# PTsolvers/JustRelax.jl

Hardware: AMD Instinct MI355X
Metric: PT-iterations/s (3D Stokes SolVi3D, 512^3 fp64 block per GPU, block-iterations summed over GPUs) (higher is better)
Workload: dtype f64; 1 GPU; SolVi3D 512^3 per GPU (configs[3]): eta inclusion 1e-3, G=1, K=Inf, dt=Inf, free-slip, pure shear; kernel_form=viscous_limit_no_body_forces, halo=none, arrays=library constructor, field_placement=1 (pool-dealt chunks, mapped once), operand_cache=0

## Files before the change

justrelax.jl_amd/csrc/handle.hip:

```cpp
#include "jrx_internal.hpp"
#include "jrx_tuning.h"

char g_jrx_create_err[512] = {0};

jrx_status jrx_ensure_etatau(jrx_handle *h, size_t n)
{
    if (h->etatau_cap >= n) return JRX_OK;
    if (h->etatau) JRX_TRY(jrx_dev_free(h, h->etatau));
    h->etatau = nullptr;
    h->etatau_cap = 0;
    JRX_TRY(jrx_dev_alloc(h, n * sizeof(double), (void **)&h->etatau, 2));
    h->etatau_cap = n;
    return JRX_OK;
}

jrx_status jrx_check_device(jrx_handle *h)
{
    if (!h) return JRX_ERR_ARG;
    int cur = -1;
    JRX_HIP(h, hipGetDevice(&cur));
    if (cur != h->device)
        return jrx_fail(h, JRX_ERR_ARG, "this handle is bound to device %d but the calling thread's current device is %d (hipSetDevice / torch.cuda.set_device "
                                        "first: the library does not change it)", h->device, cur);
    return JRX_OK;
}

extern "C" {

int32_t jrx_version(void) { return JRX_VERSION; }

#ifndef JRX_BUILD_ID
#define JRX_BUILD_ID "unknown"
#endif
static const char g_jrx_build_marker[] = "JRX_BUILD_ID=" JRX_BUILD_ID;
const char *jrx_build_id(void) { return g_jrx_build_marker + 13; }

const char *jrx_last_error(const jrx_handle *h) { return h ? h->err : g_jrx_create_err; }

jrx_status jrx_create(int32_t device, jrx_handle **out)
{
    if (!out) return jrx_fail(nullptr, JRX_ERR_ARG, "jrx_create: out is NULL");
    *out = nullptr;
    int ndev = 0;
    if (hipGetDeviceCount(&ndev) != hipSuccess || ndev <= 0)
        return jrx_fail(nullptr, JRX_ERR_HIP, "jrx_create: no HIP device visible");
    if (device < 0 || device >= ndev) return jrx_fail(nullptr, JRX_ERR_ARG, "jrx_create: device %d out of range [0,%d)", device, ndev);
    jrx_handle *h = new jrx_handle();
    h->device = device;
    int prev_device = -1;
    (void)hipGetDevice(&prev_device);
#define CK(call)                                                                                   \
    do {                                                                                           \
        hipError_t e_ = (call);                                                                    \
        if (e_ != hipSuccess) {                                                                    \
            jrx_status st_ = jrx_fail(nullptr, JRX_ERR_HIP, "jrx_create: %s -> %s", #call, hipGetErrorString(e_)); \
            (void)jrx_destroy(h);                  \
            if (prev_device >= 0) (void)hipSetDevice(prev_device);                                 \
            return st_;                                                                            \
        }                                                                                          \
    } while (0)
    CK(hipSetDevice(device));
    CK(hipStreamCreateWithFlags(&h->stream, hipStreamNonBlocking));
    {
        int lo = 0, hi = 0;
        CK(hipDeviceGetStreamPriorityRange(&lo, &hi));
        CK(hipStreamCreateWithPriority(&h->halo_stream, hipStreamNonBlocking, hi));
    }
    for (int i = 0; i < 3; i++) CK(hipEventCreateWithFlags(&h->ev[i], hipEventDisableTiming));
    for (int i = 3; i < 8; i++) CK(hipEventCreate(&h->ev[i]));
    CK(hipMalloc(&h->d_partials, sizeof(double) * 4 * kMaxRedBlocks));
    CK(hipMalloc(&h->d_sums, sizeof(double) * 16));
    CK(hipMemset(h->d_sums, 0, sizeof(double) * 16));
    CK(hipHostMalloc(&h->h_sums, sizeof(double) * 16, hipHostMallocDefault));
#undef CK
    if (prev_device >= 0 && prev_device != device) (void)hipSetDevice(prev_device);
    *out = h;
    return JRX_OK;
}

jrx_status jrx_destroy(jrx_handle *h)
{
    if (!h) return JRX_OK;
    (void)hipSetDevice(h->device);
    if (h->comm) (void)jrx_comm_destroy(h);
    if (h->stream) (void)hipStreamSynchronize(h->stream);
    if (h->halo_stream) (void)hipStreamSynchronize(h->halo_stream);
    for (int i = 0; i < 8; i++)
        if (h->ev[i]) (void)hipEventDestroy(h->ev[i]);
    if (h->d_partials) (void)hipFree(h->d_partials);
    if (h->d_sums) (void)hipFree(h->d_sums);
    if (h->h_sums) (void)hipHostFree(h->h_sums);
    jrx_pool_destroy(h);
    for (int q = 0; q < 3; q++)
        if (h->tscratch2[q]) (void)hipFree(h->tscratch2[q]);
    for (int q = 0; q < 6; q++)
        if (h->scratch2d[q]) (void)hipFree(h->scratch2d[q]);
    if (h->stream) (void)hipStreamDestroy(h->stream);
    if (h->halo_stream) (void)hipStreamDestroy(h->halo_stream);
    delete h;
    return JRX_OK;
}

namespace {
struct OptRef { const char *key; int kind; void *p; };
int find_opt(jrx_handle *h, const char *key, bool tuning, OptRef *out)
{
    const OptRef pub[] = {
        {"kernel_variant", 1, &h->kernel_variant}, {"fused_overlap", 1, &h->fused_overlap}, {"thermal_fused", 0, &h->thermal_fused},
        {"fused_comm", 0, &h->fused_comm}, {"loop_graphs", 0, &h->loop_graphs}, {"scratch_sets", 0, &h->scratch_sets},
        {"viscous_limit", 0, &h->viscous_limit}, {"field_placement", 1, &h->field_placement}, {"field_chunk_mib", 1, &h->field_chunk_mib}, {"operand_cache", 0, &h->operand_cache}, {"stat_operand_cache_hits", 2, &h->stat_operand_cache_hits}, {"stat_fused3d_general_hif", 2, &h->stat_fused3d_general_hif},
        {"stat_fused3d", 2, &h->stat_fused3d}, {"stat_fused2d", 2, &h->stat_fused2d}, {"stat_fused2d_b", 2, &h->stat_fused2d_b}, {"stat_sweeps3d", 2, &h->stat_sweeps3d}, {"stat_thermal_fused", 2, &h->stat_thermal_fused},
        {"stat_vep3_fused", 2, &h->stat_vep3_fused}, {"stat_graph_replays", 2, &h->stat_graph_replays},
        {"stat_fused3d_visc", 2, &h->stat_fused3d_visc}, {"stat_fused3d_inkernel", 2, &h->stat_fused3d_inkernel}, {"stat_visc_checks", 2, &h->stat_visc_checks}, {"stat_visc_fallbacks", 2, &h->stat_visc_fallbacks}, {"stat_fused3d_nof1", 2, &h->stat_fused3d_nof1}, {"stat_fused3d_nof2", 2, &h->stat_fused3d_nof2},
        {"stat_weno_calls", 2, &h->stat_weno_calls}, {"stat_weno_fused", 2, &h->stat_weno_fused}, {"stat_principal_calls", 2, &h->stat_principal_calls},
    };
    const OptRef tun[] = {
        {"fused_split", 0, &h->fused_split}, {"fused_tile", 1, &h->fused_tile}, {"fused_ylds", 0, &h->fused_ylds}, {"fused_hiface", 0, &h->fused_hiface}, {"visc_fold", 0, &h->visc_fold}, {"zero_forces", 0, &h->zero_forces}, {"scratch_stagger", 1, &h->scratch_stagger}, {"scratch_contiguous", 0, &h->scratch_contiguous}, {"end_flips", 0, &h->end_flips}, {"comm_bcs_lazy", 0, &h->comm_bcs_lazy}, {"fused_first_pct", 1, &h->fused_first_pct},
        {"b_width_x", 1, &h->b_width_opt[0]}, {"b_width_y", 1, &h->b_width_opt[1]}, {"b_width_z", 1, &h->b_width_opt[2]},
        {"halo_self_rccl", 0, &h->halo_self_rccl}, {"thermal_cfg", 1, &h->thermal_cfg}, {"thermal_xg", 1, &h->thermal_xg}, {"thermal_tile", 1, &h->thermal_tile}, {"thermal_nt", 0, &h->thermal_nt},
        {"fused2d", 0, &h->fused2d}, {"vep3_edges", 1, &h->vep3_edges}, {"vep3_cfg", 1, &h->vep3_cfg}, {"vep3_peel", 0, &h->vep3_peel}, {"vep3_peel_fork", 0, &h->vep3_peel_fork}, {"vep3_nt", 0, &h->vep3_nt}, {"vep3_prekz", 1, &h->vep3_prekz},
        {"vep3_hide_comm", 1, &h->vep3_hide_comm}, {"vep3_fork", 0, &h->vep3_fork}, {"vep3_fuse_pc", 0, &h->vep3_fuse_pc}, {"vep3_np_const", 0, &h->vep3_np_const}, {"vep3_prec_tile", 1, &h->vep3_prec_tile}, {"thermal_np_const", 0, &h->thermal_np_const}, {"thermal_fused_ph", 0, &h->thermal_fused_ph}, {"fused2d_batch", 0, &h->fused2d_batch}, {"fused2d_max_nodes", 1, &h->fused2d_max_nodes}, {"vep3_map", 0, &h->vep3_map}, {"vep3_xcd", 0, &h->vep3_xcd}, {"comm_timeout_ms", 1, &h->comm_timeout_ms}, {"vep_store_all", 0, &h->vep_store_all}, {"chain_profile", 0, &h->chain_profile},
        {"general_hif", 1, &h->general_hif}, {"field_shuffle", 0, &h->field_shuffle}, {"field_pool_pct", 1, &h->field_pool_pct}, {"fused_kz", 1, &h->fused_kz}, {"fused_ym", 1, &h->fused_ym}, {"nbr_feeder", 0, &h->nbr_feeder}, {"stat_fused3d_ym", 2, &h->stat_fused3d_ym}, {"scratch_poison", 1, &h->scratch_poison},
        {"weno_fused", 0, &h->weno_fused}, {"weno_rows", 1, &h->weno_rows},
    };
    if (tuning) {
        for (const OptRef &o : tun)
            if (strcmp(o.key, key) == 0) { *out = o; return 1; }
    } else {
        for (const OptRef &o : pub)
            if (strcmp(o.key, key) == 0) { *out = o; return 1; }
    }
    return 0;
}
jrx_status opt_set(jrx_handle *h, const char *key, int64_t value, bool tuning, const char *fn)
{
    if (!h) return JRX_ERR_ARG;
    if (!key) return jrx_fail(h, JRX_ERR_ARG, "%s: key is NULL", fn);
    OptRef o;
    if (!find_opt(h, key, tuning, &o)) {
        if (find_opt(h, key, !tuning, &o))
            return jrx_fail(h, JRX_ERR_ARG, "%s: '%s' is %s", fn, key, tuning ? "an option of the public ABI (jrx_set_option)" : "a tuning switch (jrx_tuning_set, include/jrx_tuning.h)");
        return jrx_fail(h, JRX_ERR_ARG, "%s: unknown key '%s'", fn, key);
    }
    if (o.kind == 2) return jrx_fail(h, JRX_ERR_ARG, "%s: '%s' is a read-only counter", fn, key);
    if (o.kind == 0) *(bool *)o.p = value != 0;
    else *(int *)o.p = (int)value;
    if (strcmp(key, "comm_timeout_ms") == 0) jrx_comm_set_timeout(h, (double)value * 1e-3);
    return JRX_OK;
}
jrx_status opt_get(jrx_handle *h, const char *key, int64_t *value, bool tuning, const char *fn)
{
    if (!h) return JRX_ERR_ARG;
    if (!key || !value) return jrx_fail(h, JRX_ERR_ARG, "%s: null argument", fn);
    OptRef o;
    if (!find_opt(h, key, tuning, &o)) return jrx_fail(h, JRX_ERR_ARG, "%s: unknown key '%s'", fn, key);
    *value = o.kind == 0 ? (int64_t)*(bool *)o.p : (o.kind == 1 ? (int64_t)*(int *)o.p : *(int64_t *)o.p);
    return JRX_OK;
}
}

jrx_status jrx_fields_dirty(jrx_handle *h)
{
    if (!h) return JRX_ERR_ARG;
    h->opv.valid = false;
    return JRX_OK;
}
jrx_status jrx_set_option(jrx_handle *h, const char *key, int64_t value) { return opt_set(h, key, value, false, "jrx_set_option"); }
jrx_status jrx_get_option(jrx_handle *h, const char *key, int64_t *value) { return opt_get(h, key, value, false, "jrx_get_option"); }
jrx_status jrx_tuning_set(jrx_handle *h, const char *key, int64_t value) { return opt_set(h, key, value, true, "jrx_tuning_set"); }
jrx_status jrx_tuning_get(jrx_handle *h, const char *key, int64_t *value) { return opt_get(h, key, value, true, "jrx_tuning_get"); }
jrx_status jrx_tuning_chain_profile(jrx_handle *h, double out_us[8], int64_t *samples)
{
    if (!h) return JRX_ERR_ARG;
    if (!out_us || !samples) return jrx_fail(h, JRX_ERR_ARG, "jrx_tuning_chain_profile: null argument");
    for (int q = 0; q < 8; q++) out_us[q] = h->chain_us[q];
    *samples = h->chain_n;
    return JRX_OK;
}

int64_t jrx_n_global(int64_t n, int32_t dims, int32_t periodic)
{
    if (n == 1) return 1;
    return (int64_t)dims * (n - 2) + (periodic ? 0 : 2);
}

jrx_status jrx_halo_planes(int64_t n, int64_t nA, int64_t *send_left, int64_t *send_right, int64_t *recv_left, int64_t *recv_right)
{
    const int64_t ol = 2 + (nA - n);
    if (ol < 2 || nA < ol) return JRX_ERR_ARG;
    if (send_left) *send_left = ol - 1;
    if (send_right) *send_right = nA - ol;
    if (recv_left) *recv_left = 0;
    if (recv_right) *recv_right = nA - 1;
    return JRX_OK;
}

jrx_status jrx_cart_create(int32_t rank, int32_t nprocs, const int64_t n[3], const int32_t dims_in[3],
                           const int32_t periods[3], jrx_cart *out)
{
    if (!out || !n || nprocs < 1 || rank < 0 || rank >= nprocs) return JRX_ERR_ARG;
    int32_t dims[3] = {1, 1, 1};
    const bool fixed = dims_in && (dims_in[0] || dims_in[1] || dims_in[2]);
    if (fixed) {
        for (int d = 0; d < 3; d++) dims[d] = dims_in[d] ? dims_in[d] : 1;
    } else {
        int idx[3], na = 0;
        for (int d = 0; d < 3; d++)
            if (n[d] > 1) idx[na++] = d;
        if (na > 0) {
            int fac[32], nf = 0, m = nprocs;
            for (int p = 2; m > 1; p++)
                while (m % p == 0) { fac[nf++] = p; m /= p; }
            int v[3] = {1, 1, 1};
            for (int q = nf - 1; q >= 0; q--) {
                int j = 0;
                for (int a = 1; a < na; a++)
                    if (v[a] < v[j]) j = a;
                v[j] *= fac[q];
            }
            for (int a = 0; a < na; a++)
                for (int b = a + 1; b < na; b++)
                    if (v[b] > v[a]) { int t = v[a]; v[a] = v[b]; v[b] = t; }
            for (int a = 0; a < na; a++) dims[idx[a]] = v[a];
        }
    }
    if ((int64_t)dims[0] * dims[1] * dims[2] != nprocs) return JRX_ERR_ARG;
    out->rank = rank; out->nprocs = nprocs;
    int r = rank;
    for (int d = 2; d >= 0; d--) { out->coords[d] = r % dims[d]; r /= dims[d]; }
    for (int d = 0; d < 3; d++) { out->dims[d] = dims[d]; out->periods[d] = periods ? periods[d] : 0; }
    for (int d = 0; d < 3; d++)
        for (int sgn = 0; sgn < 2; sgn++) {
            int c[3] = {out->coords[0], out->coords[1], out->coords[2]};
            c[d] += sgn ? 1 : -1;
            int nb = -1;
            if (c[d] >= 0 && c[d] < dims[d]) nb = (c[0] * dims[1] + c[1]) * dims[2] + c[2];
            else if (out->periods[d]) {
                c[d] = (c[d] + dims[d]) % dims[d];
                nb = (c[0] * dims[1] + c[1]) * dims[2] + c[2];
            }
            out->neighbor[d][sgn] = nb;
        }
    return JRX_OK;
}

}
```

justrelax.jl_amd/csrc/jrx_internal.hpp:

```cpp
#pragma once
#include <hip/hip_runtime.h>
#include <cstdarg>
#include <cstdint>
#include <cstdio>
#include <cstring>
#include <cmath>
#include "jrx.h"

struct jrx_comm_state;
struct jrx_field_pool;

struct jrx_handle {
    int device = 0;
    hipStream_t stream = nullptr;
    hipStream_t halo_stream = nullptr;
    hipEvent_t ev[8] = {};
    double *d_partials = nullptr;
    double *d_sums = nullptr;
    double *h_sums = nullptr;
    double *etatau = nullptr;
    size_t etatau_cap = 0;
    jrx_comm_state *comm = nullptr;
    jrx_field_pool *pool = nullptr;
    int field_placement = 0;
    int field_chunk_mib = 64;
    bool field_shuffle = true;
    int scratch_poison = 0;
    int fused_kz = 0;
    int field_pool_pct = 70;
    double *scratch_base[10] = {};
    bool scratch_contiguous = false;
    int scratch_stagger = 0, scratch_stagger_used = 0;
    double *scratch[10] = {};
    int scratch_dims[3] = {0, 0, 0};
    double *tscratch[4] = {};
    int tscratch_dims[3] = {0, 0, 0};
    double *scratch2d[6] = {};
    int scratch2d_dims[2] = {0, 0};
    double *tscratch2[3] = {};
    int tscratch2_dims[2] = {0, 0};
    bool loop_graphs = true;
    bool thermal_fused = true;
    int fused_overlap = 3;
    int kernel_variant = 0;
    bool fused_split = false;
    int fused_tile = 2;
    bool fused_comm = true;
    bool vep_store_all = false;
    bool viscous_limit = true;
    bool visc_ok = false;
    int fused_first_pct = 15;
    bool comm_bcs_lazy = false;
    bool end_flips = true;
    bool zero_forces = true;
    bool operand_cache = false;
    struct { bool valid = false; const void *ptr[14] = {}; int64_t n[3] = {}; double dt = 0.0; int flags = 0; bool visc_ok = false; int nof = 0; } opv;
    int64_t stat_operand_cache_hits = 0;
    int nof = 0;
    bool visc_fold = true;
    bool fused_hiface = true;
    bool fused_ylds = true;
    int general_hif = 0;
    int64_t stat_fused3d_general_hif = 0;
    bool nbr_feeder = true;
    int fused_ym = 0;
    int64_t stat_fused3d_ym = 0;
    int b_width_opt[3] = {0, 0, 0};
    bool halo_self_rccl = false;
    int thermal_cfg = 0, thermal_xg = 8;
    bool thermal_nt = false;
    int thermal_tile = 0;
    bool fused2d = true;
    bool vep3_peel = true;
    bool vep3_peel_fork = false;
    bool vep3_nt = false;
    int vep3_prekz = 0;
    int vep3_cfg = 0;
    int vep3_edges = 4;
    int vep3_hide_comm = 0;
    bool fused2d_batch = true;
    int fused2d_max_nodes = 1200000;
    bool thermal_fused_ph = true;
    bool thermal_np_const = true;
    int vep3_prec_tile = 2;
    bool vep3_np_const = true;
    bool vep3_fuse_pc = true;
    bool vep3_fork = false;
    bool vep3_map = true, vep3_xcd = true;
    bool scratch_sets = true;
    bool weno_fused = true;
    int weno_rows = 0;
    int64_t stat_weno_calls = 0, stat_weno_fused = 0;
    int64_t stat_principal_calls = 0;
    int64_t stat_fused3d_inkernel = 0;
    int64_t stat_fused3d_visc = 0, stat_visc_checks = 0, stat_visc_fallbacks = 0, stat_fused3d_nof1 = 0, stat_fused3d_nof2 = 0;
    int64_t stat_sweeps3d = 0;
    int64_t stat_fused2d_b = 0;
    int64_t stat_fused3d = 0, stat_fused2d = 0, stat_thermal_fused = 0, stat_vep3_fused = 0, stat_graph_replays = 0;
    bool chain_profile = false;
    double chain_us[8] = {};
    int64_t chain_n = 0;
    int comm_timeout_ms = 120000;
    char err[512] = {0};
};

static constexpr int kMaxRedBlocks = 2048;

extern char g_jrx_create_err[512];

static inline jrx_status jrx_fail(jrx_handle *h, jrx_status st, const char *fmt, ...)
{
    char *dst = h ? h->err : g_jrx_create_err;
    va_list ap;
    va_start(ap, fmt);
    vsnprintf(dst, 512, fmt, ap);
    va_end(ap);
    return st;
}

#define JRX_HIP(h, call)                                                                         \
    do {                                                                                         \
        hipError_t e_ = (call);                                                                  \
        if (e_ != hipSuccess)                                                                    \
            return jrx_fail((h), JRX_ERR_HIP, "%s:%d: %s -> %s", __FILE__, __LINE__, #call,      \
                            hipGetErrorString(e_));                                              \
    } while (0)

#define JRX_TRY(call)                          \
    do {                                       \
        jrx_status s_ = (call);                \
        if (s_ != JRX_OK) return s_;           \
    } while (0)

#define JRX_LAUNCH_CHECK(h) JRX_HIP(h, hipGetLastError())

struct GraphExecs {
    hipGraphExec_t g[2] = {nullptr, nullptr};
    GraphExecs() = default;
    GraphExecs(const GraphExecs &) = delete;
    GraphExecs &operator=(const GraphExecs &) = delete;
    ~GraphExecs() { reset(); }
    void reset() { for (auto &x : g) if (x) { (void)hipGraphExecDestroy(x); x = nullptr; } }
    hipGraphExec_t &operator[](int i) { return g[i]; }
};

template <class F>
static inline jrx_status jrx_capture_graph(hipStream_t s, hipGraphExec_t *out, F &&body)
{
    *out = nullptr;
    if (hipStreamBeginCapture(s, hipStreamCaptureModeThreadLocal) != hipSuccess) { (void)hipGetLastError(); return JRX_OK; }
    const jrx_status st = body();
    hipGraph_t g = nullptr;
    const hipError_t e = hipStreamEndCapture(s, &g);
    if (st == JRX_OK && e == hipSuccess && g && hipGraphInstantiate(out, g, nullptr, nullptr, 0) != hipSuccess) *out = nullptr;
    if (g) (void)hipGraphDestroy(g);
    (void)hipGetLastError();
    return st;
}
static constexpr double kGraphCells3D = 48.0 * 48.0 * 48.0;

jrx_status jrx_check_device(jrx_handle *h);

jrx_status jrx_dev_alloc(jrx_handle *h, size_t bytes, void **out, int tag = 4);
jrx_status jrx_dev_free(jrx_handle *h, void *p);
void jrx_pool_destroy(jrx_handle *h);

jrx_status jrx_ensure_etatau(jrx_handle *h, size_t n);

__device__ __forceinline__ double wave_sum(double v)
{
#pragma unroll
    for (int off = 32; off > 0; off >>= 1) v += __shfl_down(v, off, 64);
    return v;
}

typedef long long i64;

__device__ __forceinline__ i64 clampll(i64 v, i64 lo, i64 hi) { return v < lo ? lo : (v > hi ? hi : v); }
__device__ __forceinline__ int clampi(int v, int lo, int hi) { return v < lo ? lo : (v > hi ? hi : v); }

__device__ __forceinline__ double dev_dtau_r(double theta_dtau, double eta, double _Gdt)
{
    return 1.0 / (theta_dtau + fma(eta, _Gdt, 1.0));
}
__device__ __forceinline__ double dev_stress_inc(double t, double to, double eta, double e, double _Gdt, double dtr)
{
    return dtr * fma(2.0 * eta, e, fma(-(t - to) * eta, _Gdt, -t));
}

jrx_status jrx_halo_exchange(jrx_handle *h, hipStream_t s, int narrays, double *const *arrays,
                             const int64_t (*ext)[3], const int64_t n[3]);
bool jrx_comm_active(const jrx_handle *h);
jrx_status jrx_allreduce_sum_host(jrx_handle *h, double *vals, int count);
jrx_status jrx_allreduce_host(jrx_handle *h, double *vals, int count, int op);
int jrx_comm_rank(const jrx_handle *h);
void jrx_comm_set_timeout(jrx_handle *h, double seconds);
bool jrx_comm_has_neighbor(const jrx_handle *h, int d, int side);

jrx_status jrx3d_velocity_sweep(jrx_handle *h, hipStream_t s, const jrx_stokes3d_fields *f, const double *etatau, const jrx_stokes3d_params *p, bool diag, int nof = 0);
jrx_status jrx3d_forces_zero(jrx_handle *h, hipStream_t s, const double *fx, const double *fy, const double *fz, int64_t nc, int *nof);
jrx_status jrx3d_velocity_hidden(jrx_handle *h, const jrx_stokes3d_fields *f, const double *etatau, const jrx_stokes3d_params *p, bool diag, int bc_kind);
jrx_status jrx3d_scaleU(jrx_handle *h, hipStream_t s, const jrx_stokes3d_fields *f, const jrx_stokes3d_params *p);
jrx_status jrx3d_bcs(jrx_handle *h, hipStream_t s, double *Vx, double *Vy, double *Vz, int nx, int ny, int nz, uint32_t fs, uint32_t ns, uint32_t pe);
jrx_status jrx3d_bcs_faces(jrx_handle *h, hipStream_t s, double *Vx, double *Vy, double *Vz, int nx, int ny, int nz, uint32_t fs, uint32_t ns);
jrx_status jrx3d_sumsq(jrx_handle *h, hipStream_t s, const jrx_stokes3d_fields *f, const jrx_stokes3d_params *p);

jrx_status jrx2d_bcs(jrx_handle *h, hipStream_t s, double *Vx, double *Vy, int nx, int ny, uint32_t fs, uint32_t ns, uint32_t pe);
jrx_status jrx2d_sumsq(jrx_handle *h, hipStream_t s, const jrx_stokes2d_fields *f, const jrx_stokes2d_params *p);
bool jrx2d_spacing_ok(const double *const sp[6]);
```

justrelax.jl_amd/csrc/stokes3d.hip:

```cpp
#include <vector>
#include <cstdlib>
#include "jrx_internal.hpp"
#include "jrx_kernels.hpp"
#include "stokes3d_kernels.hpp"
#include "jrx_tuning.h"

namespace {

SweepArgs make_args(const jrx_stokes3d_fields *f, const double *etatau, const jrx_stokes3d_params *p)
{
    SweepArgs a;
    a.f = *f;
    a.o = Out10{f->P, f->txx, f->tyy, f->tzz, f->tyz, f->txz, f->txy, f->Vx, f->Vy, f->Vz};
    a.etatau = etatau;
    a._dx = p->_dx; a._dy = p->_dy; a._dz = p->_dz;
    a.dt = p->dt; a.r = p->r; a.theta_dtau = p->theta_dtau; a.eta_dtau = p->eta_dtau;
    a.L = make_lay((int)p->nx, (int)p->ny, (int)p->nz);
    a.i0 = a.j0 = a.k0 = 0;
    a.i1 = a.j1 = a.k1 = 0;
    return a;
}

jrx_status check_params(jrx_handle *h, const jrx_stokes3d_fields *f, const jrx_stokes3d_params *p)
{
    if (!h) return JRX_ERR_ARG;
    if (!f || !p) return jrx_fail(h, JRX_ERR_ARG, "null fields/params");
    JRX_TRY(jrx_check_device(h));
    if (p->nx < 3 || p->ny < 3 || p->nz < 3) return jrx_fail(h, JRX_ERR_ARG, "3D Stokes needs at least 3 cells per dimension");
    const double cells = (double)(p->nx + 2) * (double)(p->ny + 2) * (double)(p->nz + 2);
    if (cells >= 2147483647.0) return jrx_fail(h, JRX_ERR_UNSUPPORTED, "local block too large for 32-bit plane indices");
    const void *req[] = {f->P, f->P0, f->Q, f->Vx, f->Vy, f->Vz, f->txx, f->tyy, f->tzz, f->tyz, f->txz, f->txy,
                         f->toxx, f->toyy, f->tozz, f->toyz, f->toxz, f->toxy, f->eta, f->K, f->G, f->fx, f->fy, f->fz};
    for (const void *q : req)
        if (!q) return jrx_fail(h, JRX_ERR_ARG, "a required field pointer is NULL");
    return JRX_OK;
}

jrx_status check_diag(jrx_handle *h, const jrx_stokes3d_fields *f)
{
    const void *req[] = {f->divV, f->exx, f->eyy, f->ezz, f->eyz, f->exz, f->exy, f->RP, f->Rx, f->Ry, f->Rz, f->Ux, f->Uy, f->Uz};
    for (const void *q : req)
        if (!q) return jrx_fail(h, JRX_ERR_ARG, "a diagnostic field pointer (∇V, ε, R, U) is NULL");
    return JRX_OK;
}

jrx_status launch_stress_v1(jrx_handle *h, hipStream_t s, SweepArgs a, bool diag, int i0, int i1, int j0, int j1, int k0, int k1)
{
    if (i1 <= i0 || j1 <= j0 || k1 <= k0) return JRX_OK;
    a.i0 = i0; a.i1 = i1; a.j0 = j0; a.j1 = j1; a.k0 = k0; a.k1 = k1;
    const i64 plane = (i64)(i1 - i0) * (j1 - j0);
    dim3 grid((unsigned)((plane + 255) / 256), (unsigned)(k1 - k0));
    if (diag) hipLaunchKernelGGL(k_stress3d<true>, grid, dim3(256), 0, s, a);
    else hipLaunchKernelGGL(k_stress3d<false>, grid, dim3(256), 0, s, a);
    JRX_LAUNCH_CHECK(h);
    return JRX_OK;
}

jrx_status launch_velocity_v1(jrx_handle *h, hipStream_t s, SweepArgs a, bool diag, int i0, int i1, int j0, int j1, int k0, int k1)
{
    if (i1 <= i0 || j1 <= j0 || k1 <= k0) return JRX_OK;
    a.i0 = i0; a.i1 = i1; a.j0 = j0; a.j1 = j1; a.k0 = k0; a.k1 = k1;
    const i64 plane = (i64)(i1 - i0) * (j1 - j0);
    dim3 grid((unsigned)((plane + 255) / 256), (unsigned)(k1 - k0));
    if (diag) hipLaunchKernelGGL(k_velocity3d<true>, grid, dim3(256), 0, s, a);
    else hipLaunchKernelGGL(k_velocity3d<false>, grid, dim3(256), 0, s, a);
    JRX_LAUNCH_CHECK(h);
    return JRX_OK;
}

bool fits_u32(const Lay3 &L)
{
    const double m = (double)(L.nx + 2) * (double)(L.ny + 2) * (double)(L.nz + 2) * 8.0;
    return m < 4294967296.0;
}

template <class F>
__device__ __forceinline__ void scan_pairs(const double *__restrict__ p, i64 n, F f)
{
    if (n <= 0) return;
    const i64 stride = (i64)gridDim.x * blockDim.x, t0 = (i64)blockIdx.x * blockDim.x + threadIdx.x;
    const i64 head = (reinterpret_cast<uintptr_t>(p) & 15) ? 1 : 0;
    const double2 *__restrict__ q = reinterpret_cast<const double2 *>(p + head);
    const i64 m = n - head;
    for (i64 t = t0; t < (m >> 1); t += stride) { const double2 v = q[t]; f(v.x); f(v.y); }
    if (t0 == 0) { if (head) f(p[0]); if (m & 1) f(p[n - 1]); }
}
__global__ __launch_bounds__(256) void k_visc_operands_ok(const double *__restrict__ c0, const double *__restrict__ c1, const double *__restrict__ c2, const double *__restrict__ c3,
                                                          const double *__restrict__ c4, const double *__restrict__ eta, i64 nc, const double *__restrict__ K, const double *__restrict__ G,
                                                          const double *__restrict__ yz, i64 nyz, const double *__restrict__ xz, i64 nxz, const double *__restrict__ xy, i64 nxy, int *bad,
                                                          const unsigned long long *__restrict__ fx, const unsigned long long *__restrict__ fy, const unsigned long long *__restrict__ fz)
{
    bool b = false;
    unsigned long long bxy = 0, bz = 0;
    auto fin = [&](double v) { b |= !isfinite(v); };
    auto mod = [&](double v) { b |= (v != v) || v == 0.0; };
    scan_pairs(c0, nc, fin); scan_pairs(c1, nc, fin); scan_pairs(c2, nc, fin); scan_pairs(c3, nc, fin); scan_pairs(c4, nc, fin); scan_pairs(eta, nc, fin);
    scan_pairs(K, nc, mod); scan_pairs(G, nc, mod);
    scan_pairs(yz, nyz, fin); scan_pairs(xz, nxz, fin); scan_pairs(xy, nxy, fin);
    if (fx) {
        scan_pairs(reinterpret_cast<const double *>(fx), nc, [&](double v) { bxy |= (unsigned long long)__double_as_longlong(v); });
        scan_pairs(reinterpret_cast<const double *>(fy), nc, [&](double v) { bxy |= (unsigned long long)__double_as_longlong(v); });
        scan_pairs(reinterpret_cast<const double *>(fz), nc, [&](double v) { bz |= (unsigned long long)__double_as_longlong(v); });
    }
    if (__any(b) && (threadIdx.x & 63) == 0) atomicOr(bad, 1);
    if (fx) {
        const int m = (__any(bxy != 0) ? 2 : 0) | (__any(bz != 0) ? 4 : 0);
        if (m && (threadIdx.x & 63) == 0) atomicOr(bad, m);
    }
}

__global__ __launch_bounds__(256) void k_forces_zero(const unsigned long long *__restrict__ fx, const unsigned long long *__restrict__ fy, const unsigned long long *__restrict__ fz, i64 nc, int *bad)
{
    const i64 stride = (i64)gridDim.x * blockDim.x;
    unsigned long long bxy = 0, bz = 0;
    for (i64 t = (i64)blockIdx.x * blockDim.x + threadIdx.x; t < nc; t += stride) { bxy |= fx[t] | fy[t]; bz |= fz[t]; }
    const int m = (__any(bxy != 0) ? 2 : 0) | (__any(bz != 0) ? 4 : 0);
    if (m && (threadIdx.x & 63) == 0) atomicOr(bad, m);
}

static jrx_status visc_operands_local(jrx_handle *h, const jrx_stokes3d_fields *f, const jrx_stokes3d_params *p, bool forces);
jrx_status visc_operands_check(jrx_handle *h, const jrx_stokes3d_fields *f, const jrx_stokes3d_params *p, bool forces = true)
{
    JRX_TRY(visc_operands_local(h, f, p, forces));
    if (jrx_comm_active(h)) {
        double v[2] = {h->visc_ok ? 0.0 : 1.0, (double)(2 - h->nof)};
        JRX_TRY(jrx_allreduce_host(h, v, 2, 1));
        h->visc_ok = v[0] == 0.0;
        h->nof = 2 - (int)v[1];
    }
    return JRX_OK;
}
static jrx_status visc_operands_local(jrx_handle *h, const jrx_stokes3d_fields *f, const jrx_stokes3d_params *p, bool forces)
{
    h->visc_ok = false;
    h->nof = 0;
    forces = forces && h->zero_forces && f->fx && f->fy && f->fz;
    const void *key[14] = {f->P0, f->Q, f->toxx, f->toyy, f->tozz, f->toyz, f->toxz, f->toxy, f->eta, f->K, f->G, f->fx, f->fy, f->fz};
    const int kflags = (forces ? 1 : 0) | (h->viscous_limit ? 2 : 0) | (p->displacement_bcs ? 4 : 0) | (h->kernel_variant << 3);
    if (h->operand_cache && h->opv.valid && h->opv.dt == p->dt && h->opv.flags == kflags && h->opv.n[0] == p->nx && h->opv.n[1] == p->ny && h->opv.n[2] == p->nz &&
        memcmp(h->opv.ptr, key, sizeof(key)) == 0) {
        h->visc_ok = h->opv.visc_ok;
        h->nof = h->opv.nof;
        h->stat_operand_cache_hits++;
        return JRX_OK;
    }
    struct Remember {
        jrx_handle *h; const void *const *key; const jrx_stokes3d_params *p; int kflags; bool ok = false;
        ~Remember() {
            h->opv.valid = ok;
            if (!ok) return;
            memcpy(h->opv.ptr, key, sizeof(h->opv.ptr));
            h->opv.n[0] = p->nx; h->opv.n[1] = p->ny; h->opv.n[2] = p->nz; h->opv.dt = p->dt; h->opv.flags = kflags; h->opv.visc_ok = h->visc_ok; h->opv.nof = h->nof;
        }
    } remember{h, key, p, kflags};
    if ((!h->viscous_limit || p->dt != INFINITY) && forces && !p->displacement_bcs && (h->kernel_variant == 0 || h->kernel_variant == 3) && p->nx >= 48) {
        const i64 nc = (i64)p->nx * p->ny * p->nz;
        int *d_bad = reinterpret_cast<int *>(h->d_sums + 6), *h_bad = reinterpret_cast<int *>(h->h_sums + 6);
        hipStream_t s = h->stream;
        JRX_HIP(h, hipMemsetAsync(d_bad, 0, sizeof(double), s));
        hipLaunchKernelGGL(k_forces_zero, dim3(2048), dim3(256), 0, s, reinterpret_cast<const unsigned long long *>(f->fx), reinterpret_cast<const unsigned long long *>(f->fy),
                           reinterpret_cast<const unsigned long long *>(f->fz), nc, d_bad);
        JRX_LAUNCH_CHECK(h);
        JRX_HIP(h, hipMemcpyAsync(h_bad, d_bad, sizeof(double), hipMemcpyDeviceToHost, s));
        JRX_HIP(h, hipStreamSynchronize(s));
        if (!(*h_bad & 2)) h->nof = (*h_bad & 4) ? 1 : 2;
        remember.ok = true;
        return JRX_OK;
    }
    if (!h->viscous_limit || p->dt != INFINITY) { remember.ok = true; return JRX_OK; }
    const i64 nx = p->nx, ny = p->ny, nz = p->nz;
    int *d_bad = reinterpret_cast<int *>(h->d_sums + 6), *h_bad = reinterpret_cast<int *>(h->h_sums + 6);
    hipStream_t s = h->stream;
    JRX_HIP(h, hipMemsetAsync(d_bad, 0, sizeof(double), s));
    hipLaunchKernelGGL(k_visc_operands_ok, dim3(4096), dim3(256), 0, s, f->P0, f->Q, f->toxx, f->toyy, f->tozz, f->eta, nx * ny * nz, f->K, f->G, f->toyz, nx * (ny + 1) * (nz + 1),
                       f->toxz, (nx + 1) * ny * (nz + 1), f->toxy, (nx + 1) * (ny + 1) * nz, d_bad,
                       forces ? reinterpret_cast<const unsigned long long *>(f->fx) : nullptr, reinterpret_cast<const unsigned long long *>(f->fy), reinterpret_cast<const unsigned long long *>(f->fz));
    JRX_LAUNCH_CHECK(h);
    JRX_HIP(h, hipMemcpyAsync(h_bad, d_bad, sizeof(double), hipMemcpyDeviceToHost, s));
    JRX_HIP(h, hipStreamSynchronize(s));
    h->visc_ok = ((*h_bad & 1) == 0);
    if (h->visc_ok && forces && !(*h_bad & 2)) h->nof = (*h_bad & 4) ? 1 : 2;
    h->stat_visc_checks++;
    if (!h->visc_ok) h->stat_visc_fallbacks++;
    remember.ok = true;
    return JRX_OK;
}

template <int TX, int TY, int KZ>
jrx_status launch_stress_zb(jrx_handle *h, hipStream_t s, const SweepArgs &a, bool diag)
{
    const TileMap tm = make_tilemap(a.L.nx, a.L.ny, a.L.nz, TX, TY, KZ);
    if (diag) hipLaunchKernelGGL((k_stress3d_zb<true, TX, TY, KZ, 4, false, 8, true>), dim3(tm.ntiles), dim3(TX * TY), 0, s, a, tm);
    else if (h->viscous_limit && h->visc_ok && a.dt == INFINITY)
        hipLaunchKernelGGL((k_stress3d_zb<false, TX, TY, KZ, 4, false, 8, true, true>), dim3(tm.ntiles), dim3(TX * TY), 0, s, a, tm);
    else hipLaunchKernelGGL((k_stress3d_zb<false, TX, TY, KZ, 4, false, 8, true>), dim3(tm.ntiles), dim3(TX * TY), 0, s, a, tm);
    JRX_LAUNCH_CHECK(h);
    h->stat_sweeps3d++;
    return JRX_OK;
}

template <int TX, int TY, int KZ>
jrx_status launch_velocity_zb(jrx_handle *h, hipStream_t s, const SweepArgs &a, bool diag, int nof = 0)
{
    const TileMap tm = make_tilemap(a.i1 - a.i0, a.j1 - a.j0, a.k1 - a.k0, TX, TY, KZ);
    if (!diag && nof == 2) hipLaunchKernelGGL((k_velocity3d_zb<false, TX, TY, KZ, 4, 8, true, 2>), dim3(tm.ntiles), dim3(TX * TY), 0, s, a, tm);
    else if (!diag && nof == 1) hipLaunchKernelGGL((k_velocity3d_zb<false, TX, TY, KZ, 4, 8, true, 1>), dim3(tm.ntiles), dim3(TX * TY), 0, s, a, tm);
    else if (diag) hipLaunchKernelGGL((k_velocity3d_zb<true, TX, TY, KZ, 4, 8, true>), dim3(tm.ntiles), dim3(TX * TY), 0, s, a, tm);
    else hipLaunchKernelGGL((k_velocity3d_zb<false, TX, TY, KZ, 4, 8, true>), dim3(tm.ntiles), dim3(TX * TY), 0, s, a, tm);
    JRX_LAUNCH_CHECK(h);
    h->stat_sweeps3d++;
    return JRX_OK;
}

static jrx_status launch_stress_boxes(jrx_handle *h, hipStream_t s, const SweepArgs &a, const int (*box)[6], int nbox, bool diag,
                                      const GhostRule *rule = nullptr);

jrx_status launch_stress(jrx_handle *h, hipStream_t s, SweepArgs a, bool diag, int i0, int i1, int j0, int j1, int k0, int k1)
{
    const int nx = a.L.nx, ny = a.L.ny, nz = a.L.nz;
    const bool full = i0 == 0 && j0 == 0 && k0 == 0 && i1 == nx + 1 && j1 == ny + 1 && k1 == nz + 1;
    const bool small = (double)nx * ny * nz <= 681472.0;
    if (h->kernel_variant == 1 || !full || !fits_u32(a.L) || nx < 48 || small) return launch_stress_v1(h, s, a, diag, i0, i1, j0, j1, k0, k1);
    a.i0 = a.j0 = a.k0 = 0; a.i1 = nx; a.j1 = ny; a.k1 = nz;
    if (nx > 384) JRX_TRY((launch_stress_zb<512, 1, 4>(h, s, a, diag)));
    else if (nx > 192) JRX_TRY((launch_stress_zb<256, 1, 8>(h, s, a, diag)));
    else if (nx > 96) JRX_TRY((launch_stress_zb<128, 2, 8>(h, s, a, diag)));
    else JRX_TRY((launch_stress_zb<64, 4, 8>(h, s, a, diag)));
    const int planes[3][6] = {{nx, nx + 1, 0, ny + 1, 0, nz + 1}, {0, nx, ny, ny + 1, 0, nz + 1}, {0, nx, 0, ny, nz, nz + 1}};
    return launch_stress_boxes(h, s, a, planes, 3, diag);
}

jrx_status launch_velocity(jrx_handle *h, hipStream_t s, SweepArgs a, bool diag, int i0, int i1, int j0, int j1, int k0, int k1, int nof = 0)
{
    if (i1 <= i0 || j1 <= j0 || k1 <= k0) return JRX_OK;
    const int w = i1 - i0;
    const bool small = (double)w * (j1 - j0) * (k1 - k0) <= 681472.0;
    if (h->kernel_variant == 1 || !fits_u32(a.L) || w < 48 || (k1 - k0) < 4 || small) return launch_velocity_v1(h, s, a, diag, i0, i1, j0, j1, k0, k1);
    a.i0 = i0; a.i1 = i1; a.j0 = j0; a.j1 = j1; a.k0 = k0; a.k1 = k1;
    if (w > 384) return launch_velocity_zb<512, 1, 4>(h, s, a, diag, nof);
    if (w > 192) return launch_velocity_zb<256, 1, 8>(h, s, a, diag, nof);
    if (w > 96) return launch_velocity_zb<128, 2, 8>(h, s, a, diag, nof);
    return launch_velocity_zb<64, 4, 8>(h, s, a, diag, nof);
}

jrx_status launch_scaleU(jrx_handle *h, hipStream_t s, const jrx_stokes3d_fields *f, const jrx_stokes3d_params *p)
{
    const i64 n0 = (i64)(p->nx + 1) * (p->ny + 2) * (p->nz + 2), n1 = (i64)(p->nx + 2) * (p->ny + 1) * (p->nz + 2),
              n2 = (i64)(p->nx + 2) * (p->ny + 2) * (p->nz + 1);
    hipLaunchKernelGGL(k_scale3, dim3(2048), dim3(256), 0, s, f->Ux, f->Vx, n0, f->Uy, f->Vy, n1, f->Uz, f->Vz, n2, p->dt);
    JRX_LAUNCH_CHECK(h);
    return JRX_OK;
}

jrx_status launch_bcs(jrx_handle *h, hipStream_t s, double *Vx, double *Vy, double *Vz, int nx, int ny, int nz,
                      uint32_t fs, uint32_t ns, uint32_t pe)
{
    BcArr A[3] = {{Vx, {nx + 1, ny + 2, nz + 2}}, {Vy, {nx + 2, ny + 1, nz + 2}}, {Vz, {nx + 2, ny + 2, nz + 1}}};
    auto run = [&](int type, int dim, bool lo, bool hi) -> jrx_status {
        if (!lo && !hi) return JRX_OK;
        const int d1 = dim == 0 ? 1 : 0, d2 = dim == 2 ? 1 : 2;
        int na = 0, nb = 0;
        for (int c = 0; c < 3; c++) { na = A[c].n[d1] > na ? A[c].n[d1] : na; nb = A[c].n[d2] > nb ? A[c].n[d2] : nb; }
        hipLaunchKernelGGL(k_bc3d, dim3((na + 255) / 256, nb), dim3(256), 0, s, A[0], A[1], A[2], type, dim, (int)lo, (int)hi);
        JRX_LAUNCH_CHECK(h);
        return JRX_OK;
    };
    if (ns) {
        JRX_TRY(run(1, 0, ns & JRX_FACE_LEFT, ns & JRX_FACE_RIGHT));
        JRX_TRY(run(1, 1, ns & JRX_FACE_FRONT, ns & JRX_FACE_BACK));
        JRX_TRY(run(1, 2, ns & JRX_FACE_BOT, ns & JRX_FACE_TOP));
    }
    if (fs) {
        JRX_TRY(run(0, 1, fs & JRX_FACE_FRONT, fs & JRX_FACE_BACK));
        JRX_TRY(run(0, 2, fs & JRX_FACE_TOP, fs & JRX_FACE_BOT));
        JRX_TRY(run(0, 0, fs & JRX_FACE_LEFT, fs & JRX_FACE_RIGHT));
    }
    if (pe) {
        JRX_TRY(run(2, 0, pe & JRX_FACE_LEFT, pe & JRX_FACE_RIGHT));
        JRX_TRY(run(2, 1, pe & JRX_FACE_FRONT, pe & JRX_FACE_BACK));
        JRX_TRY(run(2, 2, pe & JRX_FACE_BOT, pe & JRX_FACE_TOP));
    }
    return JRX_OK;
}

static jrx_status launch_bcs_faces(jrx_handle *h, hipStream_t s, double *Vx, double *Vy, double *Vz, int nx, int ny, int nz, uint32_t fs, uint32_t ns)
{
    BcArr A[3] = {{Vx, {nx + 1, ny + 2, nz + 2}}, {Vy, {nx + 2, ny + 1, nz + 2}}, {Vz, {nx + 2, ny + 2, nz + 1}}};
    auto ty = [&](uint32_t fsbit, uint32_t nsbit) { return (ns & nsbit) ? 2 : ((fs & fsbit) ? 1 : 0); };
    const int t[6] = {ty(JRX_FACE_LEFT, JRX_FACE_LEFT), ty(JRX_FACE_RIGHT, JRX_FACE_RIGHT), ty(JRX_FACE_FRONT, JRX_FACE_FRONT),
                      ty(JRX_FACE_BACK, JRX_FACE_BACK), ty(JRX_FACE_TOP, JRX_FACE_BOT), ty(JRX_FACE_BOT, JRX_FACE_TOP)};
    if (!(t[0] | t[1] | t[2] | t[3] | t[4] | t[5])) return JRX_OK;
    const int na = (nx > ny ? nx : ny) + 2, nb = (ny > nz ? ny : nz) + 2;
    hipLaunchKernelGGL(k_bc3d_faces, dim3((na + 255) / 256, nb, 3), dim3(256), 0, s, A[0], A[1], A[2], t[0], t[1], t[2], t[3], t[4], t[5]);
    JRX_LAUNCH_CHECK(h);
    return JRX_OK;
}

static jrx_status launch_stress_boxes(jrx_handle *h, hipStream_t s, const SweepArgs &a, const int (*box)[6], int nbox, bool diag, const GhostRule *rule)
{
    StressBoxes B = {};
    int tot = 0;
    for (int q = 0; q < nbox; q++) {
        const int *b = box[q];
        if (b[1] <= b[0] || b[3] <= b[2] || b[5] <= b[4]) continue;
        const i64 plane = (i64)(b[1] - b[0]) * (b[3] - b[2]);
        for (int c = 0; c < 6; c++) B.box[B.n][c] = b[c];
        B.per_plane[B.n] = (int)((plane + 255) / 256);
        B.start[B.n] = tot;
        tot += B.per_plane[B.n] * (b[5] - b[4]);
        B.n++;
    }
    if (!B.n) return JRX_OK;
    B.start[B.n] = tot;
    const GhostRule none = {{0, 0, 0, 0, 0, 0}};
    const bool visc = !diag && h->viscous_limit && h->visc_ok && a.dt == INFINITY;
    if (rule && visc) hipLaunchKernelGGL((k_stress3d_boxes<false, true, true>), dim3((unsigned)tot), dim3(256), 0, s, a, B, *rule);
    else if (rule) hipLaunchKernelGGL((k_stress3d_boxes<false, true>), dim3((unsigned)tot), dim3(256), 0, s, a, B, *rule);
    else if (visc) hipLaunchKernelGGL((k_stress3d_boxes<false, false, true>), dim3((unsigned)tot), dim3(256), 0, s, a, B, none);
    else if (diag) hipLaunchKernelGGL(k_stress3d_boxes<true>, dim3((unsigned)tot), dim3(256), 0, s, a, B, none);
    else hipLaunchKernelGGL(k_stress3d_boxes<false>, dim3((unsigned)tot), dim3(256), 0, s, a, B, none);
    JRX_LAUNCH_CHECK(h);
    return JRX_OK;
}

jrx_status launch_sumsq(jrx_handle *h, hipStream_t s, const jrx_stokes3d_fields *f, const jrx_stokes3d_params *p)
{
    const int nx = (int)p->nx, ny = (int)p->ny, nz = (int)p->nz;
    RedArr A0 = {f->Rx, {nx - 1, ny, nz}, 1}, A1 = {f->Ry, {nx, ny - 1, nz}, 1}, A2 = {f->Rz, {nx, ny, nz - 1}, 1},
           A3 = {f->RP, {nx, ny, nz}, 0};
    const i64 n = (i64)nx * ny * nz;
    int nb = (int)((n + 256 * 8 - 1) / (256 * 8));
    nb = nb < 1 ? 1 : (nb > kMaxRedBlocks ? kMaxRedBlocks : nb);
    hipLaunchKernelGGL(k_sumsq_partial, dim3(nb), dim3(256), 0, s, A0, A1, A2, A3, h->d_partials);
    JRX_LAUNCH_CHECK(h);
    hipLaunchKernelGGL(k_sumsq_final, dim3(1), dim3(256), 0, s, h->d_partials, nb, h->d_sums);
    JRX_LAUNCH_CHECK(h);
    return JRX_OK;
}

}

jrx_status jrx3d_velocity_sweep(jrx_handle *h, hipStream_t s, const jrx_stokes3d_fields *f, const double *etatau, const jrx_stokes3d_params *p, bool diag, int nof)
{
    if (diag && (!f->Rx || !f->Ry || !f->Rz)) return jrx_fail(h, JRX_ERR_ARG, "residual arrays are NULL");
    return launch_velocity(h, s, make_args(f, etatau, p), diag, 0, (int)p->nx, 0, (int)p->ny, 0, (int)p->nz, nof);
}
jrx_status jrx3d_forces_zero(jrx_handle *h, hipStream_t s, const double *fx, const double *fy, const double *fz, int64_t nc, int *nof)
{
    *nof = 0;
    if (!h->zero_forces || !fx || !fy || !fz) return JRX_OK;
    int *d_bad = reinterpret_cast<int *>(h->d_sums + 6), *h_bad = reinterpret_cast<int *>(h->h_sums + 6);
    JRX_HIP(h, hipMemsetAsync(d_bad, 0, sizeof(double), s));
    hipLaunchKernelGGL(k_forces_zero, dim3(2048), dim3(256), 0, s, reinterpret_cast<const unsigned long long *>(fx), reinterpret_cast<const unsigned long long *>(fy),
                       reinterpret_cast<const unsigned long long *>(fz), (i64)nc, d_bad);
    JRX_LAUNCH_CHECK(h);
    JRX_HIP(h, hipMemcpyAsync(h_bad, d_bad, sizeof(double), hipMemcpyDeviceToHost, s));
    JRX_HIP(h, hipStreamSynchronize(s));
    if (!(*h_bad & 2)) *nof = (*h_bad & 4) ? 1 : 2;
    return JRX_OK;
}
jrx_status jrx3d_scaleU(jrx_handle *h, hipStream_t s, const jrx_stokes3d_fields *f, const jrx_stokes3d_params *p) { return launch_scaleU(h, s, f, p); }
jrx_status jrx3d_bcs(jrx_handle *h, hipStream_t s, double *Vx, double *Vy, double *Vz, int nx, int ny, int nz, uint32_t fs, uint32_t ns, uint32_t pe)
{
    return launch_bcs(h, s, Vx, Vy, Vz, nx, ny, nz, fs, ns, pe);
}
jrx_status jrx3d_sumsq(jrx_handle *h, hipStream_t s, const jrx_stokes3d_fields *f, const jrx_stokes3d_params *p) { return launch_sumsq(h, s, f, p); }
jrx_status jrx3d_bcs_faces(jrx_handle *h, hipStream_t s, double *Vx, double *Vy, double *Vz, int nx, int ny, int nz, uint32_t fs, uint32_t ns)
{
    return launch_bcs_faces(h, s, Vx, Vy, Vz, nx, ny, nz, fs, ns);
}

jrx_status jrx3d_velocity_hidden(jrx_handle *h, const jrx_stokes3d_fields *f, const double *etatau, const jrx_stokes3d_params *p, bool diag, int bc_kind)
{
    if (diag && (!f->Rx || !f->Ry || !f->Rz)) return jrx_fail(h, JRX_ERR_ARG, "residual arrays are NULL");
    const int nx = (int)p->nx, ny = (int)p->ny, nz = (int)p->nz;
    hipStream_t s = h->stream;
    const SweepArgs a = make_args(f, etatau, p);
    int bx = p->b_width[0] > 0 ? p->b_width[0] : 4, by = p->b_width[1] > 0 ? p->b_width[1] : 4,
        bz = p->b_width[2] > 0 ? p->b_width[2] : 4;
    if (h->b_width_opt[0] > 0) bx = h->b_width_opt[0];
    if (h->b_width_opt[1] > 0) by = h->b_width_opt[1];
    if (h->b_width_opt[2] > 0) bz = h->b_width_opt[2];
    const int xa = bx < nx / 2 ? bx : nx / 2, ya = by < ny / 2 ? by : ny / 2, za = bz < nz / 2 ? bz : nz / 2;
    hipStream_t hs = h->halo_stream;
    JRX_HIP(h, hipEventRecord(h->ev[0], s));
    JRX_HIP(h, hipStreamWaitEvent(hs, h->ev[0], 0));
    JRX_TRY(launch_velocity(h, hs, a, diag, 0, nx, 0, ny, 0, za));
    JRX_TRY(launch_velocity(h, hs, a, diag, 0, nx, 0, ny, nz - za, nz));
    JRX_TRY(launch_velocity(h, hs, a, diag, 0, nx, 0, ya, za, nz - za));
    JRX_TRY(launch_velocity(h, hs, a, diag, 0, nx, ny - ya, ny, za, nz - za));
    JRX_TRY(launch_velocity(h, hs, a, diag, 0, xa, ya, ny - ya, za, nz - za));
    JRX_TRY(launch_velocity(h, hs, a, diag, nx - xa, nx, ya, ny - ya, za, nz - za));
    JRX_TRY(launch_velocity(h, s, a, diag, xa, nx - xa, ya, ny - ya, za, nz - za));
    if (diag) {
        JRX_HIP(h, hipEventRecord(h->ev[1], s));
        JRX_HIP(h, hipStreamWaitEvent(hs, h->ev[1], 0));
        JRX_TRY(launch_scaleU(h, hs, f, p));
    }
    if (bc_kind == 0) JRX_TRY(launch_bcs(h, hs, f->Vx, f->Vy, f->Vz, nx, ny, nz, p->free_slip, p->no_slip, p->periodic));
    else if (bc_kind == 1) JRX_TRY(launch_bcs_faces(h, hs, f->Vx, f->Vy, f->Vz, nx, ny, nz, p->free_slip, p->no_slip));
    else if (bc_kind == 2) JRX_TRY(launch_bcs(h, hs, f->Ux, f->Uy, f->Uz, nx, ny, nz, p->free_slip, p->no_slip, p->periodic));
    double *arrs[3] = {f->Vx, f->Vy, f->Vz};
    const int64_t ext[3][3] = {{nx + 1, ny + 2, nz + 2}, {nx + 2, ny + 1, nz + 2}, {nx + 2, ny + 2, nz + 1}};
    const int64_t n[3] = {nx, ny, nz};
    JRX_TRY(jrx_halo_exchange(h, hs, 3, arrs, ext, n));
    JRX_HIP(h, hipEventRecord(h->ev[2], hs));
    JRX_HIP(h, hipStreamWaitEvent(s, h->ev[2], 0));
    return JRX_OK;
}

extern "C" {

jrx_status jrx_stokes3d_sweep_stress(jrx_handle *h, const jrx_stokes3d_fields *f, const jrx_stokes3d_params *p, int32_t flags)
{
    JRX_TRY(check_params(h, f, p));
    const bool diag = flags & JRX_OUT_DIAG;
    if (diag) JRX_TRY(check_diag(h, f));
    SweepArgs a = make_args(f, nullptr, p);
    if (h->operand_cache) JRX_TRY(visc_operands_check(h, f, p, false));
    else { h->visc_ok = false; h->nof = 0; }
    JRX_TRY(launch_stress(h, h->stream, a, diag, 0, (int)p->nx + 1, 0, (int)p->ny + 1, 0, (int)p->nz + 1));
    JRX_HIP(h, hipStreamSynchronize(h->stream));
    return JRX_OK;
}

jrx_status jrx_stokes3d_sweep_velocity(jrx_handle *h, const jrx_stokes3d_fields *f, const double *etatau,
                                       const jrx_stokes3d_params *p, int32_t flags)
{
    JRX_TRY(check_params(h, f, p));
    if (!etatau) return jrx_fail(h, JRX_ERR_ARG, "etatau is NULL");
    const bool diag = flags & JRX_OUT_DIAG;
    if (diag) JRX_TRY(check_diag(h, f));
    SweepArgs a = make_args(f, etatau, p);
    JRX_TRY(launch_velocity(h, h->stream, a, diag, 0, (int)p->nx, 0, (int)p->ny, 0, (int)p->nz));
    if (diag) JRX_TRY(launch_scaleU(h, h->stream, f, p));
    JRX_HIP(h, hipStreamSynchronize(h->stream));
    return JRX_OK;
}

jrx_status jrx_flow_bcs3d(jrx_handle *h, double *Vx, double *Vy, double *Vz, int64_t nx, int64_t ny, int64_t nz,
                          uint32_t free_slip, uint32_t no_slip, uint32_t periodic)
{
    if (!h) return JRX_ERR_ARG;
    if (!Vx || !Vy || !Vz) return jrx_fail(h, JRX_ERR_ARG, "null velocity pointer");
    JRX_TRY(launch_bcs(h, h->stream, Vx, Vy, Vz, (int)nx, (int)ny, (int)nz, free_slip, no_slip, periodic));
    JRX_HIP(h, hipStreamSynchronize(h->stream));
    return JRX_OK;
}

jrx_status jrx_stokes3d_residual_sumsq(jrx_handle *h, const jrx_stokes3d_fields *f, const jrx_stokes3d_params *p, double out[4])
{
    JRX_TRY(check_params(h, f, p));
    JRX_TRY(check_diag(h, f));
    JRX_TRY(launch_sumsq(h, h->stream, f, p));
    JRX_HIP(h, hipMemcpyAsync(h->h_sums, h->d_sums, 4 * sizeof(double), hipMemcpyDeviceToHost, h->stream));
    JRX_HIP(h, hipStreamSynchronize(h->stream));
    for (int c = 0; c < 4; c++) out[c] = h->h_sums[c];
    return JRX_OK;
}

jrx_status jrx_velocity2displacement(jrx_handle *h, double *const U[3], const double *const V[3], const int64_t n[3], double dt)
{
    if (!h) return JRX_ERR_ARG;
    if (!U || !V || !n || !U[0] || !U[1] || !V[0] || !V[1]) return jrx_fail(h, JRX_ERR_ARG, "velocity2displacement!: null argument");
    hipLaunchKernelGGL(k_scale3, dim3(2048), dim3(256), 0, h->stream, U[0], V[0], (i64)n[0], U[1], V[1], (i64)n[1], U[2], V[2], (i64)(U[2] ? n[2] : 0), dt);
    JRX_LAUNCH_CHECK(h);
    JRX_HIP(h, hipStreamSynchronize(h->stream));
    return JRX_OK;
}
jrx_status jrx_displacement2velocity(jrx_handle *h, double *const V[3], const double *const U[3], const int64_t n[3], double dt)
{
    return jrx_velocity2displacement(h, V, U, n, 1.0 / dt);
}

jrx_status jrx_compute_dt(jrx_handle *h, const double *const V[3], const int64_t n[3], const double di[3], int32_t ndim, double dt_diff, double *dt_out)
{
    if (!h) return JRX_ERR_ARG;
    if (!V || !n || !di || !dt_out || ndim < 2 || ndim > 3 || !V[0] || !V[1] || (ndim == 3 && !V[2])) return jrx_fail(h, JRX_ERR_ARG, "compute_dt: bad argument");
    i64 nmax = 0;
    for (int d = 0; d < ndim; d++) nmax = n[d] > nmax ? (i64)n[d] : nmax;
    int nb = (int)((nmax + 2047) / 2048);
    nb = nb < 1 ? 1 : (nb > kMaxRedBlocks ? kMaxRedBlocks : nb);
    hipStream_t s = h->stream;
    hipLaunchKernelGGL(k_maxabs_partial, dim3(nb), dim3(256), 0, s, V[0], (i64)n[0], V[1], (i64)n[1], ndim == 3 ? V[2] : (const double *)nullptr,
                       (i64)(ndim == 3 ? n[2] : 0), h->d_partials);
    hipLaunchKernelGGL(k_maxabs_final, dim3(1), dim3(256), 0, s, h->d_partials, nb, h->d_sums);
    JRX_LAUNCH_CHECK(h);
    JRX_HIP(h, hipMemcpyAsync(h->h_sums, h->d_sums, 4 * sizeof(double), hipMemcpyDeviceToHost, s));
    JRX_HIP(h, hipStreamSynchronize(s));
    double m[3] = {h->h_sums[0], h->h_sums[1], h->h_sums[2]};
    JRX_TRY(jrx_allreduce_host(h, m, ndim, 1));
    double dt_adv = INFINITY;
    for (int d = 0; d < ndim; d++) dt_adv = fmin(dt_adv, di[d] * (1.0 / m[d]));
    *dt_out = fmin(dt_diff, dt_adv * 0.9);
    return JRX_OK;
}

jrx_status jrx_compute_maxloc(jrx_handle *h, double *B, const double *A, int64_t nx, int64_t ny, int64_t nz)
{
    if (!h) return JRX_ERR_ARG;
    if (!A || !B || nx < 1 || ny < 1 || nz < 1) return jrx_fail(h, JRX_ERR_ARG, "bad compute_maxloc arguments");
    if (A == B) return jrx_fail(h, JRX_ERR_ARG, "compute_maxloc!: B must not alias A");
    const i64 plane = (i64)nx * ny;
    hipLaunchKernelGGL(k_maxloc, dim3((unsigned)((plane + 255) / 256), (unsigned)nz), dim3(256), 0, h->stream, B, A, (int)nx, (int)ny, (int)nz);
    JRX_LAUNCH_CHECK(h);
    JRX_HIP(h, hipStreamSynchronize(h->stream));
    return JRX_OK;
}

}

struct FusedShape { int tx, ty, kz; };
static void fused_tiles(const Lay3 &L, const FusedShape S, int nt[3])
{
    nt[0] = (L.nx + S.tx - 3) / (S.tx - 2); nt[1] = (L.ny + S.ty - 2) / (S.ty - 1); nt[2] = (L.nz + S.kz - 1) / S.kz;
}
static FusedShape fused_shape(const jrx_handle *h, const Lay3 &L, double dt)
{
    const bool narrow = h->fused_tile == 1 || (h->fused_tile == 2 && L.nx > 62 && L.nx <= 90);
    FusedShape S = narrow ? FusedShape{32, 8, 8} : FusedShape{64, 4, 8};
    int nt[3];
    {
        const int tkz = h->fused_kz == 8 || h->fused_kz == 12 ? h->fused_kz : (L.nz >= 384 ? 12 : 8);
        const FusedShape T{64, 8, tkz};
        fused_tiles(L, T, nt);
        const bool visc = h->viscous_limit && h->visc_ok && dt == INFINITY;
        if (h->fused_ylds && h->fused_tile == 4) return FusedShape{64, 16, 12};
        if (h->fused_ylds && (h->fused_tile == 3 || ((visc || L.nz >= 384) && h->fused_tile == 2 && !narrow && (long long)nt[0] * nt[1] * nt[2] >= 4096))) return T;
    }
    for (int kz = 8; kz >= 2; kz /= 2) {
        S.kz = kz;
        fused_tiles(L, S, nt);
        if ((long long)nt[0] * nt[1] * nt[2] >= 512) break;
    }
    return S;
}

struct Iter3D {
    jrx_handle *h;
    const jrx_stokes3d_params *p;
    const double *etatau;
    jrx_stokes3d_fields cur;
    Out10 setU, setS;
    bool pt_user = true, v_user = true;
    bool flip_A = false, flip_B = false;
    bool all_user() const { return pt_user && v_user; }
    bool stress_done = false;
    bool fusable = false;
    bool bcs_ordered[2] = {false, false};
    bool ghosts_stale = false;
};

static Out10 out_of(const jrx_stokes3d_fields &f) { return Out10{f.P, f.txx, f.tyy, f.tzz, f.tyz, f.txz, f.txy, f.Vx, f.Vy, f.Vz}; }
static void set_state(jrx_stokes3d_fields &f, const Out10 &o)
{
    f.P = o.P; f.txx = o.txx; f.tyy = o.tyy; f.tzz = o.tzz; f.tyz = o.tyz; f.txz = o.txz; f.txy = o.txy; f.Vx = o.Vx; f.Vy = o.Vy; f.Vz = o.Vz;
}
static Out10 mix_sets(const Out10 &pt, const Out10 &v) { return Out10{pt.P, pt.txx, pt.tyy, pt.tzz, pt.tyz, pt.txz, pt.txy, v.Vx, v.Vy, v.Vz}; }

static jrx_status ensure_scratch(jrx_handle *h, int nx, int ny, int nz)
{
    const size_t n[10] = {(size_t)nx * ny * nz, (size_t)nx * ny * nz, (size_t)nx * ny * nz, (size_t)nx * ny * nz,
                          (size_t)nx * (ny + 1) * (nz + 1), (size_t)(nx + 1) * ny * (nz + 1), (size_t)(nx + 1) * (ny + 1) * nz,
                          (size_t)(nx + 1) * (ny + 2) * (nz + 2), (size_t)(nx + 2) * (ny + 1) * (nz + 2), (size_t)(nx + 2) * (ny + 2) * (nz + 1)};
    if (h->scratch_dims[0] == nx && h->scratch_dims[1] == ny && h->scratch_dims[2] == nz && h->scratch[0] && h->scratch_stagger_used == h->scratch_stagger + 1000003 * (int)h->scratch_contiguous) return JRX_OK;
    for (int q = 0; q < 10; q++) {
        if (h->scratch_base[q]) JRX_TRY(jrx_dev_free(h, h->scratch_base[q]));
        h->scratch[q] = h->scratch_base[q] = nullptr;
    }
    h->scratch_dims[0] = h->scratch_dims[1] = h->scratch_dims[2] = 0;
    const size_t stg = (size_t)(h->scratch_stagger > 0 ? h->scratch_stagger : 0) & ~(size_t)255;
    for (int q = 0; q < 10; q++) {
        void *b = nullptr;
        const int keep = h->field_placement;
        if (h->scratch_contiguous) h->field_placement = 2;
        const jrx_status st = jrx_dev_alloc(h, n[q] * sizeof(double) + (size_t)q * stg, &b, 1);
        h->field_placement = keep;
        JRX_TRY(st);
        h->scratch_base[q] = (double *)b;
        h->scratch[q] = (double *)((char *)b + (size_t)q * stg);
    }
    h->scratch_stagger_used = h->scratch_stagger + 1000003 * (int)h->scratch_contiguous;
    h->scratch_dims[0] = nx; h->scratch_dims[1] = ny; h->scratch_dims[2] = nz;
    return JRX_OK;
}

static jrx_status iter_begin(Iter3D &I, jrx_handle *h, const jrx_stokes3d_fields *f, const double *etatau, const jrx_stokes3d_params *p)
{
    I.h = h; I.p = p; I.etatau = etatau;
    JRX_TRY(visc_operands_check(h, f, p));
    I.cur = *f;
    I.setU = out_of(*f);
    I.pt_user = I.v_user = true; I.flip_A = I.flip_B = false; I.stress_done = false;
    const Lay3 L = make_lay((int)p->nx, (int)p->ny, (int)p->nz);
    I.fusable = !p->displacement_bcs && (h->kernel_variant == 0 || h->kernel_variant == 3) && h->scratch_sets && (h->fused_comm || !jrx_comm_active(h)) && fits_u32(L) && p->nx >= 48 && p->ny >= 8 && p->nz >= 8;
    if (I.fusable && h->kernel_variant == 0) {
        const FusedShape S = fused_shape(h, L, p->dt);
        int nt[3];
        fused_tiles(L, S, nt);
        const int W = p->nx > 384 ? 512 : (p->nx > 192 ? 256 : (p->nx > 96 ? 128 : 64));
        const double lanes_f = (double)nt[0] * S.tx * S.ty / (S.ty - 1), lanes_s = (double)((p->nx + W - 1) / W) * W;
        if ((double)p->nx * (double)p->ny * (double)p->nz >= 1e6 && 0.62 * lanes_f > 1.15 * lanes_s) I.fusable = false;
    }
    if (I.fusable) {
        JRX_TRY(ensure_scratch(h, (int)p->nx, (int)p->ny, (int)p->nz));
        double **S = h->scratch;
        I.setS = Out10{S[0], S[1], S[2], S[3], S[4], S[5], S[6], S[7], S[8], S[9]};
        const int nx = (int)p->nx, ny = (int)p->ny, nz = (int)p->nz;
        const BcArr D[3] = {{I.setS.Vx, {nx + 1, ny + 2, nz + 2}}, {I.setS.Vy, {nx + 2, ny + 1, nz + 2}}, {I.setS.Vz, {nx + 2, ny + 2, nz + 1}}};
        const CBcArr S3[3] = {{f->Vx, {nx + 1, ny + 2, nz + 2}}, {f->Vy, {nx + 2, ny + 1, nz + 2}}, {f->Vz, {nx + 2, ny + 2, nz + 1}}};
        const int m1 = (nx > ny ? nx : ny) + 2, m2 = (ny > nz ? ny : nz) + 2;
        hipLaunchKernelGGL(k_copy_shell3, dim3((unsigned)(((i64)m1 * m2 + 255) / 256), 6, 3), dim3(256), 0, h->stream, D[0], D[1], D[2], S3[0], S3[1], S3[2]);
        JRX_LAUNCH_CHECK(h);
    }
    return JRX_OK;
}

static int general_hif_eff(const jrx_handle *h);
template <int TX, int TY, int KZ, int MW = 4, int XGV = 1, bool GH = false>
static jrx_status launch_fused_t(jrx_handle *h, hipStream_t s, const SweepArgs &a, const FusedBC &bc, const int b[6], bool hiface, bool fold, const FusedShell *shell = nullptr)
{
    const int ntx = b[1] - b[0], nty = b[3] - b[2], ntz = b[5] - b[4];
    if (ntx <= 0 || nty <= 0 || ntz <= 0) return JRX_OK;
    const bool visc = h->viscous_limit && h->visc_ok && a.dt == INFINITY && h->fused_ylds;
    const bool vf = h->visc_fold;
    const bool gfold = GH && fold && !visc && h->fused_ylds && general_hif_eff(h) != 0;
    const int nof = ((visc && fold && vf) || (!visc && h->fused_ylds && (!shell || gfold))) ? h->nof : 0;
    if constexpr (GH) {
        if (gfold) {
            const int nblk = shell ? (shell->cls == 0 ? shell->start[1] : shell->start[shell->nbox] - shell->start[1]) : ntx * nty * ntz;
            const FusedShell none = FusedShell{};
            const FusedShell &sh = shell ? *shell : none;
            if (nblk > 0) {
#define GHL(MW_, NBR_, NOF_) hipLaunchKernelGGL((k_fused3d<TX, TY, KZ, MW_, 1, false, XGV, false, true, 3, 1, 0, false, true, false, NBR_, NOF_>), dim3((unsigned)nblk), dim3(TX * TY), 0, s, a, bc, ntx, nty, b[0], b[2], b[4], sh)
                const int key = (general_hif_eff(h) == 3 ? 100 : 0) + (shell ? 10 : 0) + nof;
                switch (key) {
                case 0: GHL(4, false, 0); break; case 1: GHL(4, false, 1); break; case 2: GHL(4, false, 2); break;
                case 10: GHL(4, true, 0); break; case 11: GHL(4, true, 1); break; case 12: GHL(4, true, 2); break;
                case 100: GHL(3, false, 0); break; case 101: GHL(3, false, 1); break; case 102: GHL(3, false, 2); break;
                case 110: GHL(3, true, 0); break; case 111: GHL(3, true, 1); break; default: GHL(3, true, 2); break;
                }
#undef GHL
            }
            JRX_LAUNCH_CHECK(h);
            if (shell && shell->cls == 0) return JRX_OK;
            if (shell) h->stat_fused3d_inkernel++;
            if (nof == 1) h->stat_fused3d_nof1++; else if (nof == 2) h->stat_fused3d_nof2++;
            h->stat_fused3d++;
            h->stat_fused3d_general_hif++;
            return JRX_OK;
        }
    }
    if (shell) {
        if (!(visc && fold)) return jrx_fail(h, JRX_ERR_ARG, "internal: the in-kernel neighbour faces need a one-launch form of the kernel");
        const int nblk = shell->cls == 0 ? shell->start[1] : shell->start[shell->nbox] - shell->start[1];
        if (nblk > 0) {
            if (nof == 2)
                hipLaunchKernelGGL((k_fused3d<TX, TY, KZ, MW, 1, false, XGV, false, true, 3, 1, 0, true, true, true, true, 2>), dim3((unsigned)nblk), dim3(TX * TY), 0, s, a, bc, ntx, nty, b[0], b[2], b[4], *shell);
            else if (nof == 1)
                hipLaunchKernelGGL((k_fused3d<TX, TY, KZ, MW, 1, false, XGV, false, true, 3, 1, 0, true, true, true, true, 1>), dim3((unsigned)nblk), dim3(TX * TY), 0, s, a, bc, ntx, nty, b[0], b[2], b[4], *shell);
            else
                hipLaunchKernelGGL((k_fused3d<TX, TY, KZ, MW, 1, false, XGV, false, true, 3, 1, 0, true, true, true, true>), dim3((unsigned)nblk), dim3(TX * TY), 0, s, a, bc, ntx, nty, b[0], b[2], b[4], *shell);
        }
        if (shell->cls != 0) { h->stat_fused3d_inkernel++; if (nof == 1) h->stat_fused3d_nof1++; else if (nof == 2) h->stat_fused3d_nof2++; }
        else { JRX_LAUNCH_CHECK(h); return JRX_OK; }
    } else if (visc && fold && vf && TX == 64 && TY == 8 && h->fused_ym > 1) {
        const int ym = h->fused_ym >= 3 ? 4 : 2;
        const unsigned nblk = (unsigned)(ntx * ((nty + ym - 1) / ym) * ntz);
#define YML(NOF_, YM_) hipLaunchKernelGGL((k_fused3d<TX, TY, KZ, MW, 1, false, XGV, false, true, 3, 1, 0, true, true, true, false, NOF_, YM_>), dim3(nblk), dim3(TX * TY), 0, s, a, bc, ntx, nty, b[0], b[2], b[4])
        if constexpr (TX == 64 && TY == 8) {
            switch (nof * 10 + (ym >= 3 ? 4 : 2)) {
            case 2: YML(0, 2); break; case 4: YML(0, 4); break;
            case 12: YML(1, 2); break; case 14: YML(1, 4); break;
            case 22: YML(2, 2); break; default: YML(2, 4); break;
            }
        }
#undef YML
        if (nof == 1) h->stat_fused3d_nof1++; else if (nof == 2) h->stat_fused3d_nof2++;
        h->stat_fused3d_ym++;
    } else if (visc && fold && vf) {
        if (nof == 2) {
            hipLaunchKernelGGL((k_fused3d<TX, TY, KZ, MW, 1, false, XGV, false, true, 3, 1, 0, true, true, true, false, 2>), dim3((unsigned)(ntx * nty * ntz)), dim3(TX * TY), 0, s, a, bc, ntx, nty, b[0], b[2], b[4]);
            h->stat_fused3d_nof2++;
        } else if (nof == 1) {
            hipLaunchKernelGGL((k_fused3d<TX, TY, KZ, MW, 1, false, XGV, false, true, 3, 1, 0, true, true, true, false, 1>), dim3((unsigned)(ntx * nty * ntz)), dim3(TX * TY), 0, s, a, bc, ntx, nty, b[0], b[2], b[4]);
            h->stat_fused3d_nof1++;
        } else
            hipLaunchKernelGGL((k_fused3d<TX, TY, KZ, MW, 1, false, XGV, false, true, 3, 1, 0, true, true, true>), dim3((unsigned)(ntx * nty * ntz)), dim3(TX * TY), 0, s, a, bc, ntx, nty, b[0], b[2], b[4]);
    }
    else if (visc && fold)
        hipLaunchKernelGGL((k_fused3d<TX, TY, KZ, MW, 1, false, XGV, false, true, 3, 1, 0, true, true>), dim3((unsigned)(ntx * nty * ntz)), dim3(TX * TY), 0, s, a, bc, ntx, nty, b[0], b[2], b[4]);
    else if (visc && !hiface && vf)
        hipLaunchKernelGGL((k_fused3d<TX, TY, KZ, MW, 1, false, XGV, false, true, 3, 1, 0, true, false, true>), dim3((unsigned)(ntx * nty * ntz)), dim3(TX * TY), 0, s, a, bc, ntx, nty, b[0], b[2], b[4]);
    else if (visc && hiface)
        hipLaunchKernelGGL((k_fused3d<TX, TY, KZ, MW, 1, false, XGV, false, true, 3, 1, 1, true>), dim3((unsigned)(ntx * nty * ntz)), dim3(TX * TY), 0, s, a, bc, ntx, nty, b[0], b[2], b[4]);
    else if (visc)
        hipLaunchKernelGGL((k_fused3d<TX, TY, KZ, MW, 1, false, XGV, false, true, 3, 1, 0, true>), dim3((unsigned)(ntx * nty * ntz)), dim3(TX * TY), 0, s, a, bc, ntx, nty, b[0], b[2], b[4]);
    else if (h->fused_ylds && hiface) {
        if (nof == 2)
            hipLaunchKernelGGL((k_fused3d<TX, TY, KZ, MW, 1, true, XGV, false, true, 3, 1, 1, false, false, false, false, 2>), dim3((unsigned)(ntx * nty * ntz)), dim3(TX * TY), 0, s, a, bc, ntx, nty, b[0], b[2], b[4]);
        else if (nof == 1)
            hipLaunchKernelGGL((k_fused3d<TX, TY, KZ, MW, 1, true, XGV, false, true, 3, 1, 1, false, false, false, false, 1>), dim3((unsigned)(ntx * nty * ntz)), dim3(TX * TY), 0, s, a, bc, ntx, nty, b[0], b[2], b[4]);
        else
            hipLaunchKernelGGL((k_fused3d<TX, TY, KZ, MW, 1, true, XGV, false, true, 3, 1, 1>), dim3((unsigned)(ntx * nty * ntz)), dim3(TX * TY), 0, s, a, bc, ntx, nty, b[0], b[2], b[4]);
        if (nof == 1) h->stat_fused3d_nof1++; else if (nof == 2) h->stat_fused3d_nof2++;
    } else if (h->fused_ylds && nof == 2) {
        hipLaunchKernelGGL((k_fused3d<TX, TY, KZ, MW, 1, true, XGV, false, true, 3, 1, 0, false, false, false, false, 2>), dim3((unsigned)(ntx * nty * ntz)), dim3(TX * TY), 0, s, a, bc, ntx, nty, b[0], b[2], b[4]);
        h->stat_fused3d_nof2++;
    } else if (h->fused_ylds && nof == 1) {
        hipLaunchKernelGGL((k_fused3d<TX, TY, KZ, MW, 1, true, XGV, false, true, 3, 1, 0, false, false, false, false, 1>), dim3((unsigned)(ntx * nty * ntz)), dim3(TX * TY), 0, s, a, bc, ntx, nty, b[0], b[2], b[4]);
        h->stat_fused3d_nof1++;
    } else if (h->fused_ylds)
        hipLaunchKernelGGL((k_fused3d<TX, TY, KZ, MW, 1, true, XGV, false, true, 3, 1>), dim3((unsigned)(ntx * nty * ntz)), dim3(TX * TY), 0, s, a, bc, ntx, nty, b[0], b[2], b[4]);
    else
        hipLaunchKernelGGL((k_fused3d<TX, TY, KZ, 2, 1, false, 8, false, true>), dim3((unsigned)(ntx * nty * ntz)), dim3(TX * TY), 0, s, a, bc, ntx, nty, b[0], b[2], b[4]);
    JRX_LAUNCH_CHECK(h);
    h->stat_fused3d++;
    if (visc) h->stat_fused3d_visc++;
    return JRX_OK;
}
static FusedShape fused_shape(const jrx_handle *h, const Lay3 &L, double dt);
static int general_hif_eff(const jrx_handle *h) { return h->general_hif > 0 ? h->general_hif : 0; }
static bool fused_folds_hiface(const jrx_handle *h, const SweepArgs &a)
{
    if (!h->fused_hiface || !h->fused_ylds) return false;
    if (h->viscous_limit && h->visc_ok && a.dt == INFINITY) return true;
    const FusedShape S = fused_shape(h, a.L, a.dt);
    return general_hif_eff(h) != 0 && S.tx == 64 && S.ty == 4;
}
static jrx_status launch_fused(jrx_handle *h, hipStream_t s, const SweepArgs &a, const FusedBC &bc, const int b[6], bool hiface = false, bool fold = false, const FusedShell *shell = nullptr)
{
    const FusedShape S = fused_shape(h, a.L, a.dt);
    const int kz = S.kz;
    if (S.tx == 64 && S.ty == 16) return launch_fused_t<64, 16, 12, 4, 2>(h, s, a, bc, b, hiface, fold, shell);
    if (S.tx == 64 && S.ty == 8) return kz == 12 ? launch_fused_t<64, 8, 12, 4, 4>(h, s, a, bc, b, hiface, fold, shell) : launch_fused_t<64, 8, 8, 4, 4>(h, s, a, bc, b, hiface, fold, shell);
    if (S.tx == 64) {
        if (kz == 8) return launch_fused_t<64, 4, 8, 4, 1, true>(h, s, a, bc, b, hiface, fold, shell);
        if (kz == 4) return launch_fused_t<64, 4, 4, 4, 1, true>(h, s, a, bc, b, hiface, fold, shell);
        return launch_fused_t<64, 4, 2, 4, 1, true>(h, s, a, bc, b, hiface, fold, shell);
    }
    if (kz == 8) return launch_fused_t<32, 8, 8>(h, s, a, bc, b, hiface, fold, shell);
    if (kz == 4) return launch_fused_t<32, 8, 4>(h, s, a, bc, b, hiface, fold, shell);
    return launch_fused_t<32, 8, 2>(h, s, a, bc, b, hiface, fold, shell);
}

static void physical_faces(const jrx_handle *h, uint32_t *fs_keep, uint32_t *ns_keep)
{
    const uint32_t fs_lo[3] = {JRX_FACE_LEFT, JRX_FACE_FRONT, JRX_FACE_TOP}, fs_hi[3] = {JRX_FACE_RIGHT, JRX_FACE_BACK, JRX_FACE_BOT};
    const uint32_t ns_lo[3] = {JRX_FACE_LEFT, JRX_FACE_FRONT, JRX_FACE_BOT}, ns_hi[3] = {JRX_FACE_RIGHT, JRX_FACE_BACK, JRX_FACE_TOP};
    *fs_keep = *ns_keep = 0;
    for (int d = 0; d < 3; d++) {
        if (!jrx_comm_has_neighbor(h, d, 0)) { *fs_keep |= fs_lo[d]; *ns_keep |= ns_lo[d]; }
        if (!jrx_comm_has_neighbor(h, d, 1)) { *fs_keep |= fs_hi[d]; *ns_keep |= ns_hi[d]; }
    }
}

static inline int imin(int a, int b) { return a < b ? a : b; }
static jrx_status iter_step(Iter3D &I, bool diag, bool fuse_next, hipEvent_t *tev, int *was_fused, double *ncells_timed = nullptr, hipEvent_t *cev = nullptr, int *chain_mode = nullptr)
{
    jrx_handle *h = I.h;
    const jrx_stokes3d_params *p = I.p;
    const int nx = (int)p->nx, ny = (int)p->ny, nz = (int)p->nz;
    hipStream_t s = h->stream;
    SweepArgs a = make_args(&I.cur, I.etatau, p);
    if (was_fused) *was_fused = 0;
    if (chain_mode) *chain_mode = 0;
    if (ncells_timed) *ncells_timed = (double)nx * ny * nz;
    if (tev) JRX_HIP(h, hipEventRecord(tev[0], s));
    if (!I.stress_done) {
        if (I.flip_A) {
            const Out10 other = mix_sets(I.pt_user ? I.setS : I.setU, I.v_user ? I.setU : I.setS);
            a.o = other;
            JRX_TRY(launch_stress(h, s, a, diag, 0, nx + 1, 0, ny + 1, 0, nz + 1));
            set_state(I.cur, other);
            I.pt_user = !I.pt_user;
            I.flip_A = false;
            a = make_args(&I.cur, I.etatau, p);
        } else
            JRX_TRY(launch_stress(h, s, a, diag, 0, nx + 1, 0, ny + 1, 0, nz + 1));
    }
    I.stress_done = false;
    if (tev) JRX_HIP(h, hipEventRecord(tev[1], s));

    if (I.fusable && fuse_next && !diag) {
        const Out10 dst = mix_sets(I.pt_user ? I.setS : I.setU, I.v_user ? I.setS : I.setU);
        a.o = dst;
        FusedBC bc;
        const uint32_t fs = p->free_slip, ns = p->no_slip;
        bc.fsL = !!(fs & JRX_FACE_LEFT); bc.nsL = !!(ns & JRX_FACE_LEFT); bc.fsF = !!(fs & JRX_FACE_FRONT); bc.nsF = !!(ns & JRX_FACE_FRONT);
        bc.fsK0 = !!(fs & JRX_FACE_TOP);  bc.nsK0 = !!(ns & JRX_FACE_BOT);
        bc.nsR = !!(ns & JRX_FACE_RIGHT); bc.nsBk = !!(ns & JRX_FACE_BACK); bc.nsK1 = !!(ns & JRX_FACE_TOP);
        bc.fsR = !!(fs & JRX_FACE_RIGHT); bc.fsBk = !!(fs & JRX_FACE_BACK); bc.fsK1 = !!(fs & JRX_FACE_BOT);
        bc.nbL = bc.nbR = bc.nbF = bc.nbBk = bc.nbK0 = bc.nbK1 = 0;
        bc.feed = h->nbr_feeder ? 1 : 0;
        int nt[3];
        const FusedShape S = fused_shape(h, a.L, a.dt);
        fused_tiles(a.L, S, nt);
        const bool comm = jrx_comm_active(h);
        const bool per = p->periodic != 0;
        hipStream_t bs = s;
        bool &ordered = I.bcs_ordered[I.v_user ? 1 : 0];
        auto fused_bcs = [&](hipStream_t st) -> jrx_status {
            if (ordered && !per) return launch_bcs_faces(h, st, dst.Vx, dst.Vy, dst.Vz, nx, ny, nz, p->free_slip, p->no_slip);
            ordered = true;
            return launch_bcs(h, st, dst.Vx, dst.Vy, dst.Vz, nx, ny, nz, p->free_slip, p->no_slip, p->periodic);
        };
        bool nb[3][2] = {};
        bool folded = false;
        bool rules_with_comm = false;
        const bool overlap = h->fused_overlap == 1;
        const bool visc_form = h->viscous_limit && h->visc_ok && a.dt == INFINITY;
        const bool inkernel = (h->fused_overlap == 3 || h->fused_overlap == 4) && comm && !per && fused_folds_hiface(h, a) && (h->visc_fold || !visc_form);
        const bool early = (h->fused_overlap == 2 || (h->fused_overlap >= 3 && !inkernel)) && comm && !per;
        const bool split = !comm && !per && h->fused_split && nt[0] > 1 && nt[1] > 1 && nt[2] > 1;
        if (split) {
            bs = h->halo_stream;
            JRX_HIP(h, hipEventRecord(h->ev[0], s));
            JRX_HIP(h, hipStreamWaitEvent(bs, h->ev[0], 0));
            const int inner[6] = {0, nt[0] - 1, 0, nt[1] - 1, 0, nt[2] - 1};
            JRX_TRY(launch_fused(h, s, a, bc, inner));
            if (tev) JRX_HIP(h, hipEventRecord(tev[3], s));
            const int hx[6] = {nt[0] - 1, nt[0], 0, nt[1], 0, nt[2]}, hy[6] = {0, nt[0] - 1, nt[1] - 1, nt[1], 0, nt[2]},
                      hz[6] = {0, nt[0] - 1, 0, nt[1] - 1, nt[2] - 1, nt[2]};
            JRX_TRY(launch_fused(h, bs, a, bc, hx, true));
            JRX_TRY(launch_fused(h, bs, a, bc, hy, true));
            JRX_TRY(launch_fused(h, bs, a, bc, hz, true));
            I.ghosts_stale = true;
            if (ncells_timed) *ncells_timed = (double)imin(nx, (nt[0] - 1) * (S.tx - 2)) * (double)imin(ny, (nt[1] - 1) * (S.ty - 1)) * (double)imin(nz, (nt[2] - 1) * S.kz);
        } else if (inkernel) {
            bs = h->halo_stream;
            JRX_HIP(h, hipEventRecord(h->ev[0], s));
            JRX_HIP(h, hipStreamWaitEvent(bs, h->ev[0], 0));
            bool nbf[3][2];
            for (int d = 0; d < 3; d++) { nbf[d][0] = jrx_comm_has_neighbor(h, d, 0); nbf[d][1] = jrx_comm_has_neighbor(h, d, 1); }
            {
                const int w = 4;
                const int xa = imin(w, nx / 2), ya = imin(w, ny / 2), za = imin(w, nz / 2);
                const bool L0 = nbf[0][0], H0 = nbf[0][1], L1 = nbf[1][0], H1 = nbf[1][1], L2 = nbf[2][0], H2 = nbf[2][1];
                const int z0 = L2 ? za : 0, z1 = H2 ? nz - za : nz, y0 = L1 ? ya : 0, y1 = H1 ? ny - ya : ny;
                if (L2) JRX_TRY(launch_velocity(h, bs, a, false, 0, nx, 0, ny, 0, za));
                if (H2) JRX_TRY(launch_velocity(h, bs, a, false, 0, nx, 0, ny, nz - za, nz));
                if (L1) JRX_TRY(launch_velocity(h, bs, a, false, 0, nx, 0, ya, z0, z1));
                if (H1) JRX_TRY(launch_velocity(h, bs, a, false, 0, nx, ny - ya, ny, z0, z1));
                if (L0) JRX_TRY(launch_velocity(h, bs, a, false, 0, xa, y0, y1, z0, z1));
                if (H0) JRX_TRY(launch_velocity(h, bs, a, false, nx - xa, nx, y0, y1, z0, z1));
            }
            if (cev) { JRX_HIP(h, hipEventRecord(cev[0], bs)); JRX_HIP(h, hipEventRecord(cev[1], bs)); }
            {
                double *arrs[3] = {dst.Vx, dst.Vy, dst.Vz};
                const int64_t ext[3][3] = {{nx + 1, ny + 2, nz + 2}, {nx + 2, ny + 1, nz + 2}, {nx + 2, ny + 2, nz + 1}};
                const int64_t n[3] = {nx, ny, nz};
                JRX_TRY(jrx_halo_exchange(h, bs, 3, arrs, ext, n));
            }
            JRX_HIP(h, hipEventRecord(h->ev[2], bs));
            if (cev) JRX_HIP(h, hipEventRecord(cev[2], bs));
            FusedShell sh;
            memset(&sh, 0, sizeof(sh));
            int lo[3], hi[3];
            for (int d = 0; d < 3; d++) { lo[d] = (nbf[d][0] && nt[d] > 1) ? 1 : 0; hi[d] = (nbf[d][1] && nt[d] > 1) ? nt[d] - 1 : nt[d]; if (hi[d] < lo[d]) hi[d] = lo[d]; }
            for (int d = 0; d < 3; d++) if ((nbf[d][0] || nbf[d][1]) && nt[d] == 1) { lo[d] = 0; hi[d] = 0; }
            int zs = lo[2] + ((hi[2] - lo[2]) * h->fused_first_pct + 99) / 100;
            if (zs > hi[2]) zs = hi[2];
            if (hi[0] <= lo[0] || hi[1] <= lo[1]) zs = lo[2];
            {
                const int boxes[7][6] = {{lo[0], hi[0], lo[1], hi[1], lo[2], zs},
                                         {0, nt[0], 0, nt[1], zs, nt[2]},
                                         {0, nt[0], 0, nt[1], 0, lo[2]},
                                         {0, nt[0], 0, lo[1], lo[2], zs}, {0, nt[0], hi[1], nt[1], lo[2], zs},
                                         {0, lo[0], lo[1], hi[1], lo[2], zs}, {hi[0], nt[0], lo[1], hi[1], lo[2], zs}};
                const int band[7] = {1, 1, 1, 0, 0, 0, 0};
                int tot = 0;
                for (int q = 0; q < 7; q++) {
                    const int *b = boxes[q];
                    const bool empty = b[1] <= b[0] || b[3] <= b[2] || b[5] <= b[4];
                    if (empty && q > 0) continue;
                    for (int c = 0; c < 6; c++) sh.box[sh.nbox][c] = empty ? 0 : b[c];
                    if (empty) { sh.box[sh.nbox][1] = sh.box[sh.nbox][3] = sh.box[sh.nbox][5] = 1; }
                    sh.banded[sh.nbox] = band[q];
                    sh.start[sh.nbox] = tot;
                    tot += empty ? 0 : (b[1] - b[0]) * (b[3] - b[2]) * (b[5] - b[4]);
                    sh.nbox++;
                }
                sh.start[sh.nbox] = tot;
                if (tot != nt[0] * nt[1] * nt[2]) return jrx_fail(h, JRX_ERR_ARG, "internal: the tile classes of the fused kernel do not cover the block (%d of %d)", tot, nt[0] * nt[1] * nt[2]);
            }
            FusedBC bn = bc;
            bn.nbL = nbf[0][0]; bn.nbR = nbf[0][1]; bn.nbF = nbf[1][0]; bn.nbBk = nbf[1][1]; bn.nbK0 = nbf[2][0]; bn.nbK1 = nbf[2][1];
            if (bn.nbL) bn.fsL = bn.nsL = 0;
            if (bn.nbR) bn.fsR = bn.nsR = 0;
            if (bn.nbF) bn.fsF = bn.nsF = 0;
            if (bn.nbBk) bn.fsBk = bn.nsBk = 0;
            if (bn.nbK0) bn.fsK0 = bn.nsK0 = 0;
            if (bn.nbK1) bn.fsK1 = bn.nsK1 = 0;
            const int all[6] = {0, nt[0], 0, nt[1], 0, nt[2]};
            sh.blk0 = 0; sh.cls = 0;
            JRX_TRY(launch_fused(h, s, a, bn, all, false, true, &sh));
            JRX_HIP(h, hipStreamWaitEvent(s, h->ev[2], 0));
            sh.blk0 = sh.start[1]; sh.cls = 1;
            JRX_TRY(launch_fused(h, s, a, bn, all, false, true, &sh));
            if (tev) JRX_HIP(h, hipEventRecord(tev[3], s));
            bs = s;
            if (cev) { JRX_HIP(h, hipEventRecord(cev[3], s)); if (chain_mode) *chain_mode = 2; }
            I.ghosts_stale = true;
            folded = true;
        } else if (early) {
            bs = h->halo_stream;
            JRX_HIP(h, hipEventRecord(h->ev[0], s));
            JRX_HIP(h, hipStreamWaitEvent(bs, h->ev[0], 0));
            {
                const int w = 4;
                const int xa = imin(w, nx / 2), ya = imin(w, ny / 2), za = imin(w, nz / 2);
                const bool L0 = jrx_comm_has_neighbor(h, 0, 0), H0 = jrx_comm_has_neighbor(h, 0, 1), L1 = jrx_comm_has_neighbor(h, 1, 0), H1 = jrx_comm_has_neighbor(h, 1, 1),
                           L2 = jrx_comm_has_neighbor(h, 2, 0), H2 = jrx_comm_has_neighbor(h, 2, 1);
                const int z0 = L2 ? za : 0, z1 = H2 ? nz - za : nz, y0 = L1 ? ya : 0, y1 = H1 ? ny - ya : ny;
                if (L2) JRX_TRY(launch_velocity(h, bs, a, false, 0, nx, 0, ny, 0, za));
                if (H2) JRX_TRY(launch_velocity(h, bs, a, false, 0, nx, 0, ny, nz - za, nz));
                if (L1) JRX_TRY(launch_velocity(h, bs, a, false, 0, nx, 0, ya, z0, z1));
                if (H1) JRX_TRY(launch_velocity(h, bs, a, false, 0, nx, ny - ya, ny, z0, z1));
                if (L0) JRX_TRY(launch_velocity(h, bs, a, false, 0, xa, y0, y1, z0, z1));
                if (H0) JRX_TRY(launch_velocity(h, bs, a, false, nx - xa, nx, y0, y1, z0, z1));
            }
            if (cev) JRX_HIP(h, hipEventRecord(cev[0], bs));
            const bool lazy = h->comm_bcs_lazy;
            if (!lazy) JRX_TRY(fused_bcs(bs));
            if (cev) JRX_HIP(h, hipEventRecord(cev[1], bs));
            {
                double *arrs[3] = {dst.Vx, dst.Vy, dst.Vz};
                const int64_t ext[3][3] = {{nx + 1, ny + 2, nz + 2}, {nx + 2, ny + 1, nz + 2}, {nx + 2, ny + 2, nz + 1}};
                const int64_t n[3] = {nx, ny, nz};
                JRX_TRY(jrx_halo_exchange(h, bs, 3, arrs, ext, n));
            }
            if (cev) JRX_HIP(h, hipEventRecord(cev[2], bs));
            const int all[6] = {0, nt[0], 0, nt[1], 0, nt[2]};
            JRX_TRY(launch_fused(h, s, a, bc, all));
            if (tev) JRX_HIP(h, hipEventRecord(tev[3], s));
            JRX_HIP(h, hipEventRecord(h->ev[2], bs));
            JRX_HIP(h, hipStreamWaitEvent(s, h->ev[2], 0));
            bs = s;
            if (lazy) { I.ghosts_stale = true; rules_with_comm = true; }
            else {
                uint32_t fs_keep, ns_keep;
                physical_faces(h, &fs_keep, &ns_keep);
                JRX_TRY(launch_bcs_faces(h, s, dst.Vx, dst.Vy, dst.Vz, nx, ny, nz, p->free_slip & fs_keep, p->no_slip & ns_keep));
            }
            if (cev) { JRX_HIP(h, hipEventRecord(cev[3], s)); if (chain_mode) *chain_mode = 2; }
            for (int d = 0; d < 3; d++) { nb[d][0] = jrx_comm_has_neighbor(h, d, 0); nb[d][1] = jrx_comm_has_neighbor(h, d, 1); }
        } else if (!comm || !overlap) {
            const int all[6] = {0, nt[0], 0, nt[1], 0, nt[2]};
            folded = !comm && !per && fused_folds_hiface(h, a);
            JRX_TRY(launch_fused(h, s, a, bc, all, false, folded));
            if (tev) JRX_HIP(h, hipEventRecord(tev[3], s));
            if (per || (comm && !h->comm_bcs_lazy)) JRX_TRY(fused_bcs(s));
            else { I.ghosts_stale = true; rules_with_comm = comm; }
            if (cev && comm) JRX_HIP(h, hipEventRecord(cev[1], s));
            if (per) {
                const uint32_t lo[3] = {JRX_FACE_LEFT, JRX_FACE_FRONT, JRX_FACE_BOT}, hi[3] = {JRX_FACE_RIGHT, JRX_FACE_BACK, JRX_FACE_TOP};
                for (int d = 0; d < 3; d++) { nb[d][0] = (p->periodic & lo[d]) != 0; nb[d][1] = (p->periodic & hi[d]) != 0; }
            }
            if (comm) {
                double *arrs[3] = {dst.Vx, dst.Vy, dst.Vz};
                const int64_t ext[3][3] = {{nx + 1, ny + 2, nz + 2}, {nx + 2, ny + 1, nz + 2}, {nx + 2, ny + 2, nz + 1}};
                const int64_t n[3] = {nx, ny, nz};
                JRX_TRY(jrx_halo_exchange(h, s, 3, arrs, ext, n));
                for (int d = 0; d < 3; d++) { nb[d][0] |= jrx_comm_has_neighbor(h, d, 0); nb[d][1] |= jrx_comm_has_neighbor(h, d, 1); }
                if (cev) { JRX_HIP(h, hipEventRecord(cev[2], s)); if (chain_mode) *chain_mode = 1; }
            }
        } else {
            bs = h->halo_stream;
            JRX_HIP(h, hipEventRecord(h->ev[0], s));
            JRX_HIP(h, hipStreamWaitEvent(bs, h->ev[0], 0));
            int lo[3][2], mid[3][2], hi[3][2];
            for (int d = 0; d < 3; d++) {
                lo[d][0] = 0; lo[d][1] = 1;
                hi[d][0] = nt[d] > 1 ? nt[d] - 1 : 1; hi[d][1] = nt[d];
                mid[d][0] = 1; mid[d][1] = hi[d][0];
            }
            const int boxes[6][6] = {{0, nt[0], 0, nt[1], lo[2][0], lo[2][1]},  {0, nt[0], 0, nt[1], hi[2][0], hi[2][1]},
                                     {0, nt[0], lo[1][0], lo[1][1], mid[2][0], mid[2][1]}, {0, nt[0], hi[1][0], hi[1][1], mid[2][0], mid[2][1]},
                                     {lo[0][0], lo[0][1], mid[1][0], mid[1][1], mid[2][0], mid[2][1]}, {hi[0][0], hi[0][1], mid[1][0], mid[1][1], mid[2][0], mid[2][1]}};
            for (int q = 0; q < 6; q++) JRX_TRY(launch_fused(h, bs, a, bc, boxes[q]));
            const int inner[6] = {mid[0][0], mid[0][1], mid[1][0], mid[1][1], mid[2][0], mid[2][1]};
            JRX_TRY(launch_fused(h, s, a, bc, inner));
            JRX_TRY(fused_bcs(bs));
            double *arrs[3] = {dst.Vx, dst.Vy, dst.Vz};
            const int64_t ext[3][3] = {{nx + 1, ny + 2, nz + 2}, {nx + 2, ny + 1, nz + 2}, {nx + 2, ny + 2, nz + 1}};
            const int64_t n[3] = {nx, ny, nz};
            JRX_TRY(jrx_halo_exchange(h, bs, 3, arrs, ext, n));
            for (int d = 0; d < 3; d++) { nb[d][0] = jrx_comm_has_neighbor(h, d, 0); nb[d][1] = jrx_comm_has_neighbor(h, d, 1); }
            if (per) {
                const uint32_t lo[3] = {JRX_FACE_LEFT, JRX_FACE_FRONT, JRX_FACE_BOT}, hi[3] = {JRX_FACE_RIGHT, JRX_FACE_BACK, JRX_FACE_TOP};
                for (int d = 0; d < 3; d++) { nb[d][0] |= (p->periodic & lo[d]) != 0; nb[d][1] |= (p->periodic & hi[d]) != 0; }
            }
        }
        SweepArgs e = a;
        e.f.Vx = dst.Vx; e.f.Vy = dst.Vy; e.f.Vz = dst.Vz;
        const int ilo = nb[0][0] ? 1 : 0, ihi = nb[0][1] ? nx - 1 : nx, jlo = nb[1][0] ? 1 : 0, jhi = nb[1][1] ? ny - 1 : ny,
                  klo = nb[2][0] ? 1 : 0, khi = nb[2][1] ? nz - 1 : nz;
        const int fix[6][6] = {{0, ilo, 0, ny + 1, 0, nz + 1}, {ihi, nx + 1, 0, ny + 1, 0, nz + 1}, {ilo, ihi, 0, jlo, 0, nz + 1},
                               {ilo, ihi, jhi, ny + 1, 0, nz + 1}, {ilo, ihi, jlo, jhi, 0, klo}, {ilo, ihi, jlo, jhi, khi, nz + 1}};
        GhostRule gr;
        {
            auto ty = [&](uint32_t fsbit, uint32_t nsbit) { return (p->no_slip & nsbit) ? 2 : ((p->free_slip & fsbit) ? 1 : 0); };
            const int t6[6] = {ty(JRX_FACE_LEFT, JRX_FACE_LEFT), ty(JRX_FACE_RIGHT, JRX_FACE_RIGHT), ty(JRX_FACE_FRONT, JRX_FACE_FRONT),
                               ty(JRX_FACE_BACK, JRX_FACE_BACK), ty(JRX_FACE_TOP, JRX_FACE_BOT), ty(JRX_FACE_BOT, JRX_FACE_TOP)};
            for (int q = 0; q < 6; q++) gr.t[q] = t6[q];
            if (rules_with_comm)
                for (int d = 0; d < 3; d++) { if (nb[d][0]) gr.t[2 * d] = 0; if (nb[d][1]) gr.t[2 * d + 1] = 0; }
        }
        if (!folded) JRX_TRY(launch_stress_boxes(h, bs, e, fix, 6, false, ((comm || per) && !rules_with_comm) ? nullptr : &gr));
        if (bs != s) {
            JRX_HIP(h, hipEventRecord(h->ev[2], bs));
            JRX_HIP(h, hipStreamWaitEvent(s, h->ev[2], 0));
            if (tev && !split) JRX_HIP(h, hipEventRecord(tev[3], s));
        }
        set_state(I.cur, dst);
        I.pt_user = !I.pt_user; I.v_user = !I.v_user;
        I.stress_done = true;
        if (was_fused) *was_fused = 1;
        if (tev) JRX_HIP(h, hipEventRecord(tev[2], s));
        return JRX_OK;
    }

    const jrx_stokes3d_fields *f = &I.cur;
    if (!jrx_comm_active(h)) {
        if (I.ghosts_stale && diag) {
            JRX_TRY(launch_bcs(h, s, f->Vx, f->Vy, f->Vz, nx, ny, nz, p->free_slip, p->no_slip, p->periodic));
            I.bcs_ordered[I.v_user ? 0 : 1] = true;
        }
        I.ghosts_stale = false;
        if (I.flip_B && !p->displacement_bcs) {
            const Out10 other = mix_sets(I.pt_user ? I.setU : I.setS, I.v_user ? I.setS : I.setU);
            a.o = other;
            JRX_TRY(launch_velocity(h, s, a, diag, 0, nx, 0, ny, 0, nz, h->nof));
            set_state(I.cur, other);
            I.v_user = !I.v_user;
        } else
            JRX_TRY(launch_velocity(h, s, a, diag, 0, nx, 0, ny, 0, nz, h->nof));
        I.flip_B = false;
        if (tev) JRX_HIP(h, hipEventRecord(tev[2], s));
        if (diag) JRX_TRY(launch_scaleU(h, s, f, p));
        if (p->displacement_bcs) {
            if (diag) JRX_TRY(launch_bcs(h, s, f->Ux, f->Uy, f->Uz, nx, ny, nz, p->free_slip, p->no_slip, p->periodic));
            return JRX_OK;
        }
        bool &ordered = I.bcs_ordered[I.v_user ? 0 : 1];
        if (!diag && ordered && p->periodic == 0) JRX_TRY(launch_bcs_faces(h, s, f->Vx, f->Vy, f->Vz, nx, ny, nz, p->free_slip, p->no_slip));
        else {
            JRX_TRY(launch_bcs(h, s, f->Vx, f->Vy, f->Vz, nx, ny, nz, p->free_slip, p->no_slip, p->periodic));
            ordered = true;
        }
        return JRX_OK;
    }
    if (I.ghosts_stale) {
        uint32_t fs_keep, ns_keep;
        physical_faces(h, &fs_keep, &ns_keep);
        JRX_TRY(launch_bcs(h, s, f->Vx, f->Vy, f->Vz, nx, ny, nz, p->free_slip & fs_keep, p->no_slip & ns_keep, 0));
        I.ghosts_stale = false;
    }
    return jrx3d_velocity_hidden(h, f, I.etatau, p, diag, p->displacement_bcs ? (diag ? 2 : 3) : 0);
}

static jrx_status iter_end(Iter3D &I)
{
    jrx_handle *h = I.h;
    if (I.stress_done) return jrx_fail(h, JRX_ERR_ARG, "internal: iteration pipeline ended with a pending fused stress sweep");
    if (I.all_user()) return JRX_OK;
    const jrx_stokes3d_params *p = I.p;
    const i64 nc = (i64)p->nx * p->ny * p->nz, nyz = (i64)p->nx * (p->ny + 1) * (p->nz + 1), nxz = (i64)(p->nx + 1) * p->ny * (p->nz + 1),
              nxy = (i64)(p->nx + 1) * (p->ny + 1) * p->nz, n0 = (i64)(p->nx + 1) * (p->ny + 2) * (p->nz + 2),
              n1 = (i64)(p->nx + 2) * (p->ny + 1) * (p->nz + 2), n2 = (i64)(p->nx + 2) * (p->ny + 2) * (p->nz + 1);
    const Out10 &S = I.setS, &U = I.setU;
    const i64 zp = I.pt_user ? 0 : 1, zv = I.v_user ? 0 : 1;
    if (zp) {
        hipLaunchKernelGGL(k_copy6, dim3(2048), dim3(256), 0, h->stream, U.P, (const double *)S.P, nc, U.txx, (const double *)S.txx, nc, U.tyy,
                           (const double *)S.tyy, nc, U.tzz, (const double *)S.tzz, nc, U.tyz, (const double *)S.tyz, nyz, U.txz, (const double *)S.txz, nxz);
        JRX_LAUNCH_CHECK(h);
    }
    hipLaunchKernelGGL(k_copy6, dim3(2048), dim3(256), 0, h->stream, U.txy, (const double *)S.txy, nxy * zp, U.Vx, (const double *)S.Vx, n0 * zv, U.Vy,
                       (const double *)S.Vy, n1 * zv, U.Vz, (const double *)S.Vz, n2 * zv, (double *)nullptr, (const double *)nullptr, (i64)0, (double *)nullptr,
                       (const double *)nullptr, (i64)0);
    JRX_LAUNCH_CHECK(h);
    set_state(I.cur, U);
    I.pt_user = I.v_user = true;
    return JRX_OK;
}

extern "C" {

jrx_status jrx_stokes3d_solve(jrx_handle *h, const jrx_stokes3d_fields *f, const jrx_stokes3d_params *p, jrx_solve_result *res)
{
    JRX_TRY(check_params(h, f, p));
    JRX_TRY(check_diag(h, f));
    if (!res) return jrx_fail(h, JRX_ERR_ARG, "null result");
    if (p->nout < 1) return jrx_fail(h, JRX_ERR_ARG, "nout must be >= 1");
    const int nx = (int)p->nx, ny = (int)p->ny, nz = (int)p->nz;
    const size_t n = (size_t)nx * ny * nz;
    hipStream_t s = h->stream;

    JRX_TRY(jrx_ensure_etatau(h, n));
    hipLaunchKernelGGL(k_maxloc, dim3((unsigned)(((i64)nx * ny + 255) / 256), (unsigned)nz), dim3(256), 0, s, h->etatau, f->eta, nx, ny, nz);
    JRX_LAUNCH_CHECK(h);
    if (jrx_comm_active(h)) {
        double *arrs[1] = {h->etatau};
        const int64_t ext[1][3] = {{nx, ny, nz}};
        const int64_t nn[3] = {nx, ny, nz};
        JRX_TRY(jrx_halo_exchange(h, s, 1, arrs, ext, nn));
    }

    if (p->displacement_bcs) {
        hipLaunchKernelGGL(k_scale3, dim3(2048), dim3(256), 0, s, f->Vx, (const double *)f->Ux, (i64)(nx + 1) * (ny + 2) * (nz + 2), f->Vy,
                           (const double *)f->Uy, (i64)(nx + 2) * (ny + 1) * (nz + 2), f->Vz, (const double *)f->Uz, (i64)(nx + 2) * (ny + 2) * (nz + 1),
                           1.0 / p->dt);
        JRX_LAUNCH_CHECK(h);
    }
    double err_it1 = 1.0, err = 1.0;
    int64_t iter = 0, cont = 0;
    res->iter = 0; res->nchecks = 0;
    const int rank = jrx_comm_rank(h);
    hipEvent_t t0 = h->ev[6], t1 = h->ev[7];
    Iter3D I;
    JRX_TRY(iter_begin(I, h, f, h->etatau, p));
    JRX_HIP(h, hipEventRecord(t0, s));
    auto keep_going = [&](int64_t it) { return it < 2 || (((err / err_it1) > p->eps_rel && err > p->eps_abs) && it <= p->iterMax); };
    auto is_check = [&](int64_t it1) { return (it1 % p->nout == 0) && it1 > 1; };
    constexpr int GIT = 16;
    GraphExecs gexec;
    bool graphs = h->loop_graphs && !I.fusable && !jrx_comm_active(h) && !p->displacement_bcs && p->periodic == 0 && (double)n <= kGraphCells3D;
    while (keep_going(iter)) {
        if (graphs && iter >= 2 && I.bcs_ordered[0] && I.all_user() && !I.stress_done) {
            int64_t nxt = ((iter / p->nout) + 1) * p->nout;
            if (nxt > p->iterMax + 1) nxt = p->iterMax + 1;
            int64_t run = nxt - 1 - iter;
            if (run >= GIT) {
                if (!gexec[0]) {
                    JRX_TRY(jrx_capture_graph(s, &gexec[0], [&]() -> jrx_status {
                        for (int q = 0; q < GIT; q++) JRX_TRY(iter_step(I, false, false, nullptr, nullptr));
                        return JRX_OK;
                    }));
                    if (!gexec[0]) graphs = false;
                }
                if (gexec[0]) {
                    while (run >= GIT) {
                        JRX_HIP(h, hipGraphLaunch(gexec[0], s));
                        iter += GIT; run -= GIT;
                        h->stat_graph_replays++;
                    }
                    continue;
                }
            }
        }
        const int64_t it1 = iter + 1;
        const bool check = is_check(it1);
        const bool diag = check || !keep_going(it1);
        const bool fuse_next = !diag && keep_going(it1) && !(is_check(it1 + 1) || !keep_going(it1 + 1));
        JRX_TRY(iter_step(I, diag, fuse_next, nullptr, nullptr));
        iter = it1;
        if (check) {
            JRX_TRY(launch_sumsq(h, s, &I.cur, p));
            JRX_HIP(h, hipMemcpyAsync(h->h_sums, h->d_sums, 4 * sizeof(double), hipMemcpyDeviceToHost, s));
            JRX_HIP(h, hipStreamSynchronize(s));
            double ss[4] = {h->h_sums[0], h->h_sums[1], h->h_sums[2], h->h_sums[3]};
            JRX_TRY(jrx_allreduce_sum_host(h, ss, 4));
            const double nRx = sqrt(ss[0]) / (double)((p->nxg - 2) * (p->nyg - 1) * (p->nzg - 1));
            const double nRy = sqrt(ss[1]) / (double)((p->nxg - 1) * (p->nyg - 2) * (p->nzg - 1));
            const double nRz = sqrt(ss[2]) / (double)((p->nxg - 1) * (p->nyg - 1) * (p->nzg - 2));
            const double nDV = sqrt(ss[3]) / (double)(p->nxg * p->nyg * p->nzg);
            err = fmax(fmax(nRx, nRy), fmax(nRz, nDV));
            if (std::isnan(nRx) || std::isnan(nRy) || std::isnan(nRz) || std::isnan(nDV)) err = NAN;
            if (cont < res->cap) {
                if (res->norm_Rx) res->norm_Rx[cont] = nRx;
                if (res->norm_Ry) res->norm_Ry[cont] = nRy;
                if (res->norm_Rz) res->norm_Rz[cont] = nRz;
                if (res->norm_divV) res->norm_divV[cont] = nDV;
                if (res->err_evo1) res->err_evo1[cont] = err;
                if (res->err_evo2) res->err_evo2[cont] = iter;
            }
            if (cont == 0) err_it1 = err;
            cont++;
            if (rank == 0 && ((p->verbose && (err / err_it1) > p->eps_rel && err > p->eps_abs) || iter == p->iterMax))
                printf("iter = %lld, abs_err = %1.3e, rel_err = %1.3e [norm_Rx=%1.3e, norm_Ry=%1.3e, norm_Rz=%1.3e, norm_∇V=%1.3e] \n",
                       (long long)iter, err, err / err_it1, nRx, nRy, nRz, nDV);
            if (std::isnan(err)) {
                res->iter = iter; res->nchecks = cont < res->cap ? cont : res->cap;
                (void)iter_end(I);
                (void)hipStreamSynchronize(s);
                return jrx_fail(h, JRX_ERR_NAN, "NaN(s)");
            }
        }
    }
    JRX_HIP(h, hipEventRecord(t1, s));
    JRX_TRY(iter_end(I));
    h->opv.valid = false;
    const i64 nc = (i64)n, nyz = (i64)nx * (ny + 1) * (nz + 1), nxz = (i64)(nx + 1) * ny * (nz + 1), nxy = (i64)(nx + 1) * (ny + 1) * nz;
    hipLaunchKernelGGL(k_copy6, dim3(2048), dim3(256), 0, s, f->toxx, (const double *)f->txx, nc, f->toyy, (const double *)f->tyy, nc, f->tozz,
                       (const double *)f->tzz, nc, f->toyz, (const double *)f->tyz, nyz, f->toxz, (const double *)f->txz, nxz, f->toxy,
                       (const double *)f->txy, nxy);
    JRX_LAUNCH_CHECK(h);
    if (f->tyz_c && f->toyz_c && f->txz_c && f->toxz_c && f->txy_c && f->toxy_c) {
        hipLaunchKernelGGL(k_copy6, dim3(2048), dim3(256), 0, s, f->toyz_c, (const double *)f->tyz_c, nc, f->toxz_c, (const double *)f->txz_c, nc,
                           f->toxy_c, (const double *)f->txy_c, nc, (double *)nullptr, (const double *)nullptr, (i64)0, (double *)nullptr,
                           (const double *)nullptr, (i64)0, (double *)nullptr, (const double *)nullptr, (i64)0);
        JRX_LAUNCH_CHECK(h);
    }
    JRX_HIP(h, hipStreamSynchronize(s));
    float ms = 0.f;
    JRX_HIP(h, hipEventElapsedTime(&ms, t0, t1));
    res->iter = iter;
    res->nchecks = cont < res->cap ? cont : res->cap;
    res->time_s = ms * 1e-3;
    res->av_time_s = iter > 1 ? res->time_s / (double)(iter - 1) : res->time_s;
    return JRX_OK;
}

jrx_status jrx_stokes3d_iterate_timed(jrx_handle *h, const jrx_stokes3d_fields *f, const double *etatau,
                                      const jrx_stokes3d_params *p, int64_t iters, double times_ms[6])
{
    JRX_TRY(check_params(h, f, p));
    if (!etatau) return jrx_fail(h, JRX_ERR_ARG, "etatau is NULL");
    if (iters < 1) return jrx_fail(h, JRX_ERR_ARG, "iters must be >= 1");
    if (!times_ms) return jrx_fail(h, JRX_ERR_ARG, "times_ms is NULL");
    hipStream_t s = h->stream;
    const int64_t stride = iters > 64 ? (((iters + 63) / 64) | 1) : 1;
    const int nsamp = (int)((iters + stride - 1) / stride);
    const bool chain = h->chain_profile && jrx_comm_active(h);
    std::vector<hipEvent_t> evs((size_t)nsamp * (chain ? 8 : 4));
    std::vector<int> fused((size_t)nsamp, 0), cmode((size_t)nsamp, 0);
    std::vector<double> ncell((size_t)nsamp, 0.0);
    struct EvGuard { std::vector<hipEvent_t> &v; ~EvGuard() { for (auto &e : v) if (e) (void)hipEventDestroy(e); } } guard{evs};
    for (auto &e : evs) e = nullptr;
    for (auto &e : evs) JRX_HIP(h, hipEventCreate(&e));
    Iter3D I;
    JRX_TRY(iter_begin(I, h, f, etatau, p));
    JRX_HIP(h, hipStreamSynchronize(s));
    JRX_HIP(h, hipEventRecord(h->ev[6], s));
    const bool odd = I.fusable && iters >= 2 && ((iters - 1) % 2 == 1);
    const bool flips = odd && h->end_flips && !jrx_comm_active(h) && p->periodic == 0 && !p->displacement_bcs;
    const bool first_unfused = odd && !flips;
    for (int64_t it = 0; it < iters; it++) {
        const bool samp = it % stride == 0;
        const bool fuse_next = it + 1 < iters && !(first_unfused && it == 0);
        if (flips && it == 0) I.flip_A = true;
        if (flips && it == iters - 1) I.flip_B = true;
        const size_t q = (size_t)(it / stride);
        JRX_TRY(iter_step(I, false, fuse_next, samp ? &evs[q * 4] : nullptr, samp ? &fused[q] : nullptr, samp ? &ncell[q] : nullptr,
                          samp && chain ? &evs[(size_t)nsamp * 4 + q * 4] : nullptr, samp && chain ? &cmode[q] : nullptr));
    }
    JRX_HIP(h, hipEventRecord(h->ev[7], s));
    JRX_TRY(iter_end(I));
    JRX_HIP(h, hipStreamSynchronize(s));
    float ms = 0.f;
    JRX_HIP(h, hipEventElapsedTime(&ms, h->ev[6], h->ev[7]));
    times_ms[0] = ms; times_ms[1] = times_ms[2] = times_ms[3] = times_ms[4] = times_ms[5] = 0.0;
    double sa = 0.0, sb = 0.0, sf = 0.0, sk = 0.0, sc = 0.0;
    int na = 0, nb = 0, nf = 0;
    const bool comm = jrx_comm_active(h);
    for (int q = 0; q < nsamp; q++) {
        if (comm && !fused[q]) continue;
        float m1 = 0.f, m2 = 0.f;
        JRX_HIP(h, hipEventElapsedTime(&m1, evs[(size_t)q * 4], evs[(size_t)q * 4 + 1]));
        JRX_HIP(h, hipEventElapsedTime(&m2, evs[(size_t)q * 4 + 1], evs[(size_t)q * 4 + 2]));
        if (fused[q]) {
            float m3 = 0.f;
            JRX_HIP(h, hipEventElapsedTime(&m3, evs[(size_t)q * 4 + 1], evs[(size_t)q * 4 + 3]));
            sf += m2; sk += m3; sc += ncell[q]; nf++;
        }
        else { sb += m2; nb++; }
        if (m1 > 1e-3f) { sa += m1; na++; }
    }
    if (chain) {
        double acc[8] = {0, 0, 0, 0, 0, 0, 0, 0};
        int nc = 0;
        auto el = [&](hipEvent_t a, hipEvent_t b) { float m = 0.f; (void)hipEventElapsedTime(&m, a, b); return (double)m * 1e3; };
        for (int q = 0; q < nsamp; q++) {
            if (!fused[q] || !cmode[q]) continue;
            hipEvent_t *t = &evs[(size_t)q * 4], *c = &evs[(size_t)nsamp * 4 + (size_t)q * 4];
            const double step = el(t[1], t[2]), kern = el(t[1], t[3]);
            if (cmode[q] == 2) {
                const double post = fmin(el(t[3], c[3]), el(c[2], c[3]));
                acc[0] += kern; acc[1] += el(t[1], c[0]); acc[2] += el(c[0], c[1]); acc[3] += el(c[1], c[2]); acc[4] += post; acc[5] += el(c[3], t[2]);
            } else {
                acc[0] += kern; acc[2] += el(t[3], c[1]); acc[3] += el(c[1], c[2]); acc[5] += el(c[2], t[2]);
            }
            acc[6] += step; acc[7] += step - kern;
            nc++;
        }
        for (int q = 0; q < 8; q++) h->chain_us[q] = nc ? acc[q] / nc : 0.0;
        h->chain_n = nc;
        (void)hipGetLastError();
    }
    if (na) times_ms[1] = sa / na;
    if (nb) times_ms[2] = sb / nb;
    if (nf) { times_ms[3] = sf / nf; times_ms[4] = sk / nf; times_ms[5] = sc / nf; }
    return JRX_OK;
}

}
```

justrelax.jl_amd/csrc/stokes3d_kernels.hpp:

```cpp
#pragma once
#include "jrx_internal.hpp"

namespace {

struct Dims3 {
    int nx, ny, nz;
};

struct Lay3 {
    int nx, ny, nz;
    int vx1, vy1, vz1;
    i64 vxp, vyp, vzp;
    i64 cp;
    int xy1; i64 xyp;
    int xz1; i64 xzp;
    int yz1; i64 yzp;
};

__host__ __device__ inline Lay3 make_lay(int nx, int ny, int nz)
{
    Lay3 L;
    L.nx = nx; L.ny = ny; L.nz = nz;
    L.vx1 = nx + 1; L.vxp = (i64)(nx + 1) * (ny + 2);
    L.vy1 = nx + 2; L.vyp = (i64)(nx + 2) * (ny + 1);
// ... 28 lines not shown
{
    if ((i == 0 && g.t[0] == 2) || (i == L.nx && g.t[1] == 2)) return 0.0;
    double sgn = 1.0;
    ghost_tan(j, sgn, L.ny, g.t[2], g.t[3]); ghost_tan(k, sgn, L.nz, g.t[4], g.t[5]);
    return sgn * Vx[i + (i64)L.vx1 * j + L.vxp * k];
}
__device__ __forceinline__ double vy_rule(const double *__restrict__ Vy, const Lay3 &L, const GhostRule &g, int i, int j, int k)
{
    if ((j == 0 && g.t[2] == 2) || (j == L.ny && g.t[3] == 2)) return 0.0;
    double sgn = 1.0;
    ghost_tan(i, sgn, L.nx, g.t[0], g.t[1]); ghost_tan(k, sgn, L.nz, g.t[4], g.t[5]);
    return sgn * Vy[i + (i64)L.vy1 * j + L.vyp * k];
}
__device__ __forceinline__ double vz_rule(const double *__restrict__ Vz, const Lay3 &L, const GhostRule &g, int i, int j, int k)
{
    if ((k == 0 && g.t[4] == 2) || (k == L.nz && g.t[5] == 2)) return 0.0;
    double sgn = 1.0;
    ghost_tan(i, sgn, L.nx, g.t[0], g.t[1]); ghost_tan(j, sgn, L.ny, g.t[2], g.t[3]);
    return sgn * Vz[i + (i64)L.vz1 * j + L.vzp * k];
}

template <bool DIAG, bool GH = false, bool VISC = false>
__device__ __forceinline__ void stress3d_node(const SweepArgs &a, const int i, const int j, const int k, const GhostRule *gr = nullptr)
{
    const Lay3 &L = a.L;
    const int nx = L.nx, ny = L.ny, nz = L.nz;

    const double *__restrict__ Vx = a.f.Vx, *__restrict__ Vy = a.f.Vy, *__restrict__ Vz = a.f.Vz;
    const double *__restrict__ eta = a.f.eta, *__restrict__ G = a.f.G;
    const double _dx = a._dx, _dy = a._dy, _dz = a._dz, dt = a.dt, th = a.theta_dtau;

#define VX(i_, j_, k_) (GH ? vx_rule(Vx, L, *gr, (i_), (j_), (k_)) : Vx[(i_) + (i64)L.vx1 * (j_) + L.vxp * (k_)])
#define VY(i_, j_, k_) (GH ? vy_rule(Vy, L, *gr, (i_), (j_), (k_)) : Vy[(i_) + (i64)L.vy1 * (j_) + L.vyp * (k_)])
#define VZ(i_, j_, k_) (GH ? vz_rule(Vz, L, *gr, (i_), (j_), (k_)) : Vz[(i_) + (i64)L.vz1 * (j_) + L.vzp * (k_)])
#define CC(i_, j_, k_) ((i_) + (i64)nx * (j_) + L.cp * (k_))

    const bool ci = i < nx, cj = j < ny, ck = k < nz;

    if (ci && cj && ck) {
        const i64 c = CC(i, j, k);
        const double dxi = (-VX(i, j + 1, k + 1) + VX(i + 1, j + 1, k + 1)) * _dx;
        const double dyi = (-VY(i + 1, j, k + 1) + VY(i + 1, j + 1, k + 1)) * _dy;
        const double dzi = (-VZ(i + 1, j + 1, k) + VZ(i + 1, j + 1, k + 1)) * _dz;
        const double divV = dxi + dyi + dzi;
        const double e = eta[c];
        const double _Gdt = VISC ? 0.0 : 1.0 / (G[c] * dt);
        {
            const double _Kdt = VISC ? 0.0 : 1.0 / (a.f.K[c] * dt);
            const double _dt = 1.0 / dt;
            const double P = a.f.P[c], P0 = VISC ? 0.0 : a.f.P0[c];
            const double rhs = -divV + ((VISC ? 0.0 : a.f.Q[c]) * _dt);
            const double psi = 1.0 / (1.0 / e + _Gdt) * a.r / th;
            a.o.P[c] = (fma(P0, _Kdt, rhs) * psi + P) / (1.0 + _Kdt * psi);
            if (DIAG) {
                a.f.RP[c] = fma(-(P - P0), _Kdt, rhs);
                a.f.divV[c] = divV;
            }
        }
        const double d3 = divV * (1.0 / 3.0);
        const double exx = dxi - d3, eyy = dyi - d3, ezz = dzi - d3;
        if (DIAG) { a.f.exx[c] = exx; a.f.eyy[c] = eyy; a.f.ezz[c] = ezz; }
        const double dtr = dev_dtau_r(th, e, _Gdt);
        double tv;
        tv = a.f.txx[c]; a.o.txx[c] = tv + dev_stress_inc(tv, (VISC ? 0.0 : a.f.toxx[c]), e, exx, _Gdt, dtr);
        tv = a.f.tyy[c]; a.o.tyy[c] = tv + dev_stress_inc(tv, (VISC ? 0.0 : a.f.toyy[c]), e, eyy, _Gdt, dtr);
        tv = a.f.tzz[c]; a.o.tzz[c] = tv + dev_stress_inc(tv, (VISC ? 0.0 : a.f.tozz[c]), e, ezz, _Gdt, dtr);
    }

    const int im = max(i - 1, 0), ip = min(i, nx - 1);
    const int jm = max(j - 1, 0), jp = min(j, ny - 1);
    const int km = max(k - 1, 0), kp = min(k, nz - 1);

    if (ck) {
        const double exy = 0.5 * (_dy * (VX(i, j + 1, k + 1) - VX(i, j, k + 1)) + _dx * (VY(i + 1, j, k + 1) - VY(i, j, k + 1)));
        const double e = 0.25 * (eta[CC(im, jm, k)] + eta[CC(ip, jm, k)] + eta[CC(im, jp, k)] + eta[CC(ip, jp, k)]);
        const double _Gdt = VISC ? 0.0 : 1.0 / (0.25 * (G[CC(im, jm, k)] + G[CC(ip, jm, k)] + G[CC(im, jp, k)] + G[CC(ip, jp, k)]) * dt);
        const double dtr = dev_dtau_r(th, e, _Gdt);
        const i64 c = i + (i64)L.xy1 * j + L.xyp * k;
        const double tv = a.f.txy[c];
        a.o.txy[c] = tv + dev_stress_inc(tv, (VISC ? 0.0 : a.f.toxy[c]), e, exy, _Gdt, dtr);
        if (DIAG) a.f.exy[c] = exy;
    }
    if (cj) {
        const double exz = 0.5 * (_dz * (VX(i, j + 1, k + 1) - VX(i, j + 1, k)) + _dx * (VZ(i + 1, j + 1, k) - VZ(i, j + 1, k)));
        const double e = 0.25 * (eta[CC(im, j, km)] + eta[CC(ip, j, km)] + eta[CC(im, j, kp)] + eta[CC(ip, j, kp)]);
        const double _Gdt = VISC ? 0.0 : 1.0 / (0.25 * (G[CC(im, j, km)] + G[CC(ip, j, km)] + G[CC(im, j, kp)] + G[CC(ip, j, kp)]) * dt);
        const double dtr = dev_dtau_r(th, e, _Gdt);
        const i64 c = i + (i64)L.xz1 * j + L.xzp * k;
        const double tv = a.f.txz[c];
        a.o.txz[c] = tv + dev_stress_inc(tv, (VISC ? 0.0 : a.f.toxz[c]), e, exz, _Gdt, dtr);
        if (DIAG) a.f.exz[c] = exz;
    }
    if (ci) {
        const double eyz = 0.5 * (_dz * (VY(i + 1, j, k + 1) - VY(i + 1, j, k)) + _dy * (VZ(i + 1, j + 1, k) - VZ(i + 1, j, k)));
        const double e = 0.25 * (eta[CC(i, jm, km)] + eta[CC(i, jp, km)] + eta[CC(i, jm, kp)] + eta[CC(i, jp, kp)]);
        const double _Gdt = VISC ? 0.0 : 1.0 / (0.25 * (G[CC(i, jm, km)] + G[CC(i, jp, km)] + G[CC(i, jm, kp)] + G[CC(i, jp, kp)]) * dt);
        const double dtr = dev_dtau_r(th, e, _Gdt);
        const i64 c = i + (i64)L.yz1 * j + L.yzp * k;
        const double tv = a.f.tyz[c];
        a.o.tyz[c] = tv + dev_stress_inc(tv, (VISC ? 0.0 : a.f.toyz[c]), e, eyz, _Gdt, dtr);
        if (DIAG) a.f.eyz[c] = eyz;
    }
#undef VX
#undef VY
#undef VZ
}

template <bool DIAG>
__global__ __launch_bounds__(256) void k_stress3d(const SweepArgs a)
{
    const int wi = a.i1 - a.i0;
    const int t = blockIdx.x * blockDim.x + threadIdx.x;
    const int jj = t / wi;
    const int j = a.j0 + jj;
    if (j >= a.j1) return;
    stress3d_node<DIAG>(a, a.i0 + (t - jj * wi), j, a.k0 + (int)blockIdx.y);
}

struct StressBoxes {
    int n;
    int box[6][6];
    int start[7];
    int per_plane[6];
};
template <bool DIAG, bool GH = false, bool VISC = false>
__global__ __launch_bounds__(256) void k_stress3d_boxes(const SweepArgs a, const StressBoxes B, const GhostRule gr)
{
    int b = 0;
    while (b + 1 < B.n && (int)blockIdx.x >= B.start[b + 1]) b++;
    const int lb = (int)blockIdx.x - B.start[b];
    const int kz = lb / B.per_plane[b], bx = lb - kz * B.per_plane[b];
    const int wi = B.box[b][1] - B.box[b][0];
    const int t = bx * 256 + (int)threadIdx.x;
    const int jj = t / wi;
    const int j = B.box[b][2] + jj;
    if (j >= B.box[b][3]) return;
    stress3d_node<DIAG, GH, VISC>(a, B.box[b][0] + (t - jj * wi), j, B.box[b][4] + kz, &gr);
}

template <bool DIAG>
__global__ __launch_bounds__(256) void k_velocity3d(const SweepArgs a)
{
    const Lay3 &L = a.L;
    const int nx = L.nx, ny = L.ny, nz = L.nz;
    const int wi = a.i1 - a.i0;
    const int t = blockIdx.x * blockDim.x + threadIdx.x;
    const int jj = t / wi;
    const int i = a.i0 + (t - jj * wi);
    const int j = a.j0 + jj;
    const int k = a.k0 + blockIdx.y;
    if (j >= a.j1) return;

    const double _dx = a._dx, _dy = a._dy, _dz = a._dz, edt = a.eta_dtau;
    const double *__restrict__ P = a.f.P, *__restrict__ et = a.etatau;
    const double *__restrict__ txy = a.f.txy, *__restrict__ txz = a.f.txz, *__restrict__ tyz = a.f.tyz;
#define TXY(i_, j_, k_) txy[(i_) + (i64)L.xy1 * (j_) + L.xyp * (k_)]
#define TXZ(i_, j_, k_) txz[(i_) + (i64)L.xz1 * (j_) + L.xzp * (k_)]
#define TYZ(i_, j_, k_) tyz[(i_) + (i64)L.yz1 * (j_) + L.yzp * (k_)]
    const i64 c = CC(i, j, k);
    const double Pc = P[c], ec = et[c];

    if (i < nx - 1) {
        const i64 cx = c + 1;
        const double R = (-a.f.txx[c] + a.f.txx[cx]) * _dx + _dy * (TXY(i + 1, j + 1, k) - TXY(i + 1, j, k)) +
                         _dz * (TXZ(i + 1, j, k + 1) - TXZ(i + 1, j, k)) - (-Pc + P[cx]) * _dx -
                         0.5 * (a.f.fx[c] + a.f.fx[cx]);
        const i64 v = (i + 1) + (i64)L.vx1 * (j + 1) + L.vxp * (k + 1);
        a.o.Vx[v] = a.f.Vx[v] + R * edt / (0.5 * (ec + et[cx]));
        if (DIAG) a.f.Rx[i + (i64)(nx - 1) * j + (i64)(nx - 1) * ny * k] = R;
    }
    if (j < ny - 1) {
        const i64 cy = c + nx;
        const double R = _dx * (TXY(i + 1, j + 1, k) - TXY(i, j + 1, k)) + _dy * (a.f.tyy[cy] - a.f.tyy[c]) +
                         _dz * (TYZ(i, j + 1, k + 1) - TYZ(i, j + 1, k)) - (-Pc + P[cy]) * _dy -
                         0.5 * (a.f.fy[c] + a.f.fy[cy]);
        const i64 v = (i + 1) + (i64)L.vy1 * (j + 1) + L.vyp * (k + 1);
        a.o.Vy[v] = a.f.Vy[v] + R * edt / (0.5 * (ec + et[cy]));
        if (DIAG) a.f.Ry[i + (i64)nx * j + (i64)nx * (ny - 1) * k] = R;
    }
    if (k < nz - 1) {
        const i64 cz = c + L.cp;
        const double R = _dx * (TXZ(i + 1, j, k + 1) - TXZ(i, j, k + 1)) + _dy * (TYZ(i, j + 1, k + 1) - TYZ(i, j, k + 1)) +
                         (-a.f.tzz[c] + a.f.tzz[cz]) * _dz - (-Pc + P[cz]) * _dz - 0.5 * (a.f.fz[c] + a.f.fz[cz]);
        const i64 v = (i + 1) + (i64)L.vz1 * (j + 1) + L.vzp * (k + 1);
        a.o.Vz[v] = a.f.Vz[v] + R * edt / (0.5 * (ec + et[cz]));
        if (DIAG) a.f.Rz[c] = R;
    }
#undef TXY
#undef TXZ
#undef TYZ
#undef CC
}


#define CC3(i_, j_, k_) ((i_) + (i64)nx * (j_) + L.cp * (k_))

template <bool DIAG>
__device__ __forceinline__ void node_xy(const SweepArgs &a, int I, int J, int k)
{
    const Lay3 &L = a.L;
    const int nx = L.nx, ny = L.ny;
    const double *Vx = a.f.Vx, *Vy = a.f.Vy, *eta = a.f.eta, *G = a.f.G;
    const int im = max(I - 1, 0), ip = min(I, nx - 1), jm = max(J - 1, 0), jp = min(J, ny - 1);
    const double exy = 0.5 * (a._dy * (Vx[I + (i64)L.vx1 * (J + 1) + L.vxp * (k + 1)] - Vx[I + (i64)L.vx1 * J + L.vxp * (k + 1)]) +
                              a._dx * (Vy[(I + 1) + (i64)L.vy1 * J + L.vyp * (k + 1)] - Vy[I + (i64)L.vy1 * J + L.vyp * (k + 1)]));
    const double e = 0.25 * (eta[CC3(im, jm, k)] + eta[CC3(ip, jm, k)] + eta[CC3(im, jp, k)] + eta[CC3(ip, jp, k)]);
    const double g = 0.25 * (G[CC3(im, jm, k)] + G[CC3(ip, jm, k)] + G[CC3(im, jp, k)] + G[CC3(ip, jp, k)]);
    const double _Gdt = 1.0 / (g * a.dt);
    const double dtr = dev_dtau_r(a.theta_dtau, e, _Gdt);
    const i64 c = I + (i64)L.xy1 * J + L.xyp * k;
    const double tv = a.f.txy[c];
    a.o.txy[c] = tv + dev_stress_inc(tv, a.f.toxy[c], e, exy, _Gdt, dtr);
    if (DIAG) a.f.exy[c] = exy;
}
template <bool DIAG>
__device__ __forceinline__ void node_xz(const SweepArgs &a, int I, int j, int Kk)
{
    const Lay3 &L = a.L;
    const int nx = L.nx, nz = L.nz;
    const double *Vx = a.f.Vx, *Vz = a.f.Vz, *eta = a.f.eta, *G = a.f.G;
    const int im = max(I - 1, 0), ip = min(I, nx - 1), km = max(Kk - 1, 0), kp = min(Kk, nz - 1);
    const double exz = 0.5 * (a._dz * (Vx[I + (i64)L.vx1 * (j + 1) + L.vxp * (Kk + 1)] - Vx[I + (i64)L.vx1 * (j + 1) + L.vxp * Kk]) +
                              a._dx * (Vz[(I + 1) + (i64)L.vz1 * (j + 1) + L.vzp * Kk] - Vz[I + (i64)L.vz1 * (j + 1) + L.vzp * Kk]));
    const double e = 0.25 * (eta[CC3(im, j, km)] + eta[CC3(ip, j, km)] + eta[CC3(im, j, kp)] + eta[CC3(ip, j, kp)]);
    const double g = 0.25 * (G[CC3(im, j, km)] + G[CC3(ip, j, km)] + G[CC3(im, j, kp)] + G[CC3(ip, j, kp)]);
    const double _Gdt = 1.0 / (g * a.dt);
    const double dtr = dev_dtau_r(a.theta_dtau, e, _Gdt);
    const i64 c = I + (i64)L.xz1 * j + L.xzp * Kk;
    const double tv = a.f.txz[c];
    a.o.txz[c] = tv + dev_stress_inc(tv, a.f.toxz[c], e, exz, _Gdt, dtr);
    if (DIAG) a.f.exz[c] = exz;
}
template <bool DIAG>
__device__ __forceinline__ void node_yz(const SweepArgs &a, int i, int J, int Kk)
{
    const Lay3 &L = a.L;
    const int nx = L.nx, ny = L.ny, nz = L.nz;
    const double *Vy = a.f.Vy, *Vz = a.f.Vz, *eta = a.f.eta, *G = a.f.G;
    const int jm = max(J - 1, 0), jp = min(J, ny - 1), km = max(Kk - 1, 0), kp = min(Kk, nz - 1);
    const double eyz = 0.5 * (a._dz * (Vy[(i + 1) + (i64)L.vy1 * J + L.vyp * (Kk + 1)] - Vy[(i + 1) + (i64)L.vy1 * J + L.vyp * Kk]) +
                              a._dy * (Vz[(i + 1) + (i64)L.vz1 * (J + 1) + L.vzp * Kk] - Vz[(i + 1) + (i64)L.vz1 * J + L.vzp * Kk]));
    const double e = 0.25 * (eta[CC3(i, jm, km)] + eta[CC3(i, jp, km)] + eta[CC3(i, jm, kp)] + eta[CC3(i, jp, kp)]);
    const double g = 0.25 * (G[CC3(i, jm, km)] + G[CC3(i, jp, km)] + G[CC3(i, jm, kp)] + G[CC3(i, jp, kp)]);
    const double _Gdt = 1.0 / (g * a.dt);
    const double dtr = dev_dtau_r(a.theta_dtau, e, _Gdt);
    const i64 c = i + (i64)L.yz1 * J + L.yzp * Kk;
    const double tv = a.f.tyz[c];
    a.o.tyz[c] = tv + dev_stress_inc(tv, a.f.toyz[c], e, eyz, _Gdt, dtr);
    if (DIAG) a.f.eyz[c] = eyz;
}


typedef unsigned int u32;
#define LDB(p, off) (*(const double *)((const char *)(p) + (off)))
#define STB(p, off, v) (*(double *)((char *)(p) + (off)) = (v))
template <bool NT> __device__ __forceinline__ double LDN(const double *p, u32 off)
{
    const double *q = (const double *)((const char *)p + off);
    return NT ? __builtin_nontemporal_load(q) : *q;
}
template <bool NT> __device__ __forceinline__ void STN(double *p, u32 off, double v)
{
    double *q = (double *)((char *)p + off);
    if (NT) __builtin_nontemporal_store(v, q);
    else *q = v;
}

struct TileMap {
    int ntx, nty, ntz, ntiles, per;
};
__host__ __device__ inline TileMap make_tilemap(int ex, int ey, int ez, int TX, int TY, int KZ)
{
    TileMap m;
    m.ntx = (ex + TX - 1) / TX; m.nty = (ey + TY - 1) / TY; m.ntz = (ez + KZ - 1) / KZ;
    m.ntiles = m.ntx * m.nty * m.ntz;
    m.per = (m.ntiles + 7) / 8;
    return m;
}
template <int XM>
__device__ __forceinline__ bool tile_of_block(const TileMap &m, int &tx, int &ty, int &tz)
{
    const int b = blockIdx.x;
    if (XM >= 2) {
        const int per_z = m.ntx * m.nty;
        if (m.nty % (8 * XM) == 0) {
            tz = b / per_z;
            const int bz = b - tz * per_z;
            const int q = bz & 7, r = bz >> 3;
            tx = r % m.ntx;
            const int r2 = r / m.ntx;
            ty = (r2 / XM) * (8 * XM) + q * XM + (r2 % XM);
            return b < m.ntiles;
        }
    }
    const int lb = XM == 1 ? (b & 7) * m.per + (b >> 3) : b;
    if (lb >= m.ntiles) return false;
    tx = lb % m.ntx;
    const int r = lb / m.ntx;
    ty = r % m.nty;
    tz = r / m.nty;
    return true;
}

template <bool DIAG, int TX, int TY, int KZ, int MINW, bool EDGES, int XCD = 0, bool SHF = false, bool VISC = false>
__global__ __launch_bounds__(TX *TY, MINW) void k_stress3d_zb(const SweepArgs a, const TileMap tm)
{
    static_assert(!SHF || (TX % 64 == 0 && !EDGES), "SHF needs whole waves per row");
    static_assert(!VISC || (!DIAG && !EDGES), "the viscous-limit form is the state-only sweep over the interior tiles");
    const Lay3 &L = a.L;
    const int nx = L.nx, ny = L.ny, nz = L.nz;
    int tx, ty, tz;
    if (!tile_of_block<XCD>(tm, tx, ty, tz)) return;
    const int i = tx * TX + (int)(threadIdx.x % TX);
    const int j = ty * TY + (int)(threadIdx.x / TX);
    const int kb = tz * KZ;
    if (i >= nx || j >= ny) return;
    const int kend = min(kb + KZ, nz);
    const int im = max(i - 1, 0), jm = max(j - 1, 0);
    const bool xhi = (i == nx - 1), yhi = (j == ny - 1);
    const double _dx = a._dx, _dy = a._dy, _dz = a._dz, dt = a.dt, th = a.theta_dtau, _dt = 1.0 / dt, rr = a.r;
    const jrx_stokes3d_fields &f = a.f;

    const u32 sc = (u32)L.cp * 8u, svx = (u32)L.vxp * 8u, svy = (u32)L.vyp * 8u, svz = (u32)L.vzp * 8u;
    const u32 sxy = (u32)L.xyp * 8u, sxz = (u32)L.xzp * 8u, syz = (u32)L.yzp * 8u;
    const u32 rvx = (u32)L.vx1 * 8u, rvy = (u32)L.vy1 * 8u, rvz = (u32)L.vz1 * 8u;
    u32 oc = 8u * (u32)(i + nx * j) + sc * (u32)kb;
    const u32 dcx = 8u * (u32)(i - im), dcy = 8u * (u32)(nx * (j - jm));
    u32 ovx = 8u * (u32)(i + L.vx1 * (j + 1)) + svx * (u32)(kb + 1);
    u32 ovy = 8u * (u32)((i + 1) + L.vy1 * j) + svy * (u32)(kb + 1);
    u32 ovz = 8u * (u32)((i + 1) + L.vz1 * (j + 1)) + svz * (u32)(kb + 1);
    u32 oxy = 8u * (u32)(i + L.xy1 * j) + sxy * (u32)kb;
    u32 oxz = 8u * (u32)(i + L.xz1 * j) + sxz * (u32)kb;
    u32 oyz = 8u * (u32)(i + L.yz1 * j) + syz * (u32)kb;

    double a_p = LDB(f.Vx, ovx - svx), b_p = LDB(f.Vy, ovy - svy);
    double c_p = LDB(f.Vz, ovz - svz), cx_p = LDB(f.Vz, ovz - svz - 8u), cy_p = LDB(f.Vz, ovz - svz - rvz);
    const u32 back = kb > 0 ? sc : 0u;
    double e_p = LDB(f.eta, oc - back), ex_p = LDB(f.eta, oc - back - dcx), ey_p = LDB(f.eta, oc - back - dcy);
    double g_p = 1.0, gx_p = 1.0, gy_p = 1.0;
    if (!VISC) { g_p = LDB(f.G, oc - back); gx_p = LDB(f.G, oc - back - dcx); gy_p = LDB(f.G, oc - back - dcy); }

    for (int k = kb; k < kend; ++k) {
        const double va = LDB(f.Vx, ovx), vay = LDB(f.Vx, ovx - rvx);
        const double vb = LDB(f.Vy, ovy), vby = LDB(f.Vy, ovy + rvy);
        const double vc = LDB(f.Vz, ovz), vcy = LDB(f.Vz, ovz - rvz);
        const double e = LDB(f.eta, oc), ey = LDB(f.eta, oc - dcy);
        const double g = VISC ? 1.0 : LDB(f.G, oc), gy = VISC ? 1.0 : LDB(f.G, oc - dcy);
        double vax, vbx, vcx, ex, exy_, gx = 1.0, gxy = 1.0;
        if (SHF) {
            const int lane = (int)(threadIdx.x & 63);
            vax = __shfl_down(va, 1, 64);
            vbx = __shfl_up(vb, 1, 64); vcx = __shfl_up(vc, 1, 64);
            ex = __shfl_up(e, 1, 64); exy_ = __shfl_up(ey, 1, 64);
            if (!VISC) { gx = __shfl_up(g, 1, 64); gxy = __shfl_up(gy, 1, 64); }
            if (lane == 63 || xhi) vax = LDB(f.Vx, ovx + 8u);
            if (lane == 0) {
                vbx = LDB(f.Vy, ovy - 8u); vcx = LDB(f.Vz, ovz - 8u);
                ex = LDB(f.eta, oc - dcx); exy_ = LDB(f.eta, oc - dcx - dcy);
                if (!VISC) { gx = LDB(f.G, oc - dcx); gxy = LDB(f.G, oc - dcx - dcy); }
            }
        } else {
            vax = LDB(f.Vx, ovx + 8u); vbx = LDB(f.Vy, ovy - 8u); vcx = LDB(f.Vz, ovz - 8u);
            ex = LDB(f.eta, oc - dcx); exy_ = LDB(f.eta, oc - dcx - dcy);
            if (!VISC) { gx = LDB(f.G, oc - dcx); gxy = LDB(f.G, oc - dcx - dcy); }
        }
        const double P = LDB(f.P, oc), P0 = VISC ? 0.0 : LDB(f.P0, oc), Kc = VISC ? 1.0 : LDB(f.K, oc), Qc = VISC ? 0.0 : LDB(f.Q, oc);
        const double txx = LDB(f.txx, oc), tyy = LDB(f.tyy, oc), tzz = LDB(f.tzz, oc);
        const double toxx = VISC ? 0.0 : LDB(f.toxx, oc), toyy = VISC ? 0.0 : LDB(f.toyy, oc), tozz = VISC ? 0.0 : LDB(f.tozz, oc);
        const double txy = LDB(f.txy, oxy), toxy = VISC ? 0.0 : LDB(f.toxy, oxy);
        const double txz = LDB(f.txz, oxz), toxz = VISC ? 0.0 : LDB(f.toxz, oxz);
        const double tyz = LDB(f.tyz, oyz), toyz = VISC ? 0.0 : LDB(f.toyz, oyz);

        {
            const double dxi = (-va + vax) * _dx;
            const double dyi = (-vb + vby) * _dy;
            const double dzi = (-c_p + vc) * _dz;
            const double divV = dxi + dyi + dzi;
            const double _Gdt = VISC ? 0.0 : 1.0 / (g * dt);
            const double _Kdt = VISC ? 0.0 : 1.0 / (Kc * dt);
            const double rhs = -divV + (Qc * _dt);
            const double psi = 1.0 / (1.0 / e + _Gdt) * rr / th;
            STB(a.o.P, oc, (fma(P0, _Kdt, rhs) * psi + P) / (1.0 + _Kdt * psi));
            const double d3 = divV * (1.0 / 3.0);
            const double exx = dxi - d3, eyy = dyi - d3, ezz = dzi - d3;
            if (DIAG) {
                STB(f.RP, oc, fma(-(P - P0), _Kdt, rhs));
                STB(f.divV, oc, divV);
                STB(f.exx, oc, exx); STB(f.eyy, oc, eyy); STB(f.ezz, oc, ezz);
            }
            const double dtr = dev_dtau_r(th, e, _Gdt);
            STB(a.o.txx, oc, txx + dev_stress_inc(txx, toxx, e, exx, _Gdt, dtr));
            STB(a.o.tyy, oc, tyy + dev_stress_inc(tyy, toyy, e, eyy, _Gdt, dtr));
            STB(a.o.tzz, oc, tzz + dev_stress_inc(tzz, tozz, e, ezz, _Gdt, dtr));
        }
        {
            const double s_ = 0.5 * (_dy * (va - vay) + _dx * (vb - vbx));
            const double ee = 0.25 * (exy_ + ey + ex + e);
            const double gg = 0.25 * (gxy + gy + gx + g);
            const double _Gdt = VISC ? 0.0 : 1.0 / (gg * dt);
            const double dtr = dev_dtau_r(th, ee, _Gdt);
            STB(a.o.txy, oxy, txy + dev_stress_inc(txy, toxy, ee, s_, _Gdt, dtr));
            if (DIAG) STB(f.exy, oxy, s_);
        }
        {
            const double s_ = 0.5 * (_dz * (va - a_p) + _dx * (c_p - cx_p));
            const double ee = 0.25 * (ex_p + e_p + ex + e);
            const double gg = 0.25 * (gx_p + g_p + gx + g);
            const double _Gdt = VISC ? 0.0 : 1.0 / (gg * dt);
            const double dtr = dev_dtau_r(th, ee, _Gdt);
            STB(a.o.txz, oxz, txz + dev_stress_inc(txz, toxz, ee, s_, _Gdt, dtr));
            if (DIAG) STB(f.exz, oxz, s_);
        }
        {
            const double s_ = 0.5 * (_dz * (vb - b_p) + _dy * (c_p - cy_p));
            const double ee = 0.25 * (ey_p + e_p + ey + e);
            const double gg = 0.25 * (gy_p + g_p + gy + g);
            const double _Gdt = VISC ? 0.0 : 1.0 / (gg * dt);
            const double dtr = dev_dtau_r(th, ee, _Gdt);
            STB(a.o.tyz, oyz, tyz + dev_stress_inc(tyz, toyz, ee, s_, _Gdt, dtr));
            if (DIAG) STB(f.eyz, oyz, s_);
        }
        if (EDGES) {
            if (xhi) { node_xy<DIAG>(a, nx, j, k); node_xz<DIAG>(a, nx, j, k); }
            if (yhi) { node_xy<DIAG>(a, i, ny, k); node_yz<DIAG>(a, i, ny, k); }
            if (xhi && yhi) node_xy<DIAG>(a, nx, ny, k);
        }

        a_p = va; b_p = vb; c_p = vc; cx_p = vcx; cy_p = vcy;
        e_p = e; ex_p = ex; ey_p = ey; g_p = g; gx_p = gx; gy_p = gy;
        oc += sc; ovx += svx; ovy += svy; ovz += svz; oxy += sxy; oxz += sxz; oyz += syz;
    }
    if (EDGES && kend == nz) {
        node_xz<DIAG>(a, i, j, nz);
        node_yz<DIAG>(a, i, j, nz);
        if (xhi) node_xz<DIAG>(a, nx, j, nz);
        if (yhi) node_yz<DIAG>(a, i, ny, nz);
    }
}

template <bool DIAG, int TX, int TY, int KZ, int MINW, int XCD = 0, bool SHF = false, int NOF = 0>
__global__ __launch_bounds__(TX *TY, MINW) void k_velocity3d_zb(const SweepArgs a, const TileMap tm)
{
    static_assert(!SHF || TX % 64 == 0, "SHF needs whole waves per row");
    const Lay3 &L = a.L;
    const int nx = L.nx, ny = L.ny, nz = L.nz;
    int tx, ty, tz;
    if (!tile_of_block<XCD>(tm, tx, ty, tz)) return;
    const int i = a.i0 + tx * TX + (int)(threadIdx.x % TX);
    const int j = a.j0 + ty * TY + (int)(threadIdx.x / TX);
    const int kb = a.k0 + tz * KZ;
    if (i >= a.i1 || j >= a.j1) return;
    const int kend = min(kb + KZ, a.k1);
    const double _dx = a._dx, _dy = a._dy, _dz = a._dz, edt = a.eta_dtau;
    const bool hx = i < nx - 1, hy = j < ny - 1;
    const jrx_stokes3d_fields &f = a.f;
    const double *et = a.etatau;

    const u32 sc = (u32)L.cp * 8u, svx = (u32)L.vxp * 8u, svy = (u32)L.vyp * 8u, svz = (u32)L.vzp * 8u;
    const u32 sxy = (u32)L.xyp * 8u, sxz = (u32)L.xzp * 8u, syz = (u32)L.yzp * 8u;
    const u32 rc = (u32)nx * 8u, rxy = (u32)L.xy1 * 8u, ryz = (u32)L.yz1 * 8u;
    const u32 srx = (u32)(nx - 1) * (u32)ny * 8u, sry = (u32)nx * (u32)(ny - 1) * 8u;
    u32 oc = 8u * (u32)(i + nx * j) + sc * (u32)kb;
    u32 oxy = 8u * (u32)(i + L.xy1 * j) + sxy * (u32)kb;
    u32 oxz = 8u * (u32)(i + L.xz1 * j) + sxz * (u32)(kb + 1);
    u32 oyz = 8u * (u32)(i + L.yz1 * j) + syz * (u32)(kb + 1);
    u32 ovx = 8u * (u32)((i + 1) + L.vx1 * (j + 1)) + svx * (u32)(kb + 1);
    u32 ovy = 8u * (u32)((i + 1) + L.vy1 * (j + 1)) + svy * (u32)(kb + 1);
    u32 ovz = 8u * (u32)((i + 1) + L.vz1 * (j + 1)) + svz * (u32)(kb + 1);
    u32 orx = 8u * (u32)(i + (nx - 1) * j) + srx * (u32)kb;
    u32 ory = 8u * (u32)(i + nx * j) + sry * (u32)kb;
    const u32 dx1 = hx ? 8u : 0u, dy1 = hy ? rc : 0u;

    double Pc = LDB(f.P, oc), ec = LDB(et, oc), tzz_c = LDB(f.tzz, oc), fz_c = NOF >= 2 ? 0.0 : LDB(f.fz, oc);
    double s10 = LDB(f.txz, oxz + 8u - sxz), r10 = LDB(f.tyz, oyz + ryz - syz);

    for (int k = kb; k < kend; ++k) {
        const bool hz = k < nz - 1;
        const u32 dz1 = hz ? sc : 0u;
        const double q10 = LDB(f.txy, oxy + 8u), q01 = LDB(f.txy, oxy + rxy);
        const double s01 = LDB(f.txz, oxz);
        const double r11 = LDB(f.tyz, oyz + ryz), r01 = LDB(f.tyz, oyz);
        const double Pz = LDB(f.P, oc + dz1), ez = LDB(et, oc + dz1), tzz_z = LDB(f.tzz, oc + dz1), fz_z = NOF >= 2 ? 0.0 : LDB(f.fz, oc + dz1);
        const double Py = LDB(f.P, oc + dy1), ey = LDB(et, oc + dy1);
        const double txx_c = LDB(f.txx, oc), tyy_c = LDB(f.tyy, oc), tyy_y = LDB(f.tyy, oc + dy1);
        const double fx_c = NOF >= 1 ? 0.0 : LDB(f.fx, oc), fy_c = NOF >= 1 ? 0.0 : LDB(f.fy, oc), fy_y = NOF >= 1 ? 0.0 : LDB(f.fy, oc + dy1);
        const double vx = LDB(f.Vx, ovx), vy = LDB(f.Vy, ovy), vz = LDB(f.Vz, ovz);
        double q11, s11, Px, ex, txx_x, fx_x;
        if (SHF) {
            q11 = __shfl_down(q01, 1, 64); s11 = __shfl_down(s01, 1, 64);
            Px = __shfl_down(Pc, 1, 64); ex = __shfl_down(ec, 1, 64); txx_x = __shfl_down(txx_c, 1, 64); fx_x = NOF >= 1 ? 0.0 : __shfl_down(fx_c, 1, 64);
            if ((threadIdx.x & 63) == 63 || i == a.i1 - 1) {
                q11 = LDB(f.txy, oxy + 8u + rxy); s11 = LDB(f.txz, oxz + 8u);
                Px = LDB(f.P, oc + dx1); ex = LDB(et, oc + dx1); txx_x = LDB(f.txx, oc + dx1); fx_x = NOF >= 1 ? 0.0 : LDB(f.fx, oc + dx1);
            }
        } else {
            q11 = LDB(f.txy, oxy + 8u + rxy); s11 = LDB(f.txz, oxz + 8u);
            Px = LDB(f.P, oc + dx1); ex = LDB(et, oc + dx1); txx_x = LDB(f.txx, oc + dx1); fx_x = NOF >= 1 ? 0.0 : LDB(f.fx, oc + dx1);
        }
        if (hx) {
            const double R0 = (-txx_c + txx_x) * _dx + _dy * (q11 - q10) + _dz * (s11 - s10) - (-Pc + Px) * _dx;
            const double R = NOF >= 1 ? R0 : R0 - 0.5 * (fx_c + fx_x);
            STB(a.o.Vx, ovx, vx + R * edt / (0.5 * (ec + ex)));
            if (DIAG) STB(f.Rx, orx, R);
        }
        if (hy) {
            const double R0 = _dx * (q11 - q01) + _dy * (tyy_y - tyy_c) + _dz * (r11 - r10) - (-Pc + Py) * _dy;
            const double R = NOF >= 1 ? R0 : R0 - 0.5 * (fy_c + fy_y);
            STB(a.o.Vy, ovy, vy + R * edt / (0.5 * (ec + ey)));
            if (DIAG) STB(f.Ry, ory, R);
        }
        if (hz) {
            const double R0 = _dx * (s11 - s01) + _dy * (r11 - r01) + (-tzz_c + tzz_z) * _dz - (-Pc + Pz) * _dz;
            const double R = NOF >= 2 ? R0 : R0 - 0.5 * (fz_c + fz_z);
            STB(a.o.Vz, ovz, vz + R * edt / (0.5 * (ec + ez)));
            if (DIAG) STB(f.Rz, oc, R);
        }
        Pc = Pz; ec = ez; tzz_c = tzz_z; fz_c = fz_z; s10 = s11; r10 = r11;
        oc += sc; oxy += sxy; oxz += sxz; oyz += syz; ovx += svx; ovy += svy; ovz += svz; orx += srx; ory += sry;
    }
}

struct FusedBC {
    int fsL, nsL, fsF, nsF, fsK0, nsK0, nsR, nsBk, nsK1, fsR, fsBk, fsK1;
    int nbL, nbR, nbF, nbBk, nbK0, nbK1;
    int feed;
};
struct FusedShell {
    int nbox, box[7][6], start[8], banded[7];
    int blk0, cls;
};
__device__ __forceinline__ double LDC(const double *p, u32 off)
{
    const unsigned long long v = __hip_atomic_load((const unsigned long long *)((const char *)p + off), __ATOMIC_RELAXED, __HIP_MEMORY_SCOPE_AGENT);
    return __longlong_as_double((long long)v);
}

template <int TX, int TY, int KZ, int MINW, int OVX = 1, bool LOWREG = false, int XG = 0, bool LATEA = false, bool SHFL = false, int YLDS = 0, int NT = 0, int TAG = 0, bool VISC = false, bool HIF = false, bool VFOLD = false, bool NBR = false, int NOF = 0, int YM = 1>
__global__ __launch_bounds__(TX *TY, MINW) void k_fused3d(const SweepArgs a, const FusedBC bc, int ntx, int nty, int tx0 = 0, int ty0 = 0, int tz0 = 0, const FusedShell sh = FusedShell{})
{
    static_assert(!(SHFL && (LATEA || (TX != 64 && TX != 32))), "SHFL is implemented for rows of one wave or half a wave");
    static_assert(!YLDS || SHFL, "YLDS builds on the SHFL operand layout");
    static_assert(!VISC || YLDS, "the viscous-limit form is built on the YLDS operand layout");
    static_assert(!HIF || (!LOWREG && SHFL && OVX == 1 && YLDS == 3), "the folded high-face layers are built on the forms with carried planes");
    static_assert(!VFOLD || VISC, "VFOLD simplifies the viscous-limit arithmetic");
    static_assert(!NBR || HIF, "the in-kernel neighbour faces are built on the one-launch forms");
    static_assert(YM == 1 || (VISC && HIF && VFOLD && !NBR && !LOWREG && YLDS == 3), "the y march is built on the one-launch viscous-limit form");
    constexpr int NS = LOWREG ? 3 : 2;
    __shared__ double sT[YM > 1 ? KZ + 1 : 1][4][YM > 1 ? TX : 1];
    __shared__ double sV[NS][3][TY][TX];
    __shared__ double sY[YLDS ? (VISC ? 7 : 8) : 1][YLDS ? TY : 1][YLDS ? TX : 1];
    const Lay3 &L = a.L;
    const int nx = L.nx, ny = L.ny, nz = L.nz;
    const jrx_stokes3d_fields &f = a.f;
    const double *et = a.etatau;
#define NBV(flag_, arr_, off_) ((NBR && bc.flag_) ? LDC(a.o.arr_, (off_)) : LDB(f.arr_, (off_)))
#define NBVX(flag_, off_, ii_) ((NBR && bc.flag_) ? ((((ii_) == 0 && bc.nsL) || ((ii_) == nx && bc.nsR)) ? 0.0 : LDC(a.o.Vx, (off_))) : LDB(f.Vx, (off_)))
#define NBVY(flag_, off_, jj_) ((NBR && bc.flag_) ? ((((jj_) == 0 && bc.nsF) || ((jj_) == ny && bc.nsBk)) ? 0.0 : LDC(a.o.Vy, (off_))) : LDB(f.Vy, (off_)))
#define NBVZ(flag_, off_, kk_) ((NBR && bc.flag_) ? ((((kk_) == 0 && bc.nsK0) || ((kk_) == nz && bc.nsK1)) ? 0.0 : LDC(a.o.Vz, (off_))) : LDB(f.Vz, (off_)))
    static_assert(NOF == 0 || (VISC && HIF && VFOLD) || (!VISC && (LOWREG || HIF) && YLDS == 3), "the forms without body-force loads exist for the one-launch viscous-limit form and for the general forms");
#define LFX(off_) (NOF >= 1 ? 0.0 : LDN<(NT & 2) != 0>(f.fx, (off_)))
#define LFY(off_) (NOF >= 1 ? 0.0 : LDN<(NT & 2) != 0>(f.fy, (off_)))
#define LFZ(off_) (NOF >= 2 ? 0.0 : LDN<(NT & 2) != 0>(f.fz, (off_)))
    const int tx = (int)(threadIdx.x % TX), ty = (int)(threadIdx.x / TX);
    int tile = blockIdx.x;
    int tix, tiy, tiz;
    if (NBR) {
        tile += sh.blk0;
        int b = 0;
        while (b + 1 < sh.nbox && tile >= sh.start[b + 1]) b++;
        int l = tile - sh.start[b];
        const int bw = sh.box[b][1] - sh.box[b][0], bh = sh.box[b][3] - sh.box[b][2], bd = sh.box[b][5] - sh.box[b][4];
        if (XG > 0 && sh.banded[b]) {
            const int full = ((bh * bd) / (8 * XG)) * (8 * XG) * bw;
            if (l < full) {
                const int q = l & 7, r = l >> 3, r2 = r / bw;
                l = ((r2 / XG) * (8 * XG) + q * XG + r2 % XG) * bw + r % bw;
            }
        }
        tix = sh.box[b][0] + l % bw; tiy = sh.box[b][2] + (l / bw) % bh; tiz = sh.box[b][4] + l / (bw * bh);
    } else {
        const int ntyS = (nty + YM - 1) / YM;
        if (XG > 0) {
            const int full = ((ntyS * (int)(gridDim.x / (unsigned)(ntx * ntyS))) / (8 * XG)) * (8 * XG) * ntx;
            if (tile < full) {
                const int q = tile & 7, r = tile >> 3, r2 = r / ntx;
                tile = ((r2 / XG) * (8 * XG) + q * XG + r2 % XG) * ntx + r % ntx;
            }
        }
        const int tr = tile / ntx;
        tix = tx0 + tile % ntx; tiy = ty0 + (tr % ntyS) * YM; tiz = tz0 + tr / ntyS;
    }
    const int tiy_end = NBR ? tiy + 1 : min(tiy + YM, ty0 + nty);
    for (const int tiy_first = tiy; tiy < tiy_end; ++tiy) {
    const bool fed = YM > 1 && tiy > tiy_first && threadIdx.x < TX;
    const bool feeds = YM > 1 && tiy + 1 < tiy_end && (int)(threadIdx.x / TX) == TY - 1;
    const int i = tix * (TX - OVX - (SHFL ? 1 : 0)) - OVX + tx;
    const int j = tiy * (TY - 1) - 1 + ty;
    const int kb = tiz * KZ;
    const int kend = min(kb + KZ, nz);
    const bool bvalid = tx >= OVX - 1 && i >= 0 && j >= 0 && i < nx && j < ny;
    const bool avalid = bvalid && tx >= OVX && ty >= 1 && (!SHFL || tx < TX - 1);
    const bool feedL = NBR && SHFL && OVX == 1 && YLDS && !LOWREG && bc.feed && bc.nbL && tx == 0 && i == -1 && j >= 0 && j < ny;
    const bool hx = i < nx - 1, hy = j < ny - 1;
    const double _dx = a._dx, _dy = a._dy, _dz = a._dz, dt = a.dt, th = a.theta_dtau, _dt = 1.0 / dt, rr = a.r, edt = a.eta_dtau;
    const double dtr0 = VFOLD ? 1.0 / (th + 1.0) : 0.0;
    auto DTR = [&](const double eta_, const double Gdt_) { return VFOLD ? dtr0 : dev_dtau_r(th, eta_, Gdt_); };
    auto INC = [&](const double t_, const double to_, const double eta_, const double e_, const double Gdt_, const double dtr_) {
        return VFOLD ? dtr_ * fma(2.0 * eta_, e_, -t_) : dev_stress_inc(t_, to_, eta_, e_, Gdt_, dtr_);
    };

    const u32 sc = (u32)L.cp * 8u, svx = (u32)L.vxp * 8u, svy = (u32)L.vyp * 8u, svz = (u32)L.vzp * 8u;
    const u32 sxy = (u32)L.xyp * 8u, sxz = (u32)L.xzp * 8u, syz = (u32)L.yzp * 8u;
    const u32 rc = (u32)nx * 8u, rxy = (u32)L.xy1 * 8u, ryz = (u32)L.yz1 * 8u;
    const u32 rvx = (u32)L.vx1 * 8u, rvy = (u32)L.vy1 * 8u, rvz = (u32)L.vz1 * 8u;
    const int ic = bvalid ? i : (feedL ? -1 : 0), jc = (bvalid || feedL) ? j : 0;
    const int kfirst = kb > 0 ? kb - 1 : 0;
    u32 oc = 8u * (u32)(ic + nx * jc) + sc * (u32)kfirst;
    u32 oxy = 8u * (u32)(ic + L.xy1 * jc) + sxy * (u32)kfirst;
    u32 oxz = 8u * (u32)(ic + L.xz1 * jc) + sxz * (u32)(kfirst + 1);
    u32 oyz = 8u * (u32)(ic + L.yz1 * jc) + syz * (u32)(kfirst + 1);
    u32 ovx = 8u * (u32)((ic + 1) + L.vx1 * (jc + 1)) + svx * (u32)(kfirst + 1);
    u32 ovy = 8u * (u32)((ic + 1) + L.vy1 * (jc + 1)) + svy * (u32)(kfirst + 1);
    u32 ovz = 8u * (u32)((ic + 1) + L.vz1 * (jc + 1)) + svz * (u32)(kfirst + 1);
    const u32 dx1 = hx ? 8u : 0u, dy1 = hy ? rc : 0u;
    const int im = max(ic - 1, 0), jm = max(jc - 1, 0);
    const u32 dcx = 8u * (u32)(ic - im), dcy = rc * (u32)(jc - jm);

    double Pc = 0, ec = 0, tzz_c = 0, fz_c = 0, s10 = 0, r10 = 0, s01p = 0, r01p = 0;
    if (bvalid && !fed) {
        Pc = LDB(f.P, oc); ec = LDB(et, oc); tzz_c = LDB(f.tzz, oc); fz_c = LFZ(oc);
        s10 = LDB(f.txz, oxz + 8u - sxz); r10 = LDB(f.tyz, oyz + ryz - syz);
        s01p = LDB(f.txz, oxz - sxz); r01p = LDB(f.tyz, oyz - syz);
    }
    double a_p = 0, b_p = 0, c_p = 0, cx_p = 0, cy_p = 0, e_p = 0, ex_p = 0, ey_p = 0, g_p = 0, gx_p = 0, gy_p = 0;
    double exe_p = 0, eye_p = 0, gxg_p = 0, gyg_p = 0;
    double vax_p = 0, vby_p = 0;

    for (int k = kfirst; k < kend; ++k) {
        const bool hz = k < nz - 1;
        const bool live = k >= kb;
        const int slot = LOWREG ? k % 3 : (k & 1);
        double vxn = 0, vyn = 0, vzn = 0, txx_c = 0, tyy_c = 0, P_k = Pc, tzz_k = tzz_c, s01k = s01p, r01k = r01p;
        const double s10k = s10, r10k = r10;
        double e = 0, ex = 0, ey = 0, exy_ = 0, g = 0, gx = 0, gy = 0, gxy = 0, P0 = 0, Kc = 0, Qc = 0;
        double toxx = 0, toyy = 0, tozz = 0, txy = 0, toxy = 0, toxz = 0, toyz = 0;
        auto preload_stress = [&]() {
            if (SHFL) {
                if (YLDS) {
                    if (fed) e = sT[k - kfirst][3][tx];
                    else if (bvalid) { e = LDB(f.eta, oc); if (!VISC) g = LDB(f.G, oc); }
                } else if (bvalid) {
                    e = LDB(f.eta, oc); ey = LDB(f.eta, oc - dcy); g = LDB(f.G, oc); gy = LDB(f.G, oc - dcy);
                    const double e_l = __shfl_up(e, 1, TX), g_l = __shfl_up(g, 1, TX), ey_l = __shfl_up(ey, 1, TX), gy_l = __shfl_up(gy, 1, TX);
                    ex = i > 0 ? e_l : e; gx = i > 0 ? g_l : g; exy_ = i > 0 ? ey_l : ey; gxy = i > 0 ? gy_l : gy;
                }
                if (YLDS < 2 && !VISC && avalid && live) {
                    P0 = LDN<(NT & 2) != 0>(f.P0, oc); Kc = LDN<(NT & 2) != 0>(f.K, oc); Qc = LDN<(NT & 2) != 0>(f.Q, oc);
                    toxx = LDN<(NT & 2) != 0>(f.toxx, oc); toyy = LDN<(NT & 2) != 0>(f.toyy, oc); tozz = LDN<(NT & 2) != 0>(f.tozz, oc);
                    toxy = LDN<(NT & 2) != 0>(f.toxy, oxy);
                    toxz = LDN<(NT & 2) != 0>(f.toxz, oxz - sxz); toyz = LDN<(NT & 2) != 0>(f.toyz, oyz - syz);
                }
                return;
            }
            if (avalid) {
                e = LDB(f.eta, oc); ex = LDB(f.eta, oc - dcx); ey = LDB(f.eta, oc - dcy);
                g = LDB(f.G, oc); gx = LDB(f.G, oc - dcx); gy = LDB(f.G, oc - dcy);
                if (live) {
                    exy_ = LDB(f.eta, oc - dcx - dcy); gxy = LDB(f.G, oc - dcx - dcy);
                    P0 = LDN<(NT & 2) != 0>(f.P0, oc); Kc = LDN<(NT & 2) != 0>(f.K, oc); Qc = LDN<(NT & 2) != 0>(f.Q, oc);
                    toxx = LDN<(NT & 2) != 0>(f.toxx, oc); toyy = LDN<(NT & 2) != 0>(f.toyy, oc); tozz = LDN<(NT & 2) != 0>(f.tozz, oc);
                    txy = LDB(f.txy, oxy); toxy = LDN<(NT & 2) != 0>(f.toxy, oxy);
                    toxz = LDN<(NT & 2) != 0>(f.toxz, oxz - sxz); toyz = LDN<(NT & 2) != 0>(f.toyz, oyz - syz);
                }
            }
        };
        if (!LATEA) preload_stress();
        double q01 = 0, s01 = 0, r11 = 0, r01 = 0, Pz = 0, ez = 0, tzz_z = 0, fz_z = 0, Py = 0, eyb = 0, tyy_y = 0;
        double fx_c = 0, fy_c = 0, fy_y = 0, vx = 0, vy = 0, vz = 0, txy_own = 0;
        const bool yrow = YLDS && ty < TY - 1 && hy;
        if (fed) {
            vxn = sT[k - kfirst][0][tx]; vyn = sT[k - kfirst][1][tx]; vzn = sT[k - kfirst][2][tx];
            sY[6][ty][tx] = e;
        } else if (NBR && feedL) {
            vx = LDC(a.o.Vx, ovx); vy = LDC(a.o.Vy, ovy); vz = LDC(a.o.Vz, ovz);
        } else if (bvalid) {
            const u32 dz1 = hz ? sc : 0u;
            if (YLDS) {
                tyy_c = LDB(f.tyy, oc); fy_c = LFY(oc); txy_own = LDB(f.txy, oxy); r01 = LDB(f.tyz, oyz);
                if (!yrow) {
                    q01 = LDB(f.txy, oxy + rxy); r11 = LDB(f.tyz, oyz + ryz);
                    if (hy) { Py = LDB(f.P, oc + rc); eyb = LDB(et, oc + rc); tyy_y = LDB(f.tyy, oc + rc); fy_y = LFY(oc + rc); }
                }
                s01 = LDB(f.txz, oxz);
                Pz = LDB(f.P, oc + dz1); ez = LDB(et, oc + dz1); tzz_z = LDB(f.tzz, oc + dz1); fz_z = LFZ(oc + dz1);
                txx_c = LDB(f.txx, oc); fx_c = LFX(oc);
                vx = LDB(f.Vx, ovx); vy = LDB(f.Vy, ovy); vz = LDB(f.Vz, ovz);
                if (NBR) {
                    if (!hx && bc.nbR) vx = LDC(a.o.Vx, ovx);
                    if (!hy && bc.nbBk) vy = LDC(a.o.Vy, ovy);
                    if (!hz && bc.nbK1) vz = LDC(a.o.Vz, ovz);
                }
                if (YLDS == 2 && !VISC && avalid && live) {
                    P0 = LDN<(NT & 2) != 0>(f.P0, oc); Kc = LDN<(NT & 2) != 0>(f.K, oc); Qc = LDN<(NT & 2) != 0>(f.Q, oc);
                    toxx = LDN<(NT & 2) != 0>(f.toxx, oc); toyy = LDN<(NT & 2) != 0>(f.toyy, oc); tozz = LDN<(NT & 2) != 0>(f.tozz, oc);
                    toxy = LDN<(NT & 2) != 0>(f.toxy, oxy);
                    toxz = LDN<(NT & 2) != 0>(f.toxz, oxz - sxz); toyz = LDN<(NT & 2) != 0>(f.toyz, oyz - syz);
                }
                sY[0][ty][tx] = Pc; sY[1][ty][tx] = ec; sY[2][ty][tx] = tyy_c; if (NOF < 1) sY[3][ty][tx] = fy_c; sY[4][ty][tx] = txy_own; sY[5][ty][tx] = r01;
                sY[6][ty][tx] = e;
                if (!VISC) sY[7][ty][tx] = g;
            } else {
                q01 = LDB(f.txy, oxy + rxy); s01 = LDB(f.txz, oxz);
                r11 = LDB(f.tyz, oyz + ryz); r01 = LDB(f.tyz, oyz);
                Pz = LDB(f.P, oc + dz1); ez = LDB(et, oc + dz1); tzz_z = LDB(f.tzz, oc + dz1); fz_z = LFZ(oc + dz1);
                Py = LDB(f.P, oc + dy1); eyb = LDB(et, oc + dy1);
                txx_c = LDB(f.txx, oc); tyy_c = LDB(f.tyy, oc);
                tyy_y = LDB(f.tyy, oc + dy1);
                fx_c = LFX(oc); fy_c = LFY(oc); fy_y = LFY(oc + dy1);
                vx = LDB(f.Vx, ovx); vy = LDB(f.Vy, ovy); vz = LDB(f.Vz, ovz);
            }
        }
        if (YLDS) __syncthreads();
        if (fed) {
            sV[slot][0][ty][tx] = vxn; sV[slot][1][ty][tx] = vyn; sV[slot][2][ty][tx] = vzn;
        } else if (NBR && feedL) {
            sV[slot][0][ty][tx] = vx; sV[slot][1][ty][tx] = vy; sV[slot][2][ty][tx] = (!hz && bc.nsK1) ? 0.0 : vz;
        } else if (bvalid) {
            if (YLDS) {
                if (yrow) {
                    Py = sY[0][ty + 1][tx]; eyb = sY[1][ty + 1][tx]; tyy_y = sY[2][ty + 1][tx]; if (NOF < 1) fy_y = sY[3][ty + 1][tx];
                    q01 = sY[4][ty + 1][tx]; r11 = sY[5][ty + 1][tx];
                }
                if (ty > 0 && j > 0) { ey = sY[6][ty - 1][tx]; if (!VISC) gy = sY[7][ty - 1][tx]; }
// ... 253 lines not shown
```

Before: 210.3 it/s.

## Fold viscous-limit operand check into first stress sweep and reuse sample events

Instead of running a separate operand-validation kernel (reading P0, Q, old stresses, eta, K, G and forces over the whole grid) before the first iteration, the first stress sweep gets a checking form that validates the operands it already loads and sets a flag word. The verdict is read back after that sweep, and later iterations switch to the viscous-limit kernel. Timing events for profiling samples are now kept on the handle and reused rather than created and destroyed on every call. This removes one full-grid read pass and a host sync per solve, at the cost of the first iteration always running the general (non-viscous) stress kernel with extra checks.

```diff
diff --git a/justrelax.jl_amd/csrc/handle.hip b/justrelax.jl_amd/csrc/handle.hip
--- a/justrelax.jl_amd/csrc/handle.hip
+++ b/justrelax.jl_amd/csrc/handle.hip
@@ -87,6 +87,7 @@
     if (h->halo_stream) (void)hipStreamSynchronize(h->halo_stream);
     for (int i = 0; i < 8; i++)
         if (h->ev[i]) (void)hipEventDestroy(h->ev[i]);
+    for (hipEvent_t e : h->sample_ev) (void)hipEventDestroy(e);
     if (h->d_partials) (void)hipFree(h->d_partials);
     if (h->d_sums) (void)hipFree(h->d_sums);
     if (h->h_sums) (void)hipHostFree(h->h_sums);
@@ -121,7 +122,7 @@
         {"fused2d", 0, &h->fused2d}, {"vep3_edges", 1, &h->vep3_edges}, {"vep3_cfg", 1, &h->vep3_cfg}, {"vep3_peel", 0, &h->vep3_peel}, {"vep3_peel_fork", 0, &h->vep3_peel_fork}, {"vep3_nt", 0, &h->vep3_nt}, {"vep3_prekz", 1, &h->vep3_prekz},
         {"vep3_hide_comm", 1, &h->vep3_hide_comm}, {"vep3_fork", 0, &h->vep3_fork}, {"vep3_fuse_pc", 0, &h->vep3_fuse_pc}, {"vep3_np_const", 0, &h->vep3_np_const}, {"vep3_prec_tile", 1, &h->vep3_prec_tile}, {"thermal_np_const", 0, &h->thermal_np_const}, {"thermal_fused_ph", 0, &h->thermal_fused_ph}, {"fused2d_batch", 0, &h->fused2d_batch}, {"fused2d_max_nodes", 1, &h->fused2d_max_nodes}, {"vep3_map", 0, &h->vep3_map}, {"vep3_xcd", 0, &h->vep3_xcd}, {"comm_timeout_ms", 1, &h->comm_timeout_ms}, {"vep_store_all", 0, &h->vep_store_all}, {"chain_profile", 0, &h->chain_profile},
         {"general_hif", 1, &h->general_hif}, {"field_shuffle", 0, &h->field_shuffle}, {"field_pool_pct", 1, &h->field_pool_pct}, {"fused_kz", 1, &h->fused_kz}, {"fused_ym", 1, &h->fused_ym}, {"nbr_feeder", 0, &h->nbr_feeder}, {"stat_fused3d_ym", 2, &h->stat_fused3d_ym}, {"scratch_poison", 1, &h->scratch_poison},
-        {"weno_fused", 0, &h->weno_fused}, {"weno_rows", 1, &h->weno_rows},
+        {"weno_fused", 0, &h->weno_fused}, {"weno_rows", 1, &h->weno_rows}, {"march_small", 0, &h->march_small}, {"stat_visc_folded", 2, &h->stat_visc_folded},
     };
     if (tuning) {
         for (const OptRef &o : tun)
diff --git a/justrelax.jl_amd/csrc/jrx_internal.hpp b/justrelax.jl_amd/csrc/jrx_internal.hpp
--- a/justrelax.jl_amd/csrc/jrx_internal.hpp
+++ b/justrelax.jl_amd/csrc/jrx_internal.hpp
@@ -5,6 +5,7 @@
 #include <cstdio>
 #include <cstring>
 #include <cmath>
+#include <vector>
 #include "jrx.h"
 
 struct jrx_comm_state;
@@ -15,6 +16,7 @@
     hipStream_t stream = nullptr;
     hipStream_t halo_stream = nullptr;
     hipEvent_t ev[8] = {};
+    std::vector<hipEvent_t> sample_ev;
     double *d_partials = nullptr;
     double *d_sums = nullptr;
     double *h_sums = nullptr;
@@ -42,6 +44,7 @@
     bool loop_graphs = true;
     bool thermal_fused = true;
     int fused_overlap = 3;
+    bool march_small = false;
     int kernel_variant = 0;
     bool fused_split = false;
     int fused_tile = 2;
@@ -93,6 +96,7 @@
     int64_t stat_weno_calls = 0, stat_weno_fused = 0;
     int64_t stat_principal_calls = 0;
     int64_t stat_fused3d_inkernel = 0;
+    int64_t stat_visc_folded = 0;
     int64_t stat_fused3d_visc = 0, stat_visc_checks = 0, stat_visc_fallbacks = 0, stat_fused3d_nof1 = 0, stat_fused3d_nof2 = 0;
     int64_t stat_sweeps3d = 0;
     int64_t stat_fused2d_b = 0;
diff --git a/justrelax.jl_amd/csrc/stokes3d.hip b/justrelax.jl_amd/csrc/stokes3d.hip
--- a/justrelax.jl_amd/csrc/stokes3d.hip
+++ b/justrelax.jl_amd/csrc/stokes3d.hip
@@ -118,41 +118,81 @@
     if (m && (threadIdx.x & 63) == 0) atomicOr(bad, m);
 }
 
-static jrx_status visc_operands_local(jrx_handle *h, const jrx_stokes3d_fields *f, const jrx_stokes3d_params *p, bool forces);
-jrx_status visc_operands_check(jrx_handle *h, const jrx_stokes3d_fields *f, const jrx_stokes3d_params *p, bool forces = true)
-{
-    JRX_TRY(visc_operands_local(h, f, p, forces));
-    if (jrx_comm_active(h)) {
-        double v[2] = {h->visc_ok ? 0.0 : 1.0, (double)(2 - h->nof)};
-        JRX_TRY(jrx_allreduce_host(h, v, 2, 1));
-        h->visc_ok = v[0] == 0.0;
-        h->nof = 2 - (int)v[1];
-    }
-    return JRX_OK;
-}
-static jrx_status visc_operands_local(jrx_handle *h, const jrx_stokes3d_fields *f, const jrx_stokes3d_params *p, bool forces)
+static jrx_status visc_operands_local(jrx_handle *h, const jrx_stokes3d_fields *f, const jrx_stokes3d_params *p, bool forces, bool *fold, bool *synced);
+static void visc_operands_agree(jrx_handle *h, jrx_status *st)
+{
+    if (*st != JRX_OK || !jrx_comm_active(h)) return;
+    double v[2] = {h->visc_ok ? 0.0 : 1.0, (double)(2 - h->nof)};
+    *st = jrx_allreduce_host(h, v, 2, 1);
+    if (*st != JRX_OK) return;
+    h->visc_ok = v[0] == 0.0;
+    h->nof = 2 - (int)v[1];
+}
+jrx_status visc_operands_check(jrx_handle *h, const jrx_stokes3d_fields *f, const jrx_stokes3d_params *p, bool forces = true, bool *fold = nullptr, bool *synced = nullptr)
+{
+    jrx_status st = visc_operands_local(h, f, p, forces, fold, synced);
+    if (!(fold && *fold)) visc_operands_agree(h, &st);
+    return st;
+}
+struct OperandKey {
+    const void *ptr[14]; int kflags; bool forces;
+    OperandKey(const jrx_handle *h, const jrx_stokes3d_fields *f, const jrx_stokes3d_params *p, bool forces_)
+        : ptr{f->P0, f->Q, f->toxx, f->toyy, f->tozz, f->toyz, f->toxz, f->toxy, f->eta, f->K, f->G, f->fx, f->fy, f->fz}
+    {
+        forces = forces_ && h->zero_forces && f->fx && f->fy && f->fz;
+        kflags = (forces ? 1 : 0) | (h->viscous_limit ? 2 : 0) | (p->displacement_bcs ? 4 : 0) | (h->kernel_variant << 3);
+    }
+};
+struct OperandRemember {
+    jrx_handle *h; const OperandKey &key; const jrx_stokes3d_params *p; bool ok = false;
+    ~OperandRemember() {
+        h->opv.valid = ok;
+        if (!ok) return;
+        memcpy(h->opv.ptr, key.ptr, sizeof(h->opv.ptr));
+        h->opv.n[0] = p->nx; h->opv.n[1] = p->ny; h->opv.n[2] = p->nz; h->opv.dt = p->dt; h->opv.flags = key.kflags; h->opv.visc_ok = h->visc_ok; h->opv.nof = h->nof;
+    }
+};
+static jrx_status visc_operands_verdict(jrx_handle *h, hipStream_t s, bool forces)
+{
+    int *d_bad = reinterpret_cast<int *>(h->d_sums + 6), *h_bad = reinterpret_cast<int *>(h->h_sums + 6);
+    JRX_HIP(h, hipMemcpyAsync(h_bad, d_bad, sizeof(double), hipMemcpyDeviceToHost, s));
+    JRX_HIP(h, hipStreamSynchronize(s));
+    h->visc_ok = ((*h_bad & 1) == 0);
+    if (h->visc_ok && forces && !(*h_bad & 2)) h->nof = (*h_bad & 4) ? 1 : 2;
+    h->stat_visc_checks++;
+    if (!h->visc_ok) h->stat_visc_fallbacks++;
+    return JRX_OK;
+}
+jrx_status visc_operands_folded(jrx_handle *h, const jrx_stokes3d_fields *f, const jrx_stokes3d_params *p)
+{
+    const OperandKey key(h, f, p, true);
+    jrx_status st;
+    {
+        OperandRemember remember{h, key, p};
+        st = visc_operands_verdict(h, h->stream, key.forces);
+        remember.ok = st == JRX_OK;
+        if (remember.ok) h->stat_visc_folded++;
+    }
+    visc_operands_agree(h, &st);
+    return st;
+}
+static jrx_status visc_operands_local(jrx_handle *h, const jrx_stokes3d_fields *f, const jrx_stokes3d_params *p, bool forces_, bool *fold, bool *synced)
 {
     h->visc_ok = false;
     h->nof = 0;
-    forces = forces && h->zero_forces && f->fx && f->fy && f->fz;
-    const void *key[14] = {f->P0, f->Q, f->toxx, f->toyy, f->tozz, f->toyz, f->toxz, f->toxy, f->eta, f->K, f->G, f->fx, f->fy, f->fz};
-    const int kflags = (forces ? 1 : 0) | (h->viscous_limit ? 2 : 0) | (p->displacement_bcs ? 4 : 0) | (h->kernel_variant << 3);
-    if (h->operand_cache && h->opv.valid && h->opv.dt == p->dt && h->opv.flags == kflags && h->opv.n[0] == p->nx && h->opv.n[1] == p->ny && h->opv.n[2] == p->nz &&
-        memcmp(h->opv.ptr, key, sizeof(key)) == 0) {
+    const bool may_fold = fold && *fold;
+    if (fold) *fold = false;
+    if (synced) *synced = false;
+    const OperandKey key_(h, f, p, forces_);
+    const bool forces = key_.forces;
+    if (h->operand_cache && h->opv.valid && h->opv.dt == p->dt && h->opv.flags == key_.kflags && h->opv.n[0] == p->nx && h->opv.n[1] == p->ny && h->opv.n[2] == p->nz &&
+        memcmp(h->opv.ptr, key_.ptr, sizeof(key_.ptr)) == 0) {
         h->visc_ok = h->opv.visc_ok;
         h->nof = h->opv.nof;
         h->stat_operand_cache_hits++;
         return JRX_OK;
     }
-    struct Remember {
-        jrx_handle *h; const void *const *key; const jrx_stokes3d_params *p; int kflags; bool ok = false;
-        ~Remember() {
-            h->opv.valid = ok;
-            if (!ok) return;
-            memcpy(h->opv.ptr, key, sizeof(h->opv.ptr));
-            h->opv.n[0] = p->nx; h->opv.n[1] = p->ny; h->opv.n[2] = p->nz; h->opv.dt = p->dt; h->opv.flags = kflags; h->opv.visc_ok = h->visc_ok; h->opv.nof = h->nof;
-        }
-    } remember{h, key, p, kflags};
+    OperandRemember remember{h, key_, p};
     if ((!h->viscous_limit || p->dt != INFINITY) && forces && !p->displacement_bcs && (h->kernel_variant == 0 || h->kernel_variant == 3) && p->nx >= 48) {
         const i64 nc = (i64)p->nx * p->ny * p->nz;
         int *d_bad = reinterpret_cast<int *>(h->d_sums + 6), *h_bad = reinterpret_cast<int *>(h->h_sums + 6);
@@ -163,34 +203,39 @@
         JRX_LAUNCH_CHECK(h);
         JRX_HIP(h, hipMemcpyAsync(h_bad, d_bad, sizeof(double), hipMemcpyDeviceToHost, s));
         JRX_HIP(h, hipStreamSynchronize(s));
+        if (synced) *synced = true;
         if (!(*h_bad & 2)) h->nof = (*h_bad & 4) ? 1 : 2;
         remember.ok = true;
         return JRX_OK;
     }
     if (!h->viscous_limit || p->dt != INFINITY) { remember.ok = true; return JRX_OK; }
+    if (may_fold) { *fold = true; return JRX_OK; }
     const i64 nx = p->nx, ny = p->ny, nz = p->nz;
-    int *d_bad = reinterpret_cast<int *>(h->d_sums + 6), *h_bad = reinterpret_cast<int *>(h->h_sums + 6);
+    int *d_bad = reinterpret_cast<int *>(h->d_sums + 6);
     hipStream_t s = h->stream;
     JRX_HIP(h, hipMemsetAsync(d_bad, 0, sizeof(double), s));
     hipLaunchKernelGGL(k_visc_operands_ok, dim3(4096), dim3(256), 0, s, f->P0, f->Q, f->toxx, f->toyy, f->tozz, f->eta, nx * ny * nz, f->K, f->G, f->toyz, nx * (ny + 1) * (nz + 1),
                        f->toxz, (nx + 1) * ny * (nz + 1), f->toxy, (nx + 1) * (ny + 1) * nz, d_bad,
                        forces ? reinterpret_cast<const unsigned long long *>(f->fx) : nullptr, reinterpret_cast<const unsigned long long *>(f->fy), reinterpret_cast<const unsigned long long *>(f->fz));
     JRX_LAUNCH_CHECK(h);
-    JRX_HIP(h, hipMemcpyAsync(h_bad, d_bad, sizeof(double), hipMemcpyDeviceToHost, s));
-    JRX_HIP(h, hipStreamSynchronize(s));
-    h->visc_ok = ((*h_bad & 1) == 0);
-    if (h->visc_ok && forces && !(*h_bad & 2)) h->nof = (*h_bad & 4) ? 1 : 2;
-    h->stat_visc_checks++;
-    if (!h->visc_ok) h->stat_visc_fallbacks++;
+    JRX_TRY(visc_operands_verdict(h, s, forces));
+    if (synced) *synced = true;
     remember.ok = true;
     return JRX_OK;
 }
 
 template <int TX, int TY, int KZ>
-jrx_status launch_stress_zb(jrx_handle *h, hipStream_t s, const SweepArgs &a, bool diag)
+jrx_status launch_stress_zb(jrx_handle *h, hipStream_t s, const SweepArgs &a, bool diag, int chk = 0)
 {
     const TileMap tm = make_tilemap(a.L.nx, a.L.ny, a.L.nz, TX, TY, KZ);
-    if (diag) hipLaunchKernelGGL((k_stress3d_zb<true, TX, TY, KZ, 4, false, 8, true>), dim3(tm.ntiles), dim3(TX * TY), 0, s, a, tm);
+    if (chk) {
+        if (diag || (h->viscous_limit && h->visc_ok)) return jrx_fail(h, JRX_ERR_ARG, "internal: the checking stress sweep is the general state-only form");
+        int *d_bad = reinterpret_cast<int *>(h->d_sums + 6);
+        JRX_HIP(h, hipMemsetAsync(d_bad, 0, sizeof(double), s));
+        if (chk == 2) hipLaunchKernelGGL((k_stress3d_zb<false, TX, TY, KZ, 4, false, 8, true, false, 2>), dim3(tm.ntiles), dim3(TX * TY), 0, s, a, tm, d_bad);
+        else hipLaunchKernelGGL((k_stress3d_zb<false, TX, TY, KZ, 4, false, 8, true, false, 1>), dim3(tm.ntiles), dim3(TX * TY), 0, s, a, tm, d_bad);
+    }
+    else if (diag) hipLaunchKernelGGL((k_stress3d_zb<true, TX, TY, KZ, 4, false, 8, true>), dim3(tm.ntiles), dim3(TX * TY), 0, s, a, tm);
     else if (h->viscous_limit && h->visc_ok && a.dt == INFINITY)
         hipLaunchKernelGGL((k_stress3d_zb<false, TX, TY, KZ, 4, false, 8, true, true>), dim3(tm.ntiles), dim3(TX * TY), 0, s, a, tm);
     else hipLaunchKernelGGL((k_stress3d_zb<false, TX, TY, KZ, 4, false, 8, true>), dim3(tm.ntiles), dim3(TX * TY), 0, s, a, tm);
@@ -215,17 +260,24 @@
 static jrx_status launch_stress_boxes(jrx_handle *h, hipStream_t s, const SweepArgs &a, const int (*box)[6], int nbox, bool diag,
                                       const GhostRule *rule = nullptr);
 
-jrx_status launch_stress(jrx_handle *h, hipStream_t s, SweepArgs a, bool diag, int i0, int i1, int j0, int j1, int k0, int k1)
+bool stress_sweep_marches(const jrx_handle *h, const Lay3 &L)
+{
+    const bool small = !h->march_small && (double)L.nx * L.ny * L.nz <= 681472.0;
+    return !(h->kernel_variant == 1 || !fits_u32(L) || L.nx < 48 || small);
+}
+jrx_status launch_stress(jrx_handle *h, hipStream_t s, SweepArgs a, bool diag, int i0, int i1, int j0, int j1, int k0, int k1, int chk = 0)
 {
     const int nx = a.L.nx, ny = a.L.ny, nz = a.L.nz;
     const bool full = i0 == 0 && j0 == 0 && k0 == 0 && i1 == nx + 1 && j1 == ny + 1 && k1 == nz + 1;
-    const bool small = (double)nx * ny * nz <= 681472.0;
-    if (h->kernel_variant == 1 || !full || !fits_u32(a.L) || nx < 48 || small) return launch_stress_v1(h, s, a, diag, i0, i1, j0, j1, k0, k1);
+    if (!full || !stress_sweep_marches(h, a.L)) {
+        if (chk) return jrx_fail(h, JRX_ERR_ARG, "internal: only the z-marching stress sweep has a checking form");
+        return launch_stress_v1(h, s, a, diag, i0, i1, j0, j1, k0, k1);
+    }
     a.i0 = a.j0 = a.k0 = 0; a.i1 = nx; a.j1 = ny; a.k1 = nz;
-    if (nx > 384) JRX_TRY((launch_stress_zb<512, 1, 4>(h, s, a, diag)));
-    else if (nx > 192) JRX_TRY((launch_stress_zb<256, 1, 8>(h, s, a, diag)));
-    else if (nx > 96) JRX_TRY((launch_stress_zb<128, 2, 8>(h, s, a, diag)));
-    else JRX_TRY((launch_stress_zb<64, 4, 8>(h, s, a, diag)));
+    if (nx > 384) JRX_TRY((launch_stress_zb<512, 1, 4>(h, s, a, diag, chk)));
+    else if (nx > 192) JRX_TRY((launch_stress_zb<256, 1, 8>(h, s, a, diag, chk)));
+    else if (nx > 96) JRX_TRY((launch_stress_zb<128, 2, 8>(h, s, a, diag, chk)));
+    else JRX_TRY((launch_stress_zb<64, 4, 8>(h, s, a, diag, chk)));
     const int planes[3][6] = {{nx, nx + 1, 0, ny + 1, 0, nz + 1}, {0, nx, ny, ny + 1, 0, nz + 1}, {0, nx, 0, ny, nz, nz + 1}};
     return launch_stress_boxes(h, s, a, planes, 3, diag);
 }
@@ -549,6 +601,8 @@
     bool fusable = false;
     bool bcs_ordered[2] = {false, false};
     bool ghosts_stale = false;
+    int check_fold = 0;
+    bool check_synced = false;
 };
 
 static Out10 out_of(const jrx_stokes3d_fields &f) { return Out10{f.P, f.txx, f.tyy, f.tzz, f.tyz, f.txz, f.txy, f.Vx, f.Vy, f.Vz}; }
@@ -585,23 +639,37 @@
     return JRX_OK;
 }
 
-static jrx_status iter_begin(Iter3D &I, jrx_handle *h, const jrx_stokes3d_fields *f, const double *etatau, const jrx_stokes3d_params *p)
-{
-    I.h = h; I.p = p; I.etatau = etatau;
-    JRX_TRY(visc_operands_check(h, f, p));
-    I.cur = *f;
-    I.setU = out_of(*f);
-    I.pt_user = I.v_user = true; I.flip_A = I.flip_B = false; I.stress_done = false;
-    const Lay3 L = make_lay((int)p->nx, (int)p->ny, (int)p->nz);
-    I.fusable = !p->displacement_bcs && (h->kernel_variant == 0 || h->kernel_variant == 3) && h->scratch_sets && (h->fused_comm || !jrx_comm_active(h)) && fits_u32(L) && p->nx >= 48 && p->ny >= 8 && p->nz >= 8;
-    if (I.fusable && h->kernel_variant == 0) {
+static bool pipeline_fusable(const jrx_handle *h, const jrx_stokes3d_params *p, const Lay3 &L)
+{
+    bool fusable = !p->displacement_bcs && (h->kernel_variant == 0 || h->kernel_variant == 3) && h->scratch_sets && (h->fused_comm || !jrx_comm_active(h)) && fits_u32(L) && p->nx >= 48 && p->ny >= 8 && p->nz >= 8;
+    if (fusable && h->kernel_variant == 0) {
         const FusedShape S = fused_shape(h, L, p->dt);
         int nt[3];
         fused_tiles(L, S, nt);
         const int W = p->nx > 384 ? 512 : (p->nx > 192 ? 256 : (p->nx > 96 ? 128 : 64));
         const double lanes_f = (double)nt[0] * S.tx * S.ty / (S.ty - 1), lanes_s = (double)((p->nx + W - 1) / W) * W;
-        if ((double)p->nx * (double)p->ny * (double)p->nz >= 1e6 && 0.62 * lanes_f > 1.15 * lanes_s) I.fusable = false;
-    }
+        if ((double)p->nx * (double)p->ny * (double)p->nz >= 1e6 && 0.62 * lanes_f > 1.15 * lanes_s) fusable = false;
+    }
+    return fusable;
+}
+
+static jrx_status iter_begin(Iter3D &I, jrx_handle *h, const jrx_stokes3d_fields *f, const double *etatau, const jrx_stokes3d_params *p, bool first_plain)
+{
+    I.h = h; I.p = p; I.etatau = etatau;
+    const Lay3 L = make_lay((int)p->nx, (int)p->ny, (int)p->nz);
+    bool fold = first_plain && !p->displacement_bcs && (h->kernel_variant == 0 || h->kernel_variant == 3) && stress_sweep_marches(h, L);
+    if (fold) {
+        h->visc_ok = true;
+        const bool with = pipeline_fusable(h, p, L);
+        h->visc_ok = false;
+        fold = with == pipeline_fusable(h, p, L);
+    }
+    JRX_TRY(visc_operands_check(h, f, p, true, &fold, &I.check_synced));
+    I.check_fold = !fold ? 0 : (h->zero_forces && f->fx && f->fy && f->fz ? 2 : 1);
+    I.cur = *f;
+    I.setU = out_of(*f);
+    I.pt_user = I.v_user = true; I.flip_A = I.flip_B = false; I.stress_done = false;
+    I.fusable = pipeline_fusable(h, p, L);
     if (I.fusable) {
         JRX_TRY(ensure_scratch(h, (int)p->nx, (int)p->ny, (int)p->nz));
         double **S = h->scratch;
@@ -771,14 +839,18 @@
         if (I.flip_A) {
             const Out10 other = mix_sets(I.pt_user ? I.setS : I.setU, I.v_user ? I.setU : I.setS);
             a.o = other;
-            JRX_TRY(launch_stress(h, s, a, diag, 0, nx + 1, 0, ny + 1, 0, nz + 1));
+            JRX_TRY(launch_stress(h, s, a, diag, 0, nx + 1, 0, ny + 1, 0, nz + 1, I.check_fold));
             set_state(I.cur, other);
             I.pt_user = !I.pt_user;
             I.flip_A = false;
             a = make_args(&I.cur, I.etatau, p);
         } else
-            JRX_TRY(launch_stress(h, s, a, diag, 0, nx + 1, 0, ny + 1, 0, nz + 1));
-    }
+            JRX_TRY(launch_stress(h, s, a, diag, 0, nx + 1, 0, ny + 1, 0, nz + 1, I.check_fold));
+        if (I.check_fold) {
+            I.check_fold = 0;
+            JRX_TRY(visc_operands_folded(h, &I.cur, p));
+        }
+    } else if (I.check_fold) return jrx_fail(h, JRX_ERR_ARG, "internal: a folded operand check without its stress sweep");
     I.stress_done = false;
     if (tev) JRX_HIP(h, hipEventRecord(tev[1], s));
 
@@ -1119,10 +1191,10 @@
     const int rank = jrx_comm_rank(h);
     hipEvent_t t0 = h->ev[6], t1 = h->ev[7];
     Iter3D I;
-    JRX_TRY(iter_begin(I, h, f, h->etatau, p));
-    JRX_HIP(h, hipEventRecord(t0, s));
     auto keep_going = [&](int64_t it) { return it < 2 || (((err / err_it1) > p->eps_rel && err > p->eps_abs) && it <= p->iterMax); };
     auto is_check = [&](int64_t it1) { return (it1 % p->nout == 0) && it1 > 1; };
+    JRX_TRY(iter_begin(I, h, f, h->etatau, p, !(is_check(1) || !keep_going(1))));
+    JRX_HIP(h, hipEventRecord(t0, s));
     constexpr int GIT = 16;
     GraphExecs gexec;
     bool graphs = h->loop_graphs && !I.fusable && !jrx_comm_active(h) && !p->displacement_bcs && p->periodic == 0 && (double)n <= kGraphCells3D;
@@ -1223,15 +1295,18 @@
     const int64_t stride = iters > 64 ? (((iters + 63) / 64) | 1) : 1;
     const int nsamp = (int)((iters + stride - 1) / stride);
     const bool chain = h->chain_profile && jrx_comm_active(h);
-    std::vector<hipEvent_t> evs((size_t)nsamp * (chain ? 8 : 4));
+    std::vector<hipEvent_t> &evs = h->sample_ev;
+    const size_t nev = (size_t)nsamp * (chain ? 8 : 4);
+    while (evs.size() < nev) {
+        hipEvent_t e = nullptr;
+        JRX_HIP(h, hipEventCreate(&e));
+        evs.push_back(e);
+    }
     std::vector<int> fused((size_t)nsamp, 0), cmode((size_t)nsamp, 0);
     std::vector<double> ncell((size_t)nsamp, 0.0);
-    struct EvGuard { std::vector<hipEvent_t> &v; ~EvGuard() { for (auto &e : v) if (e) (void)hipEventDestroy(e); } } guard{evs};
-    for (auto &e : evs) e = nullptr;
-    for (auto &e : evs) JRX_HIP(h, hipEventCreate(&e));
     Iter3D I;
-    JRX_TRY(iter_begin(I, h, f, etatau, p));
-    JRX_HIP(h, hipStreamSynchronize(s));
+    JRX_TRY(iter_begin(I, h, f, etatau, p, true));
+    if (!I.check_synced && !I.check_fold) JRX_HIP(h, hipStreamSynchronize(s));
     JRX_HIP(h, hipEventRecord(h->ev[6], s));
     const bool odd = I.fusable && iters >= 2 && ((iters - 1) % 2 == 1);
     const bool flips = odd && h->end_flips && !jrx_comm_active(h) && p->periodic == 0 && !p->displacement_bcs;
diff --git a/justrelax.jl_amd/csrc/stokes3d_kernels.hpp b/justrelax.jl_amd/csrc/stokes3d_kernels.hpp
--- a/justrelax.jl_amd/csrc/stokes3d_kernels.hpp
+++ b/justrelax.jl_amd/csrc/stokes3d_kernels.hpp
@@ -354,11 +354,12 @@
     return true;
 }
 
-template <bool DIAG, int TX, int TY, int KZ, int MINW, bool EDGES, int XCD = 0, bool SHF = false, bool VISC = false>
-__global__ __launch_bounds__(TX *TY, MINW) void k_stress3d_zb(const SweepArgs a, const TileMap tm)
+template <bool DIAG, int TX, int TY, int KZ, int MINW, bool EDGES, int XCD = 0, bool SHF = false, bool VISC = false, int CHK = 0>
+__global__ __launch_bounds__(TX *TY, MINW) void k_stress3d_zb(const SweepArgs a, const TileMap tm, int *bad = nullptr)
 {
     static_assert(!SHF || (TX % 64 == 0 && !EDGES), "SHF needs whole waves per row");
     static_assert(!VISC || (!DIAG && !EDGES), "the viscous-limit form is the state-only sweep over the interior tiles");
+    static_assert(!CHK || (!VISC && !DIAG && !EDGES && TX % 64 == 0), "the checking form is the general state-only sweep, whole waves per row");
     const Lay3 &L = a.L;
     const int nx = L.nx, ny = L.ny, nz = L.nz;
     int tx, ty, tz;
@@ -391,6 +392,9 @@
     double e_p = LDB(f.eta, oc - back), ex_p = LDB(f.eta, oc - back - dcx), ey_p = LDB(f.eta, oc - back - dcy);
     double g_p = 1.0, gx_p = 1.0, gy_p = 1.0;
     if (!VISC) { g_p = LDB(f.G, oc - back); gx_p = LDB(f.G, oc - back - dcx); gy_p = LDB(f.G, oc - back - dcy); }
+    [[maybe_unused]] int chk = 0;
+    [[maybe_unused]] auto fin = [&](double v) { if (!isfinite(v)) chk |= 1; };
+    [[maybe_unused]] auto mod = [&](double v) { if (v != v || v == 0.0) chk |= 1; };
 
     for (int k = kb; k < kend; ++k) {
         const double va = LDB(f.Vx, ovx), vay = LDB(f.Vx, ovx - rvx);
@@ -422,6 +426,16 @@
         const double txy = LDB(f.txy, oxy), toxy = VISC ? 0.0 : LDB(f.toxy, oxy);
         const double txz = LDB(f.txz, oxz), toxz = VISC ? 0.0 : LDB(f.toxz, oxz);
         const double tyz = LDB(f.tyz, oyz), toyz = VISC ? 0.0 : LDB(f.toyz, oyz);
+        if (CHK) {
+            fin(P0); fin(Qc); fin(toxx); fin(toyy); fin(tozz); fin(toxy); fin(toxz); fin(toyz); fin(e); mod(Kc); mod(g);
+            if (xhi) { fin(LDB(f.toxy, oxy + 8u)); fin(LDB(f.toxz, oxz + 8u)); }
+            if (yhi) { fin(LDB(f.toxy, oxy + 8u * (u32)L.xy1)); fin(LDB(f.toyz, oyz + 8u * (u32)L.yz1)); }
+            if (xhi && yhi) fin(LDB(f.toxy, oxy + 8u * (u32)L.xy1 + 8u));
+            if (CHK == 2) {
+                if ((__double_as_longlong(LDB(f.fx, oc)) | __double_as_longlong(LDB(f.fy, oc))) != 0) chk |= 2;
+                if (__double_as_longlong(LDB(f.fz, oc)) != 0) chk |= 4;
+            }
+        }
 
         {
             const double dxi = (-va + vax) * _dx;
@@ -481,6 +495,15 @@
         a_p = va; b_p = vb; c_p = vc; cx_p = vcx; cy_p = vcy;
         e_p = e; ex_p = ex; ey_p = ey; g_p = g; gx_p = gx; gy_p = gy;
         oc += sc; ovx += svx; ovy += svy; ovz += svz; oxy += sxy; oxz += sxz; oyz += syz;
+    }
+    if (CHK) {
+        if (kend == nz) {
+            fin(LDB(f.toxz, oxz)); fin(LDB(f.toyz, oyz));
+            if (xhi) fin(LDB(f.toxz, oxz + 8u));
+            if (yhi) fin(LDB(f.toyz, oyz + 8u * (u32)L.yz1));
+        }
+        const int m = (__any(chk & 1) ? 1 : 0) | (__any(chk & 2) ? 2 : 0) | (__any(chk & 4) ? 4 : 0);
+        if (m && (threadIdx.x & 63) == 0) atomicOr(bad, m);
     }
     if (EDGES && kend == nz) {
         node_xz<DIAG>(a, i, j, nz);
```

Result: slower. 207.2 it/s (-1.5%).
